# Eric-qi/NeuroQuant

Hardware: AMD Instinct MI355X
Metric: calibration iters/sec (HNeRV Bunny 1280x640, 21k iters) + final PSNR vs ref (higher is better)
Workload: dtype f32 operands split into bf16 hi+lo, 3 BF16 MFMAs per product, fp32 accumulate (bf16x3); fp32 MFMA on small layers; 1 GPU; HNeRV Bunny_1280x640_3M, channel_wise, bits 6 5 4 5 5 6 6, phase-2 (AdaRound) iteration; per_gpu_batch=2, global_batch=2, frames=132, parallelism=dp1

## Files before the change

include/nq_hip.h:

```cpp
#ifndef NQ_HIP_H
#define NQ_HIP_H

#include <stdint.h>

#ifdef __cplusplus
extern "C" {
#endif

typedef void* nq_stream_t;

#define NQ_API __attribute__((visibility("default")))

#define NQ_OK 0
#define NQ_ERR_INVALID (-1)
#define NQ_ERR_UNSUPPORTED (-2)
#define NQ_ERR_LAUNCH (-3)

NQ_API int nq_abi_version(void);
NQ_API const char* nq_error_string(int code);


NQ_API int nq_scale_init_max(const float* x, int64_t rows, int64_t row_len, int n_levels, float* delta, float* zp,
                      nq_stream_t stream);

// ... 113 lines not shown

#define NQ_EPI_PLAIN 0
#define NQ_EPI_PS_GELU 1
#define NQ_EPI_TANH 2
#define NQ_EPI_PS 3
#define NQ_EPI_DGRAD_GELU 4
#define NQ_EPI_X_SPLIT 0x100
#define NQ_EPI_Y_SPLIT 0x200
NQ_API int nq_split_words(const float* x, float* y, int64_t n, nq_stream_t stream);
NQ_API int64_t nq_conv_forward_ws_floats(int B, int Cin, int H, int W, int Cout, int k);
NQ_API int nq_conv_split_out(int B, int Cin, int H, int W, int Cout, int k, int r, int epilogue, int in_gelu, int has_bias);
NQ_API int nq_conv_forward(const float* x, const float* wt, const float* bias, float* y, float* z, float* ws, int B, int Cin, int H,
                    int W, int Cout, int k, int krows, int ld, int r, int epilogue, int in_gelu, const float* zprev,
                    nq_stream_t stream);

NQ_API int nq_conv3_supported(int B, int Cin, int H, int W, int Cout, int k);
NQ_API int nq_conv3_split_io(int B, int Cin, int H, int W, int Cout, int k);
NQ_API int64_t nq_conv_forward3_ws_floats(int B, int Cin, int H, int W, int Cout, int k);
NQ_API int64_t nq_conv3_weight_bytes(int Cin, int Cout, int k);
NQ_API int nq_weight_layout3(const float* w, void* wt3, int Cin, int Cout, int k, int transposed, nq_stream_t stream);
typedef struct nq_wl3_seg {
  const float* w;
  void* wt3;
  int Cin, Cout, k, transposed;
} nq_wl3_seg;
NQ_API int nq_weight_layout3_multi(const nq_wl3_seg* segs, int nseg, nq_stream_t stream);
NQ_API int nq_weight_layouts_all(const nq_wl3_seg* segs3, int n3, const nq_wl_seg* segsf, int nf, nq_stream_t stream);
NQ_API int nq_conv_forward3(const float* x, const void* wt3, const float* bias, float* y, float* z, const float* zprev, float* ws, int B,
                     int Cin, int H, int W, int Cout, int k, int r, int epilogue, nq_stream_t stream);

NQ_API int nq_conv_wgrad3_supported(int B, int Cin, int H, int W, int Cout, int k);
NQ_API int64_t nq_conv_wgrad3_ws_floats(int B, int Cin, int H, int W, int Cout, int k);
NQ_API int nq_conv_wgrad3_plan(int B, int Cin, int H, int W, int Cout, int k, int* mi, int* ni, int* nsplit, int* pc);
NQ_API int nq_conv_wgrad3(const float* x, const float* dy, float* dw, float* db, float* ws, int B, int Cin, int H, int W, int Cout,
                   int k, nq_stream_t stream);
NQ_API int nq_conv_wgrad3_split_io(int B, int Cin, int H, int W, int Cout, int k);
NQ_API int nq_conv_wgrad3_fmt(const float* x, const float* dy, float* dw, float* db, float* ws, int B, int Cin, int H, int W, int Cout,
                       int k, int fmt, nq_stream_t stream);
NQ_API int nq_conv_wgrad3_swapped(const float* x, const float* dy, float* dw, float* ws, int B, int Cin, int H, int W, int Cout, int k,
                           nq_stream_t stream);

NQ_API int64_t nq_conv_wgrad_ws_floats(int B, int Cin, int H, int W, int Cout, int k);
NQ_API int nq_conv_wgrad(const float* x, const float* dy, float* dw, float* db, float* ws, int B, int Cin, int H, int W, int Cout,
                  int k, int x_gelu, nq_stream_t stream);

typedef struct nq_wgr_seg {
  const float* slab;
  const float* slab_db;
  float* dw;
  float* db;
  int Cout, N, co_pad, n_pad, nsplit;
  int swap_kk;
  int sg;
} nq_wgr_seg;
NQ_API int nq_conv_wgrad3_slabs(const float* x, const float* dy, float* dw, float* db, float* ws, int B, int Cin, int H, int W, int Cout,
                         int k, nq_wgr_seg* seg, nq_stream_t stream);
NQ_API int nq_conv_wgrad3_slabs_fmt(const float* x, const float* dy, float* dw, float* db, float* ws, int B, int Cin, int H, int W,
                             int Cout, int k, nq_wgr_seg* seg, int fmt, nq_stream_t stream);
NQ_API int nq_conv_wgrad3_swapped_slabs(const float* x, const float* dy, float* dw, float* ws, int B, int Cin, int H, int W, int Cout,
                                 int k, nq_wgr_seg* seg, nq_stream_t stream);
NQ_API int nq_conv_wgrad_slabs(const float* x, const float* dy, float* dw, float* db, float* ws, int B, int Cin, int H, int W, int Cout,
                        int k, int x_gelu, nq_wgr_seg* seg, nq_stream_t stream);
NQ_API int nq_wgrad_reduce_multi(const nq_wgr_seg* segs, int nseg, nq_stream_t stream);

NQ_API int nq_ps_gelu_backward(const float* da, const float* z, float* dconv, int B, int C, int H, int W, int r,
                        nq_stream_t stream);

NQ_API int nq_tanh_out_backward(const float* dimg, const float* img, float* dconv, int64_t n, nq_stream_t stream);

NQ_API int nq_l2_loss(const float* pred, const float* tgt, float* loss, float* dpred, float* ws, int64_t n, int64_t mean_count,
               float gscale, nq_stream_t stream);

NQ_API int nq_channel_sum(const float* x, float* out, float* ws, int B, int C, int64_t HW, nq_stream_t stream);

NQ_API int nq_l2_loss_tanh_head(const float* pred, const float* tgt, const uint8_t* cache_u8, const int64_t* idx, float* loss,
                         float* dconv, float* db, float* ws, int B, int C, int64_t HW, int64_t mean_count, float gscale,
                         nq_stream_t stream);

NQ_API int64_t nq_head_forward_loss_ws_floats(int B, int H, int W);
NQ_API int nq_head_forward_loss(const float* x, const float* wt, int ld, const float* bias, float* y, const float* tgt,
                         const uint8_t* cache_u8, const int64_t* idx, float* loss, float* dconv, float* db, float* ws, int B,
                         int Cin, int H, int W, int64_t mean_count, float gscale, nq_stream_t stream);

NQ_API int nq_frame_sse(const float* out, const float* gt, float* sse, int64_t frames, int64_t frame_len, nq_stream_t stream);

NQ_API int64_t nq_ms_ssim_ws_floats(int64_t frames, int C, int H, int W);
NQ_API int nq_ms_ssim(const float* out, const float* gt, float* msssim, float* ws, int64_t frames, int C, int H, int W,
               nq_stream_t stream);

NQ_API int nq_gather_frames_u8(const uint8_t* src, const int64_t* idx, float* dst, int64_t n, int64_t frame_len,
                        nq_stream_t stream);

NQ_API int nq_act_dd(const float* x, const float* g, const float* g2, float* y, int64_t n, int mode, nq_stream_t stream);
NQ_API int nq_pixel_shuffle(const float* x, float* y, int B, int C, int H, int W, int r, int inverse, nq_stream_t stream);
NQ_API int nq_bias_add(const float* x, const float* bias, float* y, int B, int C, int64_t HW, nq_stream_t stream);

#ifdef __cplusplus
}
#endif
#endif
```

neuroquant_amd/_lib.py:

```python
import ctypes
import os
from ctypes import c_char_p, c_float, c_int, c_int64, c_void_p, POINTER, Structure

_HERE = os.path.dirname(os.path.abspath(__file__))
LIB_PATH = os.environ.get("NQ_LIB") or os.path.join(_HERE, "libnqhip.so")

NQ_OK = 0
ABI_VERSION = 5
EPI_PLAIN, EPI_PS_GELU, EPI_TANH, EPI_PS, EPI_DGRAD_GELU = 0, 1, 2, 3, 4


class NQLibraryError(RuntimeError):
    pass


class AdaSeg(Structure):
    _fields_ = [("x", c_void_p), ("gy", c_void_p), ("alpha", c_void_p), ("delta", c_void_p), ("zp", c_void_p),
                ("out", c_void_p), ("rows", c_int64), ("row_len", c_int64), ("per_row", c_int), ("n_levels", c_int),
                ("soft", c_int), ("reg_weight", c_float)]


class WL3Seg(Structure):
    _fields_ = [("w", c_void_p), ("wt3", c_void_p), ("Cin", c_int), ("Cout", c_int), ("k", c_int), ("transposed", c_int)]


class WLSeg(Structure):
    _fields_ = [("w", c_void_p), ("wt_fwd", c_void_p), ("wt_bwd", c_void_p), ("Cout", c_int), ("Cin", c_int), ("k", c_int),
                ("krows_fwd", c_int), ("ld_fwd", c_int), ("krows_bwd", c_int), ("ld_bwd", c_int)]


class FwhtSeg(Structure):
    _fields_ = [("x", c_void_p), ("y", c_void_p), ("outer", c_int64), ("inner", c_int64), ("n", c_int), ("n_in", c_int),
                ("n_out", c_int)]


class AdaAdamSeg(Structure):
    _fields_ = [("x", c_void_p), ("gy", c_void_p), ("alpha", c_void_p), ("delta", c_void_p), ("zp", c_void_p), ("m", c_void_p),
                ("v", c_void_p), ("rows", c_int64), ("row_len", c_int64), ("per_row", c_int), ("n_levels", c_int),
                ("reg_weight", c_float)]


class WgrSeg(Structure):
    _fields_ = [("slab", c_void_p), ("slab_db", c_void_p), ("dw", c_void_p), ("db", c_void_p), ("Cout", c_int), ("N", c_int),
                ("co_pad", c_int), ("n_pad", c_int), ("nsplit", c_int), ("swap_kk", c_int), ("sg", c_int)]


class FqFwhtSeg(Structure):
    _fields_ = [("x", c_void_p), ("alpha", c_void_p), ("delta", c_void_p), ("zp", c_void_p), ("m", c_void_p), ("v", c_void_p),
                ("gy", c_void_p), ("y", c_void_p), ("outer", c_int64), ("inner", c_int64), ("n", c_int), ("c_in", c_int),
                ("per_row", c_int), ("n_levels", c_int), ("soft", c_int), ("reg_weight", c_float)]


class AdamSeg(Structure):
    _fields_ = [("p", c_void_p), ("g", c_void_p), ("m", c_void_p), ("v", c_void_p), ("n", c_int64)]


def _load():
    if not os.path.exists(LIB_PATH):
        raise NQLibraryError(
            f"{LIB_PATH} not found: build it with `python -c 'import __graft_entry__ as g; g.build()'` "
            "(or `make -C neuroquant_amd/csrc`).  neuroquant_amd has no CPU/eager fallback.")
    import torch
    lib = ctypes.CDLL(LIB_PATH)
    P, I, L, F = c_void_p, c_int, c_int64, c_float

    def sig(name, res, *args):
        fn = getattr(lib, name)
        fn.restype = res
        fn.argtypes = list(args)

    sig("nq_abi_version", I)
    got = lib.nq_abi_version()
    if got != ABI_VERSION:
        raise NQLibraryError(f"{LIB_PATH} has ABI version {got}, this package binds version {ABI_VERSION}: rebuild it "
                             "(`make -C neuroquant_amd/csrc`)")
    sig("nq_error_string", c_char_p, I)
    sig("nq_scale_init_max", I, P, L, L, I, P, P, P)
    sig("nq_uaq_forward", I, P, P, P, P, L, L, I, I, P)
    sig("nq_uaq_backward", I, P, P, P, P, P, P, L, L, I, I, P)
    sig("nq_adaround_init", I, P, P, P, P, P, P, L, L, I, P)
    sig("nq_adaround_forward", I, P, P, P, P, P, P, L, L, I, I, I, P)
    sig("nq_adaround_backward", I, P, P, P, P, P, P, L, L, I, I, F, F, P)
    sig("nq_adaround_adam_multi", I, POINTER(AdaAdamSeg), I, F, F, F, F, F, F, P, P)
    sig("nq_adaround_forward_multi", I, POINTER(AdaSeg), I, P)
    sig("nq_uaq_forward_multi", I, POINTER(AdaSeg), I, P)
    sig("nq_uaq_backward_multi", I, POINTER(AdaSeg), I, P)
    sig("nq_adaround_backward_multi", I, POINTER(AdaSeg), I, F, P)
    sig("nq_adam_step_multi", I, POINTER(AdamSeg), I, F, F, F, F, F, P)
    sig("nq_step_prologue", I, P, P, P, P, P, I, I, P)
    sig("nq_step_prologue_gather", I, P, P, P, P, P, I, I, P, L, L, P, P)
    sig("nq_adaround_backward_multi_dyn", I, POINTER(AdaSeg), I, P, P)
    sig("nq_adam_step_multi_dyn", I, POINTER(AdamSeg), I, P, F, F, F, P)
    sig("nq_reduce_ws_floats", L, L)
    sig("nq_round_loss", I, P, L, F, F, P, P, I, P)
    sig("nq_round_loss_backward", I, P, L, F, F, P, P, I, P)
    sig("nq_adam_step", I, P, P, P, P, L, F, F, F, F, F, P)
    sig("nq_fwht", I, P, P, L, I, L, I, I, P)
    sig("nq_fwht_multi", I, POINTER(FwhtSeg), I, P)
    sig("nq_weight_layouts", I, P, P, P, I, I, I, I, I, I, I, P)
    sig("nq_conv_operand_dims", I, I, I, I, POINTER(c_int), POINTER(c_int))
    sig("nq_conv_forward_ws_floats", L, I, I, I, I, I, I)
    sig("nq_conv_forward", I, P, P, P, P, P, P, I, I, I, I, I, I, I, I, I, I, I, P, P)
    sig("nq_conv3_supported", I, I, I, I, I, I, I)
    sig("nq_conv3_split_io", I, I, I, I, I, I, I)
    sig("nq_conv_split_out", I, I, I, I, I, I, I, I, I, I, I)
    sig("nq_split_words", I, P, P, L, P)
    sig("nq_conv_wgrad3_split_io", I, I, I, I, I, I, I)
    sig("nq_conv_wgrad3_fmt", I, P, P, P, P, P, I, I, I, I, I, I, I, P)
    sig("nq_conv_wgrad3_slabs_fmt", I, P, P, P, P, P, I, I, I, I, I, I, POINTER(WgrSeg), I, P)
    sig("nq_conv3_weight_bytes", L, I, I, I)
    sig("nq_weight_layout3", I, P, P, I, I, I, I, P)
    sig("nq_weight_layout3_multi", I, POINTER(WL3Seg), I, P)
    sig("nq_weight_layouts_multi", I, POINTER(WLSeg), I, P)
    sig("nq_weight_layouts_all", I, POINTER(WL3Seg), I, POINTER(WLSeg), I, P)
    sig("nq_conv_forward3_ws_floats", L, I, I, I, I, I, I)
    sig("nq_conv_forward3", I, P, P, P, P, P, P, P, I, I, I, I, I, I, I, I, P)
    sig("nq_conv_wgrad3_supported", I, I, I, I, I, I, I)
    sig("nq_conv_wgrad3_ws_floats", L, I, I, I, I, I, I)
    sig("nq_conv_wgrad3_plan", I, I, I, I, I, I, I, POINTER(c_int), POINTER(c_int), POINTER(c_int), POINTER(c_int))
    sig("nq_conv_wgrad3", I, P, P, P, P, P, I, I, I, I, I, I, P)
    sig("nq_conv_wgrad3_swapped", I, P, P, P, P, I, I, I, I, I, I, P)
    sig("nq_conv_wgrad3_slabs", I, P, P, P, P, P, I, I, I, I, I, I, POINTER(WgrSeg), P)
    sig("nq_conv_wgrad3_swapped_slabs", I, P, P, P, P, I, I, I, I, I, I, POINTER(WgrSeg), P)
    sig("nq_conv_wgrad_slabs", I, P, P, P, P, P, I, I, I, I, I, I, I, POINTER(WgrSeg), P)
    sig("nq_wgrad_reduce_multi", I, POINTER(WgrSeg), I, P)
    sig("nq_conv_wgrad_ws_floats", L, I, I, I, I, I, I)
    sig("nq_conv_wgrad", I, P, P, P, P, P, I, I, I, I, I, I, I, P)
    sig("nq_ps_gelu_backward", I, P, P, P, I, I, I, I, I, P)
    sig("nq_tanh_out_backward", I, P, P, P, L, P)
    sig("nq_l2_loss", I, P, P, P, P, P, L, L, F, P)
    sig("nq_channel_sum", I, P, P, P, I, I, L, P)
    sig("nq_l2_loss_tanh_head", I, P, P, P, P, P, P, P, P, I, I, L, L, F, P)
    sig("nq_frame_sse", I, P, P, P, L, L, P)
    sig("nq_ms_ssim_ws_floats", L, L, I, I, I)
    sig("nq_ms_ssim", I, P, P, P, P, L, I, I, I, P)
    sig("nq_gather_frames_u8", I, P, P, P, L, L, P)
    sig("nq_adaround_fwht_multi", I, POINTER(FqFwhtSeg), I, P)
    sig("nq_fwht_adaround_adam_multi", I, POINTER(FqFwhtSeg), I, F, F, F, F, F, F, P, P)
    sig("nq_head_forward_loss_ws_floats", L, I, I, I)
    sig("nq_head_forward_loss", I, P, P, I, P, P, P, P, P, P, P, P, P, I, I, I, I, L, F, P)
    sig("nq_act_dd", I, P, P, P, P, L, I, P)
    sig("nq_pixel_shuffle", I, P, P, I, I, I, I, I, I, P)
    sig("nq_bias_add", I, P, P, P, I, I, L, P)
    return lib


EXPORTS = (
    "nq_abi_version", "nq_error_string", "nq_scale_init_max", "nq_uaq_forward", "nq_uaq_backward",
    "nq_adaround_init", "nq_adaround_forward", "nq_adaround_backward", "nq_reduce_ws_floats", "nq_round_loss", "nq_round_loss_backward",
    "nq_adam_step", "nq_adaround_adam_multi", "nq_adaround_forward_multi", "nq_uaq_forward_multi", "nq_uaq_backward_multi", "nq_adaround_backward_multi", "nq_adam_step_multi", "nq_step_prologue", "nq_step_prologue_gather", "nq_adaround_backward_multi_dyn", "nq_adam_step_multi_dyn", "nq_fwht", "nq_fwht_multi", "nq_weight_layouts", "nq_conv_operand_dims", "nq_conv_forward_ws_floats", "nq_conv_forward",
    "nq_conv3_supported", "nq_conv3_weight_bytes", "nq_weight_layout3", "nq_weight_layout3_multi", "nq_weight_layouts_multi", "nq_conv_forward3_ws_floats", "nq_conv_forward3",
    "nq_conv_wgrad3_supported", "nq_conv_wgrad3_ws_floats", "nq_conv_wgrad3_plan", "nq_conv_wgrad3", "nq_conv_wgrad3_swapped",
    "nq_conv_wgrad3_slabs", "nq_conv_wgrad3_swapped_slabs", "nq_conv_wgrad_slabs", "nq_wgrad_reduce_multi",
    "nq_conv_wgrad_ws_floats", "nq_conv_wgrad", "nq_ps_gelu_backward", "nq_tanh_out_backward", "nq_l2_loss",
    "nq_channel_sum", "nq_l2_loss_tanh_head", "nq_frame_sse", "nq_ms_ssim_ws_floats", "nq_ms_ssim", "nq_gather_frames_u8",
    "nq_act_dd", "nq_pixel_shuffle", "nq_bias_add", "nq_conv3_split_io", "nq_conv_split_out", "nq_split_words",
    "nq_conv_wgrad3_split_io", "nq_conv_wgrad3_fmt", "nq_conv_wgrad3_slabs_fmt", "nq_head_forward_loss_ws_floats", "nq_head_forward_loss",
    "nq_adaround_fwht_multi", "nq_fwht_adaround_adam_multi", "nq_weight_layouts_all",
)

_lib = None


def lib():
    global _lib
    if _lib is None:
        _lib = _load()
    return _lib


def check(rc, what=""):
    if rc != NQ_OK:
        msg = lib().nq_error_string(rc).decode()
        raise NQLibraryError(f"libnqhip {what}: {msg} ({rc})")
```

neuroquant_amd/csrc/conv3.hip:

```cpp
#include <cstdlib>
#include "nq_common.h"
#include "conv3_layout.h"

extern "C" {
int nq_conv_igemm3_k3(const float*, const void*, const float*, float*, float*, const float*, int, int, int, int, int, int, int,
                      int, int, int, float*, hipStream_t);
int nq_conv_igemm3_k5(const float*, const void*, const float*, float*, float*, const float*, int, int, int, int, int, int, int,
                      int, int, int, float*, hipStream_t);
int nq_conv_splitk_finish(const float*, const float*, float*, float*, const float*, int, int, int, int, int, int, int, hipStream_t);
int nq_conv3_nst_k3();
int nq_conv3_nst_k5();
int nq_conv3_nst8_k3();
int nq_conv3_nst8_k5();
int nq_conv3_nstk_k3(int);
int nq_conv3_nstk_k5(int);
int nq_conv_flat3_plan(int, int, int, int, int, int, int*, int*, int*, int*);
int nq_conv_flat3(const float*, const void*, const float*, float*, float*, const float*, float*, int, int, int, int, int, int, int, int,
                  int, int, int, int, hipStream_t);
int nq_conv_wgrad_flat3_ok(int, int, int, int, int, int);
int nq_conv_wgrad_flat3(const float*, const float*, float*, float*, int, int, int, int, int, int, hipStream_t);
int nq_conv_wgrad3_k3(const float*, const float*, float*, float*, int, int, int, int, int, int, int, int, int, int, int, int, hipStream_t);
int nq_conv_wgrad3_k5(const float*, const float*, float*, float*, int, int, int, int, int, int, int, int, int, int, int, int, hipStream_t);
}

namespace {

constexpr int CC = 16;

inline int pick_mi3(int Cout) {
  if (Cout <= 16) return 1;
  if (Cout <= 32) return 2;
  int best = 3, best_pad = 1 << 30;
  for (int mi = 5; mi >= 3; --mi) {
    int mt = 16 * mi, pad = (Cout + mt - 1) / mt * mt;
    if (pad < best_pad) {
      best_pad = pad;
      best = mi;
    }
  }
  if (Cout > 256 && (Cout + 63) / 64 * 64 <= best_pad + best_pad * 6 / 100) return 4;
  return best;
}
inline int nst_of(int k) { return k == 5 ? nq_conv3_nst_k5() : nq_conv3_nst_k3(); }
inline int nstk_of(int k, int kind) { return k == 5 ? nq_conv3_nstk_k5(kind) : nq_conv3_nstk_k3(kind); }
inline int tail_kind_of(int Cin, int mi) {
  const int r = Cin - CC * ((Cin + CC - 1) / CC - 1);
  return r <= 4 ? 1 : (r <= 8 ? 2 : (r <= 12 ? 3 : 0));
}
inline int64_t total_steps3(int Cin, int k, int mi) {
  const int nchunk = (Cin + CC - 1) / CC;
  return (int64_t)(nchunk - 1) * nst_of(k) + nstk_of(k, tail_kind_of(Cin, mi));
}

struct WL3 {
  const float* w;
  uint4* out;
  int Cin, Cout, KK, NST, NSTT, nchunk, tail, co_tiles, MT, transposed;
  int co16;
  int64_t slots;
};

constexpr int WL3_KKMAX = 25;
template <int KK>
__device__ __forceinline__ void wl3_tile(const WL3& p, int c, int g16, float* __restrict__ T ) {
  constexpr int RS = 16 * KK + 1;
  const int tid = threadIdx.x;
  const int nfull = p.nchunk - (p.tail ? 1 : 0);
  const int kind = (c == nfull) ? p.tail : 0;
  const int nst = kind ? p.NSTT : p.NST;
  const int64_t gs0 = (int64_t)c * p.NST;
  const int Ra = p.transposed ? p.Cin : p.Cout;
  const int Cb = p.transposed ? p.Cout : p.Cin;
  const int a0 = p.transposed ? c * 16 : g16 * 16, b0 = p.transposed ? g16 * 16 : c * 16;
  {
    float v[KK];
#pragma unroll
    for (int j = 0; j < KK; ++j) {
      const int e = tid + j * 256;
      const int a = e / (16 * KK), rem = e - a * (16 * KK);
      const int bb = rem / KK;
      const bool ok = a0 + a < Ra && b0 + bb < Cb;
      const float t = p.w[ok ? ((int64_t)(a0 + a) * Cb + b0) * KK + rem : 0];
      v[j] = ok ? t : 0.f;
    }
#pragma unroll
// ... 175 lines not shown
  p.pc = 0;
  const bool pc_ok = wgrad3_pc_enabled() && (int64_t)B * Cin * H * W * 4 < (1ll << 31) && (int64_t)B * Cout * H * W * 4 < (1ll << 31);
  if (pc_ok && p.ni >= 5 && p.mi >= 3 && tiles <= 256) {
    int sy = 1;
    int ns_pc = 256 / tiles;
    const int segs_x = (W + 31) / 32;
    static const int minseg = [] { const char* e = std::getenv("NQ_WGRAD3_MINSEG"); return e ? atoi(e) : 6; }();
    if (!wgrad3_ss1() && ns_pc >= 1) {
      if (H % 4 == 0 && segs_x * (H / 4) * B / ns_pc >= minseg) sy = 4;
      else if (H % 2 == 0 && segs_x * (H / 2) * B / ns_pc >= minseg) sy = 2;
    }
    const int nseg_pc = segs_x * (H / sy) * B;
    const int need = minseg < 16 ? minseg : 16;
    static const int shrink = [] { const char* e = std::getenv("NQ_WGRAD3_SHRINK"); return e ? atoi(e) : 1; }();
    if (shrink && ns_pc >= 1 && nseg_pc / ns_pc < need && (nseg_pc / need) * tiles >= 192) ns_pc = nseg_pc / need;
    if (ns_pc >= 1 && nseg_pc / ns_pc >= need) {
      p.pc = sy == 1 ? 1 : 10 + sy;
      p.nsplit = ns_pc;
    }
  }
  if (pc_ok && p.ni == 1 && p.mi >= 2 && p.mi <= 5 && tiles == 1 && W % 128 == 0) {
    const int nseg_pc = (W / 128) * H * B;
    if (nseg_pc / 256 >= 8) {
      p.pc = 4;
      static const int hs = [] { const char* e = std::getenv("NQ_WGRAD3_HEAD_SPLITS"); return e ? atoi(e) : 512; }();
      p.nsplit = (p.mi <= 3 && nseg_pc / hs >= 8) ? hs : 256;
    }
  }
  return p;
}

template <int SG>
__global__ __launch_bounds__(256) void wgrad3_reduce_kernel(const float* __restrict__ slab, const float* __restrict__ slab_db,
                                                            float* __restrict__ dw, float* __restrict__ db, int Cout, int N,
                                                            int co_pad, int n_pad, int nsplit, int swap_kk) {
  constexpr int OG = 256 / SG;
  __shared__ float part[SG][OG];
  const int o = threadIdx.x % OG, g = threadIdx.x / OG;
  const int64_t i = (int64_t)blockIdx.x * OG + o;
  const int64_t total = (int64_t)Cout * N;
  float s = 0.f;
  if (i < total) {
    const int co = (int)(i / N), n = (int)(i - (int64_t)co * N);
    const float* p = slab + (int64_t)co * n_pad + n;
    const int64_t stride = (int64_t)co_pad * n_pad;
#pragma unroll 4
    for (int k = g; k < nsplit; k += SG) s += p[k * stride];
  } else if (db && i < total + Cout) {
    const int co = (int)(i - total);
#pragma unroll 4
    for (int k = g; k < nsplit; k += SG) s += slab_db[(int64_t)k * co_pad + co];
  }
  part[g][o] = s;
  __syncthreads();
  if (g == 0) {
    float t = part[0][o];
#pragma unroll
    for (int j = 1; j < SG; ++j) t += part[j][o];
    if (i < total) {
      if (swap_kk > 0) {
        const int co = (int)(i / N), n = (int)(i - (int64_t)co * N);
        const int ci = n / swap_kk, tap = n - ci * swap_kk;
        dw[((int64_t)ci * Cout + co) * swap_kk + (swap_kk - 1 - tap)] = t;
      } else {
        dw[i] = t;
      }
    } else if (db && i < total + Cout) {
      db[(int)(i - total)] = t;
    }
  }
}

constexpr int WGR_MAXSEG = 16;
struct WGRMulti {
  nq_wgr_seg s[WGR_MAXSEG];
  int blk0[WGR_MAXSEG + 1];
  int nseg;
};
__global__ __launch_bounds__(256) void wgrad_reduce_multi_kernel(WGRMulti t) {
  __shared__ float4 part[256];
  int k = 0;
  while (k + 1 < t.nseg && (int)blockIdx.x >= t.blk0[k + 1]) ++k;
  const nq_wgr_seg& q = t.s[k];
  const int SG = q.sg, OG = 256 / SG;
  const int o = threadIdx.x % OG, g = threadIdx.x / OG;
  const int N = q.N, Cout = q.Cout, nsplit = q.nsplit;
  const int NQ = (N + 3) >> 2;
  const int64_t i = (int64_t)((int)blockIdx.x - t.blk0[k]) * OG + o;
  const int64_t total = (int64_t)Cout * NQ;
  float4 s = make_float4(0.f, 0.f, 0.f, 0.f);
  int co = 0, n = 0;
  if (i < total) {
    co = (int)(i / NQ);
    n = 4 * (int)(i - (int64_t)co * NQ);
    const float* p = q.slab + (int64_t)co * q.n_pad + n;
    const int64_t stride = (int64_t)q.co_pad * q.n_pad;
#pragma unroll 8
    for (int j = g; j < nsplit; j += SG) {
      const float4 v = *reinterpret_cast<const float4*>(p + j * stride);
      s.x += v.x; s.y += v.y; s.z += v.z; s.w += v.w;
    }
  } else if (q.db && i < total + Cout) {
    const int cb = (int)(i - total);
#pragma unroll 8
    for (int j = g; j < nsplit; j += SG) s.x += q.slab_db[(int64_t)j * q.co_pad + cb];
  }
  if (SG > 1) {
    part[g * OG + o] = s;
    __syncthreads();
    if (g != 0) return;
    s = part[o];
    for (int j = 1; j < SG; ++j) {
      const float4 v = part[j * OG + o];
      s.x += v.x; s.y += v.y; s.z += v.z; s.w += v.w;
    }
  }
  if (i < total) {
    const float sv[4] = {s.x, s.y, s.z, s.w};
    if (q.swap_kk > 0) {
#pragma unroll
      for (int e = 0; e < 4; ++e) {
        if (n + e >= N) break;
        const int ci = (n + e) / q.swap_kk, tap = (n + e) - ci * q.swap_kk;
        q.dw[((int64_t)ci * Cout + co) * q.swap_kk + (q.swap_kk - 1 - tap)] = sv[e];
      }
    } else if ((N & 3) == 0) {
      *reinterpret_cast<float4*>(q.dw + (int64_t)co * N + n) = s;
    } else {
#pragma unroll
      for (int e = 0; e < 4; ++e)
        if (n + e < N) q.dw[(int64_t)co * N + n + e] = sv[e];
    }
  } else if (q.db && i < total + Cout) {
    q.db[(int)(i - total)] = s.x;
  }
}

}

extern "C" {

int nq_conv3_supported(int B, int Cin, int H, int W, int Cout, int k) {
  if (!(k == 3 || k == 5) || B <= 0 || Cin <= 0 || Cout <= 4 || Cin <= 4) return 0;
  if ((int64_t)B * Cin * H * W * 4 >= 0xFFFFFF00ll) return 0;
  if (use_flat3(B, Cin, H, W, Cout, k, nullptr) && (int64_t)Cin * k * k * Cout >= 65536) return 1;
  const Fwd3Plan p = plan_fwd3(B, Cin, H, W, Cout);
  return p.wgs * p.nsplit >= 128;
}

int64_t nq_conv_forward3_ws_floats(int B, int Cin, int H, int W, int Cout, int k) {
  if (!(k == 3 || k == 5) || B <= 0 || Cin <= 0 || H <= 0 || W <= 0 || Cout <= 0) return 0;
  int fns = 1;
  if (use_flat3(B, Cin, H, W, Cout, k, &fns)) return fns > 1 ? (int64_t)fns * B * Cout * H * W : 0;
  const Fwd3Plan p = plan_fwd3(B, Cin, H, W, Cout);
  return p.nsplit > 1 ? (int64_t)p.nsplit * B * Cout * H * W : 0;
}

int64_t nq_conv3_weight_bytes(int Cin, int Cout, int k) {
  if (!(k == 3 || k == 5)) return 0;
  const int mi = pick_mi3(Cout), mt = 16 * mi;
  const int64_t co_tiles = (Cout + mt - 1) / mt, nchunk = (Cin + CC - 1) / CC;
  (void)nchunk;
  return total_steps3(Cin, k, mi) * 2 * co_tiles * 4 * mt * 16;
}

static bool wl3_fill(WL3& p, const float* w, void* wt3, int Cin, int Cout, int k, int transposed) {
  if (!w || !wt3 || !(k == 3 || k == 5) || Cin <= 0 || Cout <= 0) return false;
  const int mi = pick_mi3(Cout);
  p.w = w; p.out = reinterpret_cast<uint4*>(wt3);
  p.Cin = Cin; p.Cout = Cout; p.KK = k * k; p.NST = nst_of(k); p.tail = tail_kind_of(Cin, mi); p.NSTT = nstk_of(k, p.tail);
  p.MT = 16 * mi; p.co_tiles = (Cout + p.MT - 1) / p.MT; p.nchunk = (Cin + CC - 1) / CC; p.transposed = transposed;
  p.slots = total_steps3(Cin, k, mi) * p.co_tiles * 4 * p.MT;
  p.co16 = (p.co_tiles * p.MT + 15) / 16;
  return true;
}

int nq_weight_layout3(const float* w, void* wt3, int Cin, int Cout, int k, int transposed, nq_stream_t stream) {
  WL3 p;
  if (!wl3_fill(p, w, wt3, Cin, Cout, k, transposed)) return NQ_ERR_INVALID;
  hipLaunchKernelGGL(weight_layout3_kernel, dim3((unsigned)(p.nchunk * p.co16)), dim3(256), 0, nq_s(stream), p);
  return nq_launch_status();
}

int nq_weight_layout3_multi(const nq_wl3_seg* segs, int nseg, nq_stream_t stream) {
  if (!segs || nseg <= 0) return NQ_ERR_INVALID;
  for (int base = 0; base < nseg; base += WL3_MAXSEG) {
    WL3Multi t;
    t.nseg = (nseg - base < WL3_MAXSEG) ? nseg - base : WL3_MAXSEG;
    int blocks = 0;
    for (int i = 0; i < t.nseg; ++i) {
      const nq_wl3_seg& h = segs[base + i];
      if (!wl3_fill(t.s[i], h.w, h.wt3, h.Cin, h.Cout, h.k, h.transposed)) return NQ_ERR_INVALID;
      t.blk0[i] = blocks;
      blocks += t.s[i].nchunk * t.s[i].co16;
    }
    t.blk0[t.nseg] = blocks;
    hipLaunchKernelGGL(weight_layout3_multi_kernel, dim3((unsigned)blocks), dim3(256), 0, nq_s(stream), t);
  }
  return nq_launch_status();
// ... 212 lines not shown
```

neuroquant_amd/csrc/conv_head.hip:

```cpp
#include <cstdlib>
#include <cstring>
#include <type_traits>

#include "nq_common.h"

namespace {

constexpr int MAXCO = 4;
using f32x2 = __attribute__((ext_vector_type(2))) float;
using f32x4 = __attribute__((ext_vector_type(4))) float;

template <int I0, int N, class F>
__device__ __forceinline__ void hf2_rows(F&& f) {
  if constexpr (I0 < N) {
    f(std::integral_constant<int, I0>{});
    hf2_rows<I0 + 1, N>(f);
  }
}

template <int KS>
__global__ __launch_bounds__(256) void head_fwd_kernel(const float* __restrict__ x, const float* __restrict__ wt, int ld,
                                                       const float* __restrict__ bias, float* __restrict__ y, int Cin,
                                                       int H, int W, int CO, int epi, int tiles_x) {
  constexpr int KK = KS * KS, PAD = KS / 2;
// ... 215 lines not shown
    __builtin_amdgcn_s_waitcnt(0xC07F);
    __builtin_amdgcn_sched_barrier(0);
    load_x(ci + 2, vA, eA);
    load_w(ci + 2, wA);
    __builtin_amdgcn_sched_barrier(0);
    compute(vB, eB, wB);
    __builtin_amdgcn_s_waitcnt(0xC07F);
    __builtin_amdgcn_sched_barrier(0);
  }
  if (Cin & 1) compute(vA, eA, wA);

  float bv[NCO];
#pragma unroll
  for (int co = 0; co < NCO; ++co) bv[co] = bias ? bias[co] : 0.f;
  float lsum = 0.f, gsum[NCO];
#pragma unroll
  for (int co = 0; co < NCO; ++co) gsum[co] = 0.f;
  __amdgpu_buffer_rsrc_t rs_d = rs_y;
  int64_t tbase = 0;
  if constexpr (LOSS) {
    rs_d = __builtin_amdgcn_make_buffer_rsrc(la.dconv, 0, (int)((unsigned)a.B * NCO * HWb), 0x00020000);
    tbase = (la.cache ? la.idx[b] : (int64_t)b) * NCO * (int64_t)H * W;
  }
#pragma unroll
  for (int r = 0; r < R; ++r) {
    const int oy = y0 + r;
    const bool in = oy < H && gx < W;
    const unsigned so = in ? ((unsigned)b * NCO * (unsigned)H + (unsigned)oy) * Wb + (unsigned)gx * 4u : OOB;
#pragma unroll
    for (int co = 0; co < NCO; ++co) {
      f32x4 o;
#pragma unroll
      for (int p = 0; p < 4; ++p) {
        const float v = acc[r][co][p >> 1][p & 1] + bv[co];
        o[p] = TANH ? tanhf(v) * 0.5f + 0.5f : v;
      }
      __builtin_amdgcn_raw_buffer_store_b128(__builtin_bit_cast(__attribute__((ext_vector_type(4))) unsigned, o), rs_y,
                                             so == OOB ? OOB : so + (unsigned)co * HWb, 0, 0);
      if constexpr (LOSS) {
        f32x4 t4 = {0.f, 0.f, 0.f, 0.f};
        if (in) {
          const int64_t te = tbase + ((int64_t)co * H + oy) * W + gx;
          if (la.cache) {
            const uchar4 u = *reinterpret_cast<const uchar4*>(la.cache + te);
            t4 = f32x4{(float)u.x / 255.f, (float)u.y / 255.f, (float)u.z / 255.f, (float)u.w / 255.f};
          } else {
            t4 = *reinterpret_cast<const f32x4*>(la.tgt + te);
          }
        }
        f32x4 dc;
#pragma unroll
        for (int p = 0; p < 4; ++p) {
          const float d = o[p] - t4[p];
          const float g = la.gcoef * d;
          const float u = 2.f * o[p] - 1.f;
          const float rr = g * 0.5f * (1.f - u * u);
          dc[p] = rr;
          if (in) {
            lsum += d * d;
            gsum[co] += rr;
          }
        }
        __builtin_amdgcn_raw_buffer_store_b128(__builtin_bit_cast(__attribute__((ext_vector_type(4))) unsigned, dc), rs_d,
                                               so == OOB ? OOB : so + (unsigned)co * HWb, 0, 0);
      }
    }
  }
  if constexpr (LOSS) {
    lsum = nq_wave_sum(lsum);
#pragma unroll
    for (int co = 0; co < NCO; ++co) gsum[co] = nq_wave_sum(gsum[co]);
    if (lane == 0) {
      float* w4 = la.ws + (int64_t)wid * 4;
      w4[0] = lsum;
#pragma unroll
      for (int co = 0; co < NCO && co < 3; ++co) w4[1 + co] = gsum[co];
    }
  }
}

__global__ __launch_bounds__(256) void head_loss_stage2(const float* __restrict__ ws, int waves, float scale,
                                                        float* __restrict__ loss, float* __restrict__ db) {
  __shared__ float red[16];
  float acc = 0.f;
  for (int i = threadIdx.x; i < waves; i += 256) acc += ws[(int64_t)i * 4 + blockIdx.x];
  const float s = nq_block_sum(acc, red);
  if (threadIdx.x == 0) {
    if (blockIdx.x == 0) loss[0] = 0.f + s * scale;
    else db[blockIdx.x - 1] = s;
  }
}

template <int KS, int R2, int NCO, int PX>
__global__ __launch_bounds__(256) __attribute__((amdgpu_waves_per_eu((KS <= 3 && NCO <= 3 && R2 && PX == 4) ? 4 : 1, 8))) void head_dgrad_kernel(const float* __restrict__ dy, const float* __restrict__ wt, int ld,
                                                         const float* __restrict__ zprev, float* __restrict__ out,
                                                         int Cin, int H, int W, int CO, int r, int tiles_x) {
  constexpr int KK = KS * KS, PAD = KS / 2;
  constexpr int TW = 64, TPR = TW / PX, TH = 256 / TPR;
  constexpr int PH = TH + KS - 1, PW = TW + KS - 1;
  constexpr int PWS = (PW + 3) / 4 * 4;
  __shared__ __attribute__((aligned(16))) float patch[NCO * PH * PWS];
  constexpr int KKP = (KK + 3) / 4 * 4;
  constexpr int WROW = NCO * KKP;
  constexpr int WL_MAX = 64;
  __shared__ __attribute__((aligned(16))) float wl[WL_MAX * WROW];

  const int tid = threadIdx.x;
  const int row = tid / TPR, c4 = (tid % TPR) * PX;
  const int lid = nq_xcd_chunk((int)blockIdx.x, (int)gridDim.x);
  const int tiles = tiles_x * ((H + TH - 1) / TH), tile = lid % tiles;
  const int tile_x = tile % tiles_x, tile_y = tile / tiles_x;
  const int x0 = tile_x * TW, y0 = tile_y * TH, b = lid / tiles;
  const int64_t HW = (int64_t)H * W;
  const float* __restrict__ dyb = dy + (int64_t)b * CO * HW;

  for (int e = tid; e < CO * PH * PW; e += 256) {
    int co = e / (PH * PW), rem = e - co * (PH * PW);
    int rr = rem / PW, c = rem - rr * PW;
    int gy = y0 - PAD + rr, gx = x0 - PAD + c;
    float v = 0.f;
    if (gy >= 0 && gy < H && gx >= 0 && gx < W) v = dyb[(int64_t)co * HW + (int64_t)gy * W + gx];
    patch[(co * PH + rr) * PWS + c] = v;
  }
  __syncthreads();
  float nb[NCO][KS][PX + KS - 1];
#pragma unroll
  for (int co = 0; co < NCO; ++co)
#pragma unroll
    for (int kh = 0; kh < KS; ++kh)
#pragma unroll
      for (int j = 0; j < PX + KS - 1; ++j) nb[co][kh][j] = (co < CO) ? patch[(co * PH + row + kh) * PWS + c4 + j] : 0.f;

  const int gy = y0 + row, gx0 = x0 + c4;
  const bool active = (gy < H && gx0 < W);
  const bool full = (gx0 + PX - 1 < W);
#pragma unroll 1
  for (int ci = 0; ci < Cin; ++ci) {
    if (ci % WL_MAX == 0) {
      __syncthreads();
      const int nci = min(WL_MAX, Cin - ci);
      for (int e = tid; e < nci * WROW; e += 256) {
        const int cl = e / WROW, j = e - cl * WROW;
        const int co = j / KKP, tap = j - co * KKP;
        wl[e] = (co < CO && tap < KK) ? wt[(int64_t)(co * KK + tap) * ld + ci + cl] : 0.f;
      }
      __syncthreads();
    }
    if (!active) continue;
    float acc[PX];
#pragma unroll
    for (int p = 0; p < PX; ++p) acc[p] = 0.f;
    const float* __restrict__ wrow = wl + (ci % WL_MAX) * WROW;
#pragma unroll
    for (int co = 0; co < NCO; ++co) {
      if (co < CO) {
        float wv[KKP];
#pragma unroll
        for (int q = 0; q < KKP / 4; ++q) {
          const float4 t = *reinterpret_cast<const float4*>(wrow + co * KKP + 4 * q);
          wv[4 * q] = t.x; wv[4 * q + 1] = t.y; wv[4 * q + 2] = t.z; wv[4 * q + 3] = t.w;
        }
#pragma unroll
        for (int kh = 0; kh < KS; ++kh)
#pragma unroll
          for (int kw = 0; kw < KS; ++kw) {
#pragma unroll
            for (int p = 0; p < PX; ++p) acc[p] = fmaf(wv[kh * KS + kw], nb[co][kh][p + kw], acc[p]);
          }
        __builtin_amdgcn_sched_barrier(0);
// ... 148 lines not shown
            acc0 = __builtin_elementwise_fma(w2, f32x2{in[kw], in[kw + 1]}, acc0);
            acc1 = __builtin_elementwise_fma(w2, f32x2{in[kw + 2], in[kw + 3]}, acc1);
          }
      const f32x4 zz = z[r];
      f32x2 ev = {acc0[0] * zz[0], acc1[0] * zz[2]}, od = {acc0[1] * zz[1], acc1[1] * zz[3]};
      if (a.out_split) {
        ev = f32x2{nq_split_word_f(ev[0]), nq_split_word_f(ev[1])};
        od = f32x2{nq_split_word_f(od[0]), nq_split_word_f(od[1])};
      }
      const unsigned vo = oo[r];
      __builtin_amdgcn_raw_buffer_store_b64(__builtin_bit_cast(__attribute__((ext_vector_type(2))) unsigned, ev), rs_o, vo, so, 0);
      __builtin_amdgcn_raw_buffer_store_b64(__builtin_bit_cast(__attribute__((ext_vector_type(2))) unsigned, od), rs_o,
                                            vo == OOB ? OOB : vo + plane_b, so, 0);
    }
  };

  f32x4 zA[R], zB[R], wA[WROW / 4], wB[WROW / 4];
  load_z(0, zA);
  load_w(0, wA);
#pragma unroll 1
  for (int ci = 0; ci + 1 < Cin; ci += 2) {
    load_z(ci + 1, zB);
    load_w(ci + 1, wB);
    __builtin_amdgcn_sched_barrier(0);
    compute(ci, zA, wA);
    __builtin_amdgcn_sched_barrier(0);
    load_z(ci + 2, zA);
    load_w(ci + 2, wA);
    __builtin_amdgcn_sched_barrier(0);
    compute(ci + 1, zB, wB);
    __builtin_amdgcn_sched_barrier(0);
  }
  if (Cin & 1) compute(Cin - 1, zA, wA);
}

}

extern "C" {

int nq_head_supported(int Cout, int k) { return Cout <= MAXCO && (k == 1 || k == 3 || k == 5); }

int nq_head_forward(const float* x, const float* wt, int ld, const float* bias, float* y, int B, int Cin, int H, int W,
                    int Cout, int k, int epi, hipStream_t st) {
  const char* hv = getenv("NQ_HEAD_FWD");
  const bool v1 = hv && hv[0] == '1';
  if (k == 3 && Cout == 3 && (W & 3) == 0 && (ld & 3) == 0 && (int64_t)B * Cin * H * W * 4 < 0xFFFFFF00ll && !v1) {
    int R = 4;
    if (const char* rd = getenv("NQ_HEAD_RD")) R = atoi(rd);
    HeadFwd2Args a;
    a.B = B; a.Cin = Cin; a.H = H; a.W = W; a.ld = ld;
    a.strips = (W + 255) / 256; a.rblocks = (H + R - 1) / R;
    a.x_bytes = (unsigned)((int64_t)B * Cin * H * W * 4);
    a.hot_first = head_hot_first(B, a.strips, a.rblocks);
    const int waves = B * a.strips * a.rblocks;
    dim3 g2((unsigned)((waves + 3) / 4)), blk2(256);
    const size_t lds = 0;
    const bool th = epi == NQ_EPI_TANH;
#define NQ_HF2(R_)                                                                                              \
  if (R == R_) {                                                                                                \
    if (th) hipLaunchKernelGGL((head_fwd2_kernel<R_, 3, true>), g2, blk2, lds, st, x, wt, bias, y, a);          \
    else hipLaunchKernelGGL((head_fwd2_kernel<R_, 3, false>), g2, blk2, lds, st, x, wt, bias, y, a);            \
    return nq_launch_status();                                                                                  \
  }
    NQ_HF2(4)
    NQ_HF2(5)
#undef NQ_HF2
    return NQ_ERR_UNSUPPORTED;
  }
  const int tiles_x = (W + 63) / 64, tiles = tiles_x * ((H + 15) / 16);
  dim3 g((unsigned)(tiles * B)), blk(256);
  switch (k) {
    case 1: hipLaunchKernelGGL(head_fwd_kernel<1>, g, blk, 0, st, x, wt, ld, bias, y, Cin, H, W, Cout, epi, tiles_x); break;
    case 3: hipLaunchKernelGGL(head_fwd_kernel<3>, g, blk, 0, st, x, wt, ld, bias, y, Cin, H, W, Cout, epi, tiles_x); break;
    default: hipLaunchKernelGGL(head_fwd_kernel<5>, g, blk, 0, st, x, wt, ld, bias, y, Cin, H, W, Cout, epi, tiles_x); break;
  }
  return nq_launch_status();
}

int64_t nq_head_forward_loss_ws_floats(int B, int H, int W) {
  if (B <= 0 || H <= 0 || W <= 0) return 0;
  return (int64_t)B * ((W + 255) / 256) * ((H + 3) / 4) * 4;
}

int nq_head_forward_loss(const float* x, const float* wt, int ld, const float* bias, float* y, const float* tgt,
                         const uint8_t* cache_u8, const int64_t* idx, float* loss, float* dconv, float* db, float* ws, int B,
                         int Cin, int H, int W, int64_t mean_count, float gscale, nq_stream_t stream) {
  if (!x || !wt || !y || !loss || !dconv || !db || !ws || B <= 0 || Cin <= 0 || H <= 0 || W <= 0 || mean_count <= 0) return NQ_ERR_INVALID;
  if ((tgt == nullptr) == (cache_u8 == nullptr) || (cache_u8 && !idx)) return NQ_ERR_INVALID;
  if ((W & 3) != 0 || (ld & 3) != 0 || (int64_t)B * Cin * H * W * 4 >= 0xFFFFFF00ll) return NQ_ERR_UNSUPPORTED;
  constexpr int R = 4;
  HeadFwd2Args a;
  a.B = B; a.Cin = Cin; a.H = H; a.W = W; a.ld = ld;
  a.strips = (W + 255) / 256; a.rblocks = (H + R - 1) / R;
  a.x_bytes = (unsigned)((int64_t)B * Cin * H * W * 4);
  a.hot_first = head_hot_first(B, a.strips, a.rblocks);
  HeadLossArgs la;
  la.tgt = tgt; la.cache = cache_u8; la.idx = idx; la.dconv = dconv; la.ws = ws;
  la.gcoef = (float)(2.0 / (double)mean_count) * gscale;
  const int waves = B * a.strips * a.rblocks;
  hipStream_t st = nq_s(stream);
  hipLaunchKernelGGL((head_fwd2_kernel<R, 3, true, true>), dim3((unsigned)((waves + 3) / 4)), dim3(256), 0, st, x, wt, bias, y, a, la);
  hipLaunchKernelGGL(head_loss_stage2, dim3(4), dim3(256), 0, st, ws, waves, (float)(1.0 / (double)mean_count), loss, db);
  return nq_launch_status();
}

int nq_head_dgrad_streams(int B, int Cin, int H, int W, int Cout, int k, int r, int has_z) {
  const char* hv = getenv("NQ_HEAD_DGRAD");
  const char* rd = getenv("NQ_HEAD_DG_R");
  const int R = rd ? atoi(rd) : 4;
  return k == 3 && Cout == 3 && r == 2 && has_z && (W % 4 == 0) && (H % 2 == 0) && (int64_t)B * Cin * H * W * 4 < 0xFFFFFF00ll &&
         !(hv && hv[0] == '1') && (size_t)Cin * 28 * 4 <= 64 * 1024 && (R == 2 || R == 4);
}

int nq_head_dgrad(const float* dy, const float* wt, int ld, const float* zprev, float* out, int B, int Cin, int H, int W,
                  int Cout, int k, int r, int out_split, hipStream_t st) {
  if (out_split && !nq_head_dgrad_streams(B, Cin, H, W, Cout, k, r, zprev != nullptr)) return NQ_ERR_UNSUPPORTED;
  const char* hv = getenv("NQ_HEAD_DGRAD");
  if (k == 3 && Cout == 3 && r == 2 && zprev && (W % 4 == 0) && (H % 2 == 0) && (int64_t)B * Cin * H * W * 4 < 0xFFFFFF00ll &&
      !(hv && hv[0] == '1')) {
    int R = 4;
    if (const char* rd = getenv("NQ_HEAD_DG_R")) R = atoi(rd);
    HeadDg2Args a;
    a.B = B; a.Cin = Cin; a.H = H; a.W = W; a.ld = ld;
    a.strips = (W + 255) / 256; a.rblocks = (H + R - 1) / R;
    a.dy_bytes = (unsigned)((int64_t)B * Cout * H * W * 4);
    a.z_bytes = (unsigned)((int64_t)B * Cin * H * W * 4);
    a.out_split = out_split;
    const int waves = B * a.strips * a.rblocks;
    dim3 g2((unsigned)((waves + 3) / 4)), blk2(256);
    const size_t lds = (size_t)Cin * 28 * 4;
    if (lds <= 64 * 1024) {
      if (R == 2) hipLaunchKernelGGL((head_dgrad2_kernel<2, 3>), g2, blk2, lds, st, dy, wt, zprev, out, a);
      else if (R == 4) hipLaunchKernelGGL((head_dgrad2_kernel<4, 3>), g2, blk2, lds, st, dy, wt, zprev, out, a);
      else return NQ_ERR_UNSUPPORTED;
      return nq_launch_status();
    }
  }
  const bool r2 = (r == 2) && (W % 4 == 0) && (H % 2 == 0);
  const bool px8 = r2 && (W % 8 == 0) && k <= 3;
  const int th = px8 ? 32 : 16;
  const int tiles_x = (W + 63) / 64, tiles = tiles_x * ((H + th - 1) / th);
  dim3 g((unsigned)(tiles * B)), blk(256);
#define NQ_HD(KS_, R2_, PX_)                                                                                          \
  do {                                                                                                                \
    if (Cout <= 3)                                                                                                    \
      hipLaunchKernelGGL((head_dgrad_kernel<KS_, R2_, 3, PX_>), g, blk, 0, st, dy, wt, ld, zprev, out, Cin, H, W, Cout, r, \
                         tiles_x);                                                                                    \
    else                                                                                                              \
      hipLaunchKernelGGL((head_dgrad_kernel<KS_, R2_, 4, PX_>), g, blk, 0, st, dy, wt, ld, zprev, out, Cin, H, W, Cout, r, \
                         tiles_x);                                                                                    \
  } while (0)
  switch (k) {
    case 1: if (px8) NQ_HD(1, 1, 8); else if (r2) NQ_HD(1, 1, 4); else NQ_HD(1, 0, 4); break;
    case 3: if (px8) NQ_HD(3, 1, 8); else if (r2) NQ_HD(3, 1, 4); else NQ_HD(3, 0, 4); break;
    default: if (r2) NQ_HD(5, 1, 4); else NQ_HD(5, 0, 4); break;
  }
#undef NQ_HD
  return nq_launch_status();
}

}
```

neuroquant_amd/csrc/conv_tiny.hip:

```cpp
#include "nq_common.h"

namespace {

template <int KSL>
__global__ __launch_bounds__(256) void tiny_pw_fwd_kernel(const float* __restrict__ x, const float* __restrict__ wt,
                                                          const float* __restrict__ bias, float* __restrict__ y,
                                                          float* __restrict__ z, const float* __restrict__ zprev, int B,
                                                          int Cin, int H, int W, int Cout, int ld, int r, int epi) {
  constexpr int OPB = 256 / KSL;
  __shared__ float part[KSL][OPB];
  const int HW = H * W;
  const int o = threadIdx.x % OPB, ks = threadIdx.x / OPB;
  const int64_t t = (int64_t)blockIdx.x * OPB + o;
  const bool live = t < (int64_t)B * HW * Cout;
  const int co = live ? (int)(t % Cout) : 0, bp = live ? (int)(t / Cout) : 0;
  const int b = bp / HW, p = bp - b * HW;
  const float* __restrict__ xp = x + (int64_t)b * Cin * HW + p;
  float acc = 0.f;
#pragma unroll 8
  for (int ci = ks; ci < Cin; ci += KSL) acc = fmaf(wt[(int64_t)ci * ld + co], xp[(int64_t)ci * HW], acc);
  if (KSL > 1) {
    part[ks][o] = acc;
    __syncthreads();
    if (ks != 0) return;
    acc = part[0][o];
#pragma unroll
    for (int j = 1; j < KSL; ++j) acc += part[j][o];
  }
  if (!live) return;
  float v = acc + (bias ? bias[co] : 0.f);
  const int py = p / W, px = p - py * W;
  if (epi == NQ_EPI_PS_GELU || epi == NQ_EPI_PS) {
    const int rr = r * r, C = Cout / rr;
    const int c = co / rr, rem = co - c * rr, si = rem / r, sj = rem - si * r;
    const int64_t o = (((int64_t)b * C + c) * (H * r) + (int64_t)py * r + si) * ((int64_t)W * r) + (int64_t)px * r + sj;
    if (epi == NQ_EPI_PS_GELU) {
      float gv, dv;
      nq_gelu_pair(v, gv, dv);
      y[o] = gv;
      z[o] = dv;
    } else {
      z[o] = v;
    }
  } else if (epi == NQ_EPI_DGRAD_GELU) {
    const int64_t i = ((int64_t)b * Cout + co) * HW + p;
    v *= zprev[i];
    if (r == 1) {
      y[i] = v;
    } else {
      const int rr = r * r, yq = py / r, xq = px / r;
      const int ch = co * rr + (py - yq * r) * r + (px - xq * r);
      y[(((int64_t)b * Cout * rr + ch) * (H / r) + yq) * (int64_t)(W / r) + xq] = v;
    }
  } else {
    const int64_t i = ((int64_t)b * Cout + co) * HW + p;
    y[i] = (epi == NQ_EPI_TANH) ? tanhf(v) * 0.5f + 0.5f : v;
  }
}

__global__ __launch_bounds__(256) void tiny_pw_wgrad_kernel(const float* __restrict__ x, const float* __restrict__ dy,
                                                            float* __restrict__ dw, float* __restrict__ db, int B, int Cin,
                                                            int HW, int Cout) {
  const int64_t t = (int64_t)blockIdx.x * 256 + threadIdx.x;
  const int64_t nw = (int64_t)Cout * Cin;
  if (t < nw) {
    const int co = (int)(t / Cin), ci = (int)(t - (int64_t)co * Cin);
    float acc = 0.f;
    for (int b = 0; b < B; ++b) {
      const float* __restrict__ dp = dy + ((int64_t)b * Cout + co) * HW;
      const float* __restrict__ xp = x + ((int64_t)b * Cin + ci) * HW;
      if ((HW & 7) == 0) {
        for (int p = 0; p < HW; p += 8) {
          const float4 d0 = *reinterpret_cast<const float4*>(dp + p), d1 = *reinterpret_cast<const float4*>(dp + p + 4);
          const float4 x0 = *reinterpret_cast<const float4*>(xp + p), x1 = *reinterpret_cast<const float4*>(xp + p + 4);
          acc = fmaf(d0.x, x0.x, acc); acc = fmaf(d0.y, x0.y, acc); acc = fmaf(d0.z, x0.z, acc); acc = fmaf(d0.w, x0.w, acc);
          acc = fmaf(d1.x, x1.x, acc); acc = fmaf(d1.y, x1.y, acc); acc = fmaf(d1.z, x1.z, acc); acc = fmaf(d1.w, x1.w, acc);
        }
      } else {
        for (int p = 0; p < HW; ++p) acc = fmaf(dp[p], xp[p], acc);
      }
    }
    dw[t] = acc;
  } else if (db && t < nw + Cout) {
    const int co = (int)(t - nw);
    float acc = 0.f;
    for (int b = 0; b < B; ++b) {
      const float* __restrict__ dp = dy + ((int64_t)b * Cout + co) * HW;
      for (int p = 0; p < HW; ++p) acc += dp[p];
    }
    db[co] = acc;
  }
}

}

extern "C" {

int nq_tiny_pw_supported(int B, int Cin, int H, int W, int Cout, int k) {
  return k == 1 && (int64_t)B * H * W <= 256 && (int64_t)B * H * W * Cout < (1ll << 31);
}

int nq_tiny_pw_forward(const float* x, const float* wt, const float* bias, float* y, float* z, const float* zprev, int B,
                       int Cin, int H, int W, int Cout, int ld, int r, int epi, hipStream_t st) {
  const int64_t total = (int64_t)B * H * W * Cout;
  if (Cin > 1024)
    hipLaunchKernelGGL(tiny_pw_fwd_kernel<64>, dim3((unsigned)((total + 3) / 4)), dim3(256), 0, st, x, wt, bias, y, z, zprev,
                       B, Cin, H, W, Cout, ld, r, epi);
  else if (Cin > 256)
    hipLaunchKernelGGL(tiny_pw_fwd_kernel<16>, dim3((unsigned)((total + 15) / 16)), dim3(256), 0, st, x, wt, bias, y, z, zprev,
                       B, Cin, H, W, Cout, ld, r, epi);
  else if (Cin > 48)
    hipLaunchKernelGGL(tiny_pw_fwd_kernel<4>, dim3((unsigned)((total + 63) / 64)), dim3(256), 0, st, x, wt, bias, y, z, zprev,
                       B, Cin, H, W, Cout, ld, r, epi);
  else
    hipLaunchKernelGGL(tiny_pw_fwd_kernel<1>, dim3((unsigned)((total + 255) / 256)), dim3(256), 0, st, x, wt, bias, y, z, zprev,
                       B, Cin, H, W, Cout, ld, r, epi);
  return nq_launch_status();
}

int nq_tiny_pw_wgrad(const float* x, const float* dy, float* dw, float* db, int B, int Cin, int H, int W, int Cout,
                     hipStream_t st) {
  const int64_t total = (int64_t)Cout * Cin + (db ? Cout : 0);
  hipLaunchKernelGGL(tiny_pw_wgrad_kernel, dim3((unsigned)((total + 255) / 256)), dim3(256), 0, st, x, dy, dw, db, B, Cin,
                     H * W, Cout);
  return nq_launch_status();
}

}
```

neuroquant_amd/csrc/nq_common.h:

```cpp
#pragma once
#include <hip/hip_runtime.h>
#include <stdint.h>

#include <atomic>

#include "../../include/nq_hip.h"

#define NQ_WAVE 64

static inline int nq_launch_status() {
  hipError_t e = hipGetLastError();
  return e == hipSuccess ? NQ_OK : NQ_ERR_LAUNCH;
}

static inline hipStream_t nq_s(nq_stream_t s) { return reinterpret_cast<hipStream_t>(s); }

template <auto Kernel>
static inline int nq_lds_optin(size_t lds) {
  if (lds <= 64 * 1024) return NQ_OK;
  static std::atomic<size_t> granted[64];
  int dev = 0;
  if (hipGetDevice(&dev) != hipSuccess) return NQ_ERR_LAUNCH;
  std::atomic<size_t>& g = granted[dev & 63];
  if (g.load(std::memory_order_acquire) >= lds) return NQ_OK;
  if (hipFuncSetAttribute(reinterpret_cast<const void*>(Kernel), hipFuncAttributeMaxDynamicSharedMemorySize, (int)lds) != hipSuccess)
    return NQ_ERR_LAUNCH;
  size_t cur = g.load(std::memory_order_relaxed);
  while (cur < lds && !g.compare_exchange_weak(cur, lds, std::memory_order_release)) {
  }
  return NQ_OK;
}

__device__ __forceinline__ int nq_xcd_chunk(int id, int n) {
  const int q = n >> 3, r = n & 7;
  const int k = id & 7, i = id >> 3;
  return k * q + (k < r ? k : r) + i;
}

__device__ __forceinline__ void nq_gelu_pair(float v, float& g, float& dg) {
  const float ax = fabsf(v) * 0.70710678118654752440f;
  const float e = __builtin_amdgcn_exp2f((v * v) * -0.72134752044448170368f);
  const float t = __builtin_amdgcn_rcpf(__builtin_fmaf(0.3275911f, ax, 1.0f));
  float p = __builtin_fmaf(1.061405429f, t, -1.453152027f);
  p = __builtin_fmaf(p, t, 1.421413741f);
  p = __builtin_fmaf(p, t, -0.284496736f);
  p = __builtin_fmaf(p, t, 0.254829592f);
  const float erf_abs = 1.0f - (p * t) * e;
  const float er = __builtin_copysignf(erf_abs, v);
  const float cdf = __builtin_fmaf(0.5f, er, 0.5f);
  g = v * cdf;
  dg = __builtin_fmaf(v, 0.39894228040143267794f * e, cdf);
}

__device__ __forceinline__ unsigned nq_split_word_u(float v) {
  const __bf16 h = (__bf16)v;
  const __bf16 l = (__bf16)(v - (float)h);
  return ((unsigned)__builtin_bit_cast(unsigned short, h) << 16) | (unsigned)__builtin_bit_cast(unsigned short, l);
}
__device__ __forceinline__ float nq_split_word_f(float v) { return __builtin_bit_cast(float, nq_split_word_u(v)); }
__device__ __forceinline__ float nq_split_word_value(unsigned w) {
  return __builtin_bit_cast(float, w & 0xffff0000u) + __builtin_bit_cast(float, w << 16);
}

__device__ __forceinline__ float nq_wave_sum(float v) {
#pragma unroll
  for (int o = 32; o > 0; o >>= 1) v += __shfl_down(v, o, 64);
  return v;
}
__device__ __forceinline__ float nq_wave_min(float v) {
#pragma unroll
  for (int o = 32; o > 0; o >>= 1) v = fminf(v, __shfl_down(v, o, 64));
  return v;
}
__device__ __forceinline__ float nq_wave_max(float v) {
#pragma unroll
  for (int o = 32; o > 0; o >>= 1) v = fmaxf(v, __shfl_down(v, o, 64));
  return v;
}

__device__ __forceinline__ float nq_block_sum(float v, float* smem ) {
  const int lane = threadIdx.x & 63, wave = threadIdx.x >> 6, nw = (blockDim.x + 63) >> 6;
  v = nq_wave_sum(v);
  __syncthreads();
  if (lane == 0) smem[wave] = v;
  __syncthreads();
  float r = 0.f;
  if (threadIdx.x == 0)
    for (int i = 0; i < nw; ++i) r += smem[i];
  return r;
}

#define NQ_GAMMA (-0.1f)
#define NQ_ZETA (1.1f)

__device__ __forceinline__ float nq_sigmoid(float a) { return 1.0f / (1.0f + expf(-a)); }

static __global__ __launch_bounds__(256) void nq_sum_stage2(const float* __restrict__ ws, int64_t nparts, float scale,
                                                           float* __restrict__ out, int accumulate) {
  __shared__ float red[16];
  float acc = 0.f;
  for (int64_t i = threadIdx.x; i < nparts; i += 256) acc += ws[i];
  float s = nq_block_sum(acc, red);
  if (threadIdx.x == 0) out[0] = (accumulate ? out[0] : 0.f) + s * scale;
}
#define NQ_RED_CHUNK 4096
```

neuroquant_amd/csrc/quant.hip:

```cpp
#include "nq_common.h"
#include "quant_elem.h"

namespace {

constexpr int TPB = 256;
constexpr int EPT = 4;

__global__ __launch_bounds__(TPB) void scale_init_kernel(const float* __restrict__ x, int64_t row_len, int n_levels,
                                                         float* __restrict__ delta, float* __restrict__ zp) {
  __shared__ float smin[4], smax[4];
  const float* xr = x + (int64_t)blockIdx.x * row_len;
  float mn = 0.f, mx = 0.f;
  for (int64_t i = threadIdx.x; i < row_len; i += TPB) {
    float v = xr[i];
    mn = fminf(mn, v);
    mx = fmaxf(mx, v);
  }
  mn = nq_wave_min(mn);
  mx = nq_wave_max(mx);
  if ((threadIdx.x & 63) == 0) {
    smin[threadIdx.x >> 6] = mn;
    smax[threadIdx.x >> 6] = mx;
  }
  __syncthreads();
  if (threadIdx.x == 0) {
    for (int i = 1; i < TPB / 64; ++i) {
      mn = fminf(mn, smin[i]);
      mx = fmaxf(mx, smax[i]);
    }
    float d = (float)(((double)mx - (double)mn) / (double)(n_levels - 1));
    d = fmaxf(d, 1e-8f);
    delta[blockIdx.x] = d;
    zp[blockIdx.x] = rintf((-mn) / d);
  }
}

__global__ __launch_bounds__(TPB) void uaq_fwd_kernel(const float* __restrict__ x, const float* __restrict__ delta,
                                                      const float* __restrict__ zp, float* __restrict__ y,
                                                      int64_t row_len, int per_row, float qmax, unsigned bpr) {
  const int64_t row = blockIdx.x / bpr;
  const float d = per_row ? delta[row] : delta[0];
  const float z = per_row ? zp[row] : zp[0];
  const int64_t base = row * row_len;
  int64_t i = (int64_t)(blockIdx.x - row * bpr) * (TPB * EPT) + threadIdx.x;
#pragma unroll
  for (int e = 0; e < EPT; ++e, i += TPB) {
    if (i < row_len) {
      float xi = rintf(x[base + i] / d) + z;
      float xq = fminf(fmaxf(xi, 0.f), qmax);
      y[base + i] = (xq - z) * d;
    }
  }
}

__global__ __launch_bounds__(TPB) void uaq_bwd_kernel(const float* __restrict__ x, const float* __restrict__ gy,
                                                      const float* __restrict__ delta, const float* __restrict__ zp,
                                                      float* __restrict__ ddelta, float* __restrict__ dx,
                                                      int64_t row_len, int per_row, float qmax) {
  __shared__ float red[16];
  const int64_t row = blockIdx.x;
  const float d = per_row ? delta[row] : delta[0];
  const float z = per_row ? zp[row] : zp[0];
  const int64_t base = row * row_len;
  float acc = 0.f;
  for (int64_t i = threadIdx.x; i < row_len; i += TPB) {
    float u = x[base + i] / d;
    float xi = rintf(u) + z;
    float xq = fminf(fmaxf(xi, 0.f), qmax);
    float inside = (xi >= 0.f && xi <= qmax) ? 1.f : 0.f;
    const float g = gy[base + i];
    acc += g * ((xq - z) - inside * u);
    if (dx) dx[base + i] = inside != 0.f ? (g * d) / d : 0.f;
  }
  float s = nq_block_sum(acc, red);
  if (threadIdx.x == 0) ddelta[row] = s;
}

__device__ __forceinline__ float half_round_trip(float v) { return (float)(_Float16)v; }

__global__ void adaround_scale_kernel(const float* __restrict__ din, const float* __restrict__ zin,
                                      float* __restrict__ dout, float* __restrict__ zout, int64_t n) {
  int64_t i = (int64_t)blockIdx.x * blockDim.x + threadIdx.x;
  if (i < n) {
    dout[i] = half_round_trip(din[i]);
// ... 178 lines not shown
      const bool in = i0 + j < sg.n;
      xv[j] = in ? sg.x[i0 + j] : 0.f;
      av[j] = in ? sg.alpha[i0 + j] : 0.f;
      if (BWD) gv[j] = in ? sg.gy[i0 + j] : 0.f;
    }
  }
  const int64_t row0 = sg.per_row ? i0 / sg.row_len : 0;
  const int rem0 = sg.per_row ? (int)(i0 - row0 * sg.row_len) : 0;
  const float rb = (BWD && t.dyn) ? t.dyn[0] : t.reg_b;
  const float rw = (BWD && t.dyn) ? sg.reg_weight * t.dyn[1] : sg.reg_weight;
#pragma unroll
  for (int j = 0; j < 4; ++j) {
    int64_t row = 0;
    if (sg.per_row) row = (sg.row_len >= 4) ? row0 + ((rem0 + j >= sg.row_len) ? 1 : 0) : (i0 + j) / sg.row_len;
    if (i0 + j >= sg.n) row = 0;
    const float d = sg.delta[row], z = sg.zp[row];
    if (BWD) {
      ov[j] = ada_bwd_elem(xv[j], gv[j], av[j], d, z, sg.qmax, rw, rb);
    } else {
      float xq;
      ov[j] = ada_fwd_elem(xv[j], av[j], d, z, sg.qmax, sg.soft, xq);
    }
  }
  if (vec) {
    *reinterpret_cast<float4*>(sg.out + i0) = make_float4(ov[0], ov[1], ov[2], ov[3]);
  } else {
#pragma unroll
    for (int j = 0; j < 4; ++j)
      if (i0 + j < sg.n) sg.out[i0 + j] = ov[j];
  }
}

__global__ __launch_bounds__(TPB) void adam_multi_kernel(AdamMulti t, float step_size, float beta1, float beta2, float eps,
                                                         float bc2_sqrt, const float* __restrict__ dyn) {
  if (dyn) {
    step_size = dyn[2];
    bc2_sqrt = dyn[3];
  }
  const int k = find_seg(t, blockIdx.x);
  const AdamSegD& sg = t.s[k];
  const int64_t i0 = (int64_t)(blockIdx.x - t.blk0[k]) * (TPB * EPT) + 4 * threadIdx.x;
  if (i0 >= sg.n) return;
  if (sg.vec && i0 + 3 < sg.n) {
    const float4 g4 = *reinterpret_cast<const float4*>(sg.g + i0);
    float4 m4 = *reinterpret_cast<const float4*>(sg.m + i0), v4 = *reinterpret_cast<const float4*>(sg.v + i0);
    float4 p4 = *reinterpret_cast<const float4*>(sg.p + i0);
    const float g[4] = {g4.x, g4.y, g4.z, g4.w};
    float m[4] = {m4.x, m4.y, m4.z, m4.w}, v[4] = {v4.x, v4.y, v4.z, v4.w}, p[4] = {p4.x, p4.y, p4.z, p4.w};
#pragma unroll
    for (int j = 0; j < 4; ++j) {
      m[j] = m[j] + (1.f - beta1) * (g[j] - m[j]);
      v[j] = v[j] * beta2 + (1.f - beta2) * (g[j] * g[j]);
      const float denom = sqrtf(v[j]) / bc2_sqrt + eps;
      p[j] = p[j] - step_size * (m[j] / denom);
    }
    *reinterpret_cast<float4*>(sg.m + i0) = make_float4(m[0], m[1], m[2], m[3]);
    *reinterpret_cast<float4*>(sg.v + i0) = make_float4(v[0], v[1], v[2], v[3]);
    *reinterpret_cast<float4*>(sg.p + i0) = make_float4(p[0], p[1], p[2], p[3]);
  } else {
#pragma unroll
    for (int j = 0; j < 4; ++j)
      if (i0 + j < sg.n) adam_elem(sg.p, sg.g, sg.m, sg.v, i0 + j, step_size, beta1, beta2, eps, bc2_sqrt);
  }
}

struct AdaAdamSegD {
  const float* x;
  const float* gy;
  float* alpha;
  const float* delta;
  const float* zp;
  float* m;
  float* v;
  int64_t n;
  int row_len, per_row;
  float qmax, reg_weight;
  int vec;
};
struct AdaAdamMulti {
  AdaAdamSegD s[MAXSEG];
  int blk0[MAXSEG + 1];
  int nseg;
};
__global__ __launch_bounds__(TPB) void adaround_adam_multi_kernel(AdaAdamMulti t, float reg_b, float step_size, float beta1,
                                                                  float beta2, float eps, float bc2_sqrt,
                                                                  const float* __restrict__ dyn) {
  float gate = 1.f;
  if (dyn) {
    reg_b = dyn[0];
    gate = dyn[1];
    step_size = dyn[2];
    bc2_sqrt = dyn[3];
  }
  const int k = find_seg(t, blockIdx.x);
  const AdaAdamSegD& sg = t.s[k];
  const int64_t i0 = (int64_t)(blockIdx.x - t.blk0[k]) * (TPB * EPT) + 4 * threadIdx.x;
  if (i0 >= sg.n) return;
  const bool vec = sg.vec && (i0 + 3 < sg.n);
  float xv[4], av[4], gv[4], mv[4], vv[4];
  if (vec) {
    const float4 x4 = *reinterpret_cast<const float4*>(sg.x + i0), a4 = *reinterpret_cast<const float4*>(sg.alpha + i0);
    const float4 g4 = *reinterpret_cast<const float4*>(sg.gy + i0);
    const float4 m4 = *reinterpret_cast<const float4*>(sg.m + i0), v4 = *reinterpret_cast<const float4*>(sg.v + i0);
    xv[0] = x4.x; xv[1] = x4.y; xv[2] = x4.z; xv[3] = x4.w;
    av[0] = a4.x; av[1] = a4.y; av[2] = a4.z; av[3] = a4.w;
    gv[0] = g4.x; gv[1] = g4.y; gv[2] = g4.z; gv[3] = g4.w;
    mv[0] = m4.x; mv[1] = m4.y; mv[2] = m4.z; mv[3] = m4.w;
    vv[0] = v4.x; vv[1] = v4.y; vv[2] = v4.z; vv[3] = v4.w;
  } else {
#pragma unroll
    for (int j = 0; j < 4; ++j) {
      const bool in = i0 + j < sg.n;
      xv[j] = in ? sg.x[i0 + j] : 0.f;
      av[j] = in ? sg.alpha[i0 + j] : 0.f;
      gv[j] = in ? sg.gy[i0 + j] : 0.f;
      mv[j] = in ? sg.m[i0 + j] : 0.f;
      vv[j] = in ? sg.v[i0 + j] : 0.f;
    }
  }
  const int64_t row0 = sg.per_row ? i0 / sg.row_len : 0;
  const int rem0 = sg.per_row ? (int)(i0 - row0 * sg.row_len) : 0;
  const float rw = dyn ? sg.reg_weight * gate : sg.reg_weight;
#pragma unroll
  for (int j = 0; j < 4; ++j) {
    int64_t row = 0;
    if (sg.per_row) row = (sg.row_len >= 4) ? row0 + ((rem0 + j >= sg.row_len) ? 1 : 0) : (i0 + j) / sg.row_len;
    if (i0 + j >= sg.n) row = 0;
    const float g = ada_bwd_elem(xv[j], gv[j], av[j], sg.delta[row], sg.zp[row], sg.qmax, rw, reg_b);
    mv[j] = mv[j] + (1.f - beta1) * (g - mv[j]);
    vv[j] = vv[j] * beta2 + (1.f - beta2) * (g * g);
    const float denom = sqrtf(vv[j]) / bc2_sqrt + eps;
    av[j] = av[j] - step_size * (mv[j] / denom);
  }
  if (vec) {
    *reinterpret_cast<float4*>(sg.m + i0) = make_float4(mv[0], mv[1], mv[2], mv[3]);
    *reinterpret_cast<float4*>(sg.v + i0) = make_float4(vv[0], vv[1], vv[2], vv[3]);
    *reinterpret_cast<float4*>(sg.alpha + i0) = make_float4(av[0], av[1], av[2], av[3]);
  } else {
#pragma unroll
    for (int j = 0; j < 4; ++j)
      if (i0 + j < sg.n) {
        sg.m[i0 + j] = mv[j];
        sg.v[i0 + j] = vv[j];
        sg.alpha[i0 + j] = av[j];
      }
  }
}

struct UaqSegD {
  const float* x;
  const float* gy;
  const float* delta;
  const float* zp;
  float* out;
  int64_t n;
  int64_t rows;
  int row_len, per_row;
  float qmax;
};
struct UaqMulti {
  UaqSegD s[MAXSEG];
  int blk0[MAXSEG + 1];
  int nseg;
};
__global__ __launch_bounds__(TPB) void uaq_fwd_multi_kernel(UaqMulti t) {
  const int k = find_seg(t, blockIdx.x);
  const UaqSegD& sg = t.s[k];
  int64_t i = (int64_t)(blockIdx.x - t.blk0[k]) * (TPB * EPT) + threadIdx.x;
#pragma unroll
  for (int e = 0; e < EPT; ++e, i += TPB) {
    if (i < sg.n) {
      const int64_t row = sg.per_row ? i / sg.row_len : 0;
      const float d = sg.delta[row], z = sg.zp[row];
      float xi = rintf(sg.x[i] / d) + z;
      float xq = fminf(fmaxf(xi, 0.f), sg.qmax);
      sg.out[i] = (xq - z) * d;
    }
  }
}
__global__ __launch_bounds__(TPB) void uaq_bwd_multi_kernel(UaqMulti t) {
  __shared__ float red[16];
  const int k = find_seg(t, blockIdx.x);
  const UaqSegD& sg = t.s[k];
  const int64_t row = blockIdx.x - t.blk0[k];
  const float d = sg.delta[row], z = sg.zp[row];
  const int64_t base = row * sg.row_len;
  float acc = 0.f;
  for (int64_t i = threadIdx.x; i < sg.row_len; i += TPB) {
    float u = sg.x[base + i] / d;
    float xi = rintf(u) + z;
    float xq = fminf(fmaxf(xi, 0.f), sg.qmax);
    float inside = (xi >= 0.f && xi <= sg.qmax) ? 1.f : 0.f;
    acc += sg.gy[base + i] * ((xq - z) - inside * u);
  }
  float s = nq_block_sum(acc, red);
  if (threadIdx.x == 0) sg.out[row] = s;
}

inline unsigned blocks_per_row(int64_t row_len) { return (unsigned)((row_len + TPB * EPT - 1) / (TPB * EPT)); }
inline dim3 row_grid(int64_t rows, int64_t row_len) { return dim3((unsigned)(rows * blocks_per_row(row_len)), 1, 1); }
inline bool bad_rows(int64_t rows, int64_t row_len) {
  return rows <= 0 || row_len <= 0 || rows * (int64_t)blocks_per_row(row_len) > 0x7fffffffLL;
}

}

extern "C" {

int nq_abi_version(void) { return 5; }

const char* nq_error_string(int code) {
  switch (code) {
    case NQ_OK: return "ok";
    case NQ_ERR_INVALID: return "invalid argument";
    case NQ_ERR_UNSUPPORTED: return "unsupported shape";
    case NQ_ERR_LAUNCH: return "HIP launch error";
    default: return "unknown error";
  }
}

int nq_scale_init_max(const float* x, int64_t rows, int64_t row_len, int n_levels, float* delta, float* zp,
                      nq_stream_t stream) {
  if (!x || !delta || !zp || rows <= 0 || row_len <= 0 || n_levels < 2) return NQ_ERR_INVALID;
  hipLaunchKernelGGL(scale_init_kernel, dim3((unsigned)rows), dim3(TPB), 0, nq_s(stream), x, row_len, n_levels, delta,
                     zp);
  return nq_launch_status();
}

// ... 160 lines not shown
          h.row_len > 0x7fffffffLL)
        return NQ_ERR_INVALID;
      AdaSegD& d = t.s[k];
      d.x = h.x; d.gy = h.gy; d.alpha = h.alpha; d.delta = h.delta; d.zp = h.zp; d.out = h.out;
      d.n = h.rows * h.row_len; d.row_len = (int)h.row_len; d.per_row = h.per_row; d.soft = h.soft;
      d.qmax = (float)(h.n_levels - 1); d.reg_weight = h.reg_weight;
      d.vec = (((uintptr_t)h.x | (uintptr_t)h.alpha | (uintptr_t)h.out | (uintptr_t)(bwd ? h.gy : h.x)) & 15) == 0;
      t.blk0[k] = blocks;
      blocks += (int)((d.n + TPB * EPT - 1) / (TPB * EPT));
    }
    t.blk0[t.nseg] = blocks;
    if (bwd)
      hipLaunchKernelGGL(adaround_multi_kernel<true>, dim3((unsigned)blocks), dim3(TPB), 0, nq_s(stream), t);
    else
      hipLaunchKernelGGL(adaround_multi_kernel<false>, dim3((unsigned)blocks), dim3(TPB), 0, nq_s(stream), t);
  }
  return nq_launch_status();
}

int nq_adaround_forward_multi(const nq_ada_seg* segs, int nseg, nq_stream_t stream) {
  return ada_multi(segs, nseg, 0.f, nullptr, false, stream);
}

int nq_adaround_backward_multi(const nq_ada_seg* segs, int nseg, float reg_b, nq_stream_t stream) {
  return ada_multi(segs, nseg, reg_b, nullptr, true, stream);
}

int nq_adaround_backward_multi_dyn(const nq_ada_seg* segs, int nseg, const float* dyn, nq_stream_t stream) {
  if (!dyn) return NQ_ERR_INVALID;
  return ada_multi(segs, nseg, 0.f, dyn, true, stream);
}

int nq_step_prologue(const int64_t* order, const float* scal, int* step, int64_t* cur_idx, float* cur_scal, int B, int nscal,
                     nq_stream_t stream) {
  if (!order || !scal || !step || !cur_idx || !cur_scal || B <= 0 || B > 256 || nscal <= 0 || nscal > 256) return NQ_ERR_INVALID;
  hipLaunchKernelGGL(step_prologue_kernel, dim3(1), dim3(256), 0, nq_s(stream), order, scal, step, cur_idx, cur_scal, B, nscal);
  return nq_launch_status();
}

int nq_step_prologue_gather(const int64_t* order, const float* scal, int* step, int64_t* cur_idx, float* cur_scal, int B, int nscal,
                            const float* table, int64_t table_rows, int64_t row_len, float* out, nq_stream_t stream) {
  if (!order || !scal || !step || !cur_idx || !cur_scal || B <= 0 || B > 256 || nscal <= 0 || nscal > 256 || !table || !out ||
      table_rows <= 0 || row_len <= 0)
    return NQ_ERR_INVALID;
  const int64_t total = (int64_t)B * row_len;
  int gb = (int)((total + 4095) / 4096);
  if (gb < 1) gb = 1;
  if (gb > 64) gb = 64;
  hipLaunchKernelGGL(step_prologue_gather_kernel, dim3(1 + gb), dim3(256), 0, nq_s(stream), order, scal, step, cur_idx, cur_scal, B,
                     nscal, table, table_rows, row_len, out);
  return nq_launch_status();
}

static int adam_multi(const nq_adam_seg* segs, int nseg, float step_size, float beta1, float beta2, float eps, float bc2_sqrt,
                      const float* dyn, nq_stream_t stream);

int nq_adaround_adam_multi(const nq_ada_adam_seg* segs, int nseg, float reg_b, float step_size, float beta1, float beta2, float eps,
                           float bc2_sqrt, const float* dyn, nq_stream_t stream) {
  if (!segs || nseg <= 0) return NQ_ERR_INVALID;
  for (int base = 0; base < nseg; base += MAXSEG) {
    AdaAdamMulti t;
    t.nseg = (nseg - base < MAXSEG) ? nseg - base : MAXSEG;
    int blocks = 0;
    for (int k = 0; k < t.nseg; ++k) {
      const nq_ada_adam_seg& h = segs[base + k];
      if (!h.x || !h.gy || !h.alpha || !h.delta || !h.zp || !h.m || !h.v || h.rows <= 0 || h.row_len <= 0 ||
          h.row_len > 0x7fffffffLL)
        return NQ_ERR_INVALID;
      AdaAdamSegD& d = t.s[k];
      d.x = h.x; d.gy = h.gy; d.alpha = h.alpha; d.delta = h.delta; d.zp = h.zp; d.m = h.m; d.v = h.v;
      d.n = h.rows * h.row_len; d.row_len = (int)h.row_len; d.per_row = h.per_row;
      d.qmax = (float)(h.n_levels - 1); d.reg_weight = h.reg_weight;
      d.vec = (((uintptr_t)h.x | (uintptr_t)h.gy | (uintptr_t)h.alpha | (uintptr_t)h.m | (uintptr_t)h.v) & 15) == 0;
      t.blk0[k] = blocks;
      blocks += (int)((d.n + TPB * EPT - 1) / (TPB * EPT));
    }
    t.blk0[t.nseg] = blocks;
    hipLaunchKernelGGL(adaround_adam_multi_kernel, dim3((unsigned)blocks), dim3(TPB), 0, nq_s(stream), t, reg_b, step_size,
                       beta1, beta2, eps, bc2_sqrt, dyn);
  }
  return nq_launch_status();
}

int nq_adam_step_multi(const nq_adam_seg* segs, int nseg, float step_size, float beta1, float beta2, float eps,
                       float bc2_sqrt, nq_stream_t stream) {
  return adam_multi(segs, nseg, step_size, beta1, beta2, eps, bc2_sqrt, nullptr, stream);
}

int nq_adam_step_multi_dyn(const nq_adam_seg* segs, int nseg, const float* dyn, float beta1, float beta2, float eps,
                           nq_stream_t stream) {
  if (!dyn) return NQ_ERR_INVALID;
  return adam_multi(segs, nseg, 0.f, beta1, beta2, eps, 1.f, dyn, stream);
}

static int adam_multi(const nq_adam_seg* segs, int nseg, float step_size, float beta1, float beta2, float eps, float bc2_sqrt,
                      const float* dyn, nq_stream_t stream) {
  if (!segs || nseg <= 0) return NQ_ERR_INVALID;
  for (int base = 0; base < nseg; base += MAXSEG) {
    AdamMulti t;
    t.nseg = (nseg - base < MAXSEG) ? nseg - base : MAXSEG;
    int blocks = 0;
    for (int k = 0; k < t.nseg; ++k) {
      const nq_adam_seg& h = segs[base + k];
      if (!h.p || !h.g || !h.m || !h.v || h.n <= 0) return NQ_ERR_INVALID;
      t.s[k].p = h.p; t.s[k].g = h.g; t.s[k].m = h.m; t.s[k].v = h.v; t.s[k].n = h.n;
      t.s[k].vec = (((uintptr_t)h.p | (uintptr_t)h.g | (uintptr_t)h.m | (uintptr_t)h.v) & 15) == 0;
      t.blk0[k] = blocks;
      blocks += (int)((h.n + TPB * EPT - 1) / (TPB * EPT));
    }
    t.blk0[t.nseg] = blocks;
    hipLaunchKernelGGL(adam_multi_kernel, dim3((unsigned)blocks), dim3(TPB), 0, nq_s(stream), t, step_size, beta1, beta2,
                       eps, bc2_sqrt, dyn);
  }
  return nq_launch_status();
}

}
```

neuroquant_amd/ops.py:

```python
import contextlib
import ctypes
import functools
import math
import os
import threading

import torch
from torch.autograd import Function

from . import _lib as L

_QCACHE = {}


def _q(name, *args):
    key = (name, args, os.environ.get("NQ_WGRAD3_PC"), os.environ.get("NQ_WGRAD3_SS"))
    v = _QCACHE.get(key)
    if v is None:
        v = _QCACHE[key] = getattr(L.lib(), name)(*args)
    return v

EPI_PLAIN, EPI_PS_GELU, EPI_TANH, EPI_PS, EPI_DGRAD_GELU = (L.EPI_PLAIN, L.EPI_PS_GELU, L.EPI_TANH, L.EPI_PS,
                                                                L.EPI_DGRAD_GELU)
EPI_X_SPLIT, EPI_Y_SPLIT = 0x100, 0x200
# ... 135 lines not shown


def adam_step(p, g, m, v, lr, step, beta1=0.9, beta2=0.999, eps=1e-8):
    bc1 = 1 - beta1 ** step
    bc2 = 1 - beta2 ** step
    L.check(L.lib().nq_adam_step(_p(p), _p(_dev(g)), _p(m), _p(v), p.numel(), lr / bc1, beta1, beta2, eps, bc2 ** 0.5,
                                 _stream()), "adam_step")


def adaround_forward_multi(items):
    segs = (L.AdaSeg * len(items))()
    outs = []
    for sg, (x, alpha, delta, zp, n_levels, soft) in zip(segs, items):
        x, alpha, delta, zp = _dev(x), _dev(alpha), _dev(delta), _dev(zp)
        rows, rl, per_row = _rows(x, delta)
        y = torch.empty_like(x)
        outs.append(y)
        sg.x, sg.gy, sg.alpha, sg.delta, sg.zp, sg.out = _p(x), None, _p(alpha), _p(delta), _p(zp), _p(y)
        sg.rows, sg.row_len, sg.per_row, sg.n_levels, sg.soft, sg.reg_weight = rows, rl, per_row, n_levels, int(bool(soft)), 0.0
    L.check(L.lib().nq_adaround_forward_multi(segs, len(items), _stream()), "adaround_forward_multi")
    return outs


def uaq_forward_multi(items):
    segs = (L.AdaSeg * len(items))()
    outs = []
    for sg, (x, delta, zp, n_levels) in zip(segs, items):
        x, delta, zp = _dev(x), _dev(delta), _dev(zp)
        rows, rl, per_row = _rows(x, delta)
        y = torch.empty_like(x)
        outs.append(y)
        sg.x, sg.gy, sg.alpha, sg.delta, sg.zp, sg.out = _p(x), None, None, _p(delta), _p(zp), _p(y)
        sg.rows, sg.row_len, sg.per_row, sg.n_levels, sg.soft, sg.reg_weight = rows, rl, per_row, n_levels, 0, 0.0
    L.check(L.lib().nq_uaq_forward_multi(segs, len(items), _stream()), "uaq_forward_multi")
    return outs


def uaq_backward_multi(items):
    segs = (L.AdaSeg * len(items))()
    outs, keep = [], []
    for sg, (x, gy, delta, zp, n_levels) in zip(segs, items):
        x, gy, delta, zp = _dev(x), _dev(gy), _dev(delta), _dev(zp)
        rows, rl, per_row = _rows(x, delta)
        dd = torch.empty_like(delta)
        outs.append(dd)
        keep.append((x, gy))
        sg.x, sg.gy, sg.alpha, sg.delta, sg.zp, sg.out = _p(x), _p(gy), None, _p(delta), _p(zp), _p(dd)
        sg.rows, sg.row_len, sg.per_row, sg.n_levels, sg.soft, sg.reg_weight = rows, rl, per_row, n_levels, 0, 0.0
    L.check(L.lib().nq_uaq_backward_multi(segs, len(items), _stream()), "uaq_backward_multi")
    return outs


def step_prologue(order_tab, scal_tab, step_ctr, cur_idx, cur_scal):
    L.check(L.lib().nq_step_prologue(_p(order_tab), _p(scal_tab), _p(step_ctr), _p(cur_idx), _p(cur_scal), cur_idx.numel(),
                                     cur_scal.numel(), _stream()), "step_prologue")


def step_prologue_gather(order_tab, scal_tab, step_ctr, cur_idx, cur_scal, table, out):
    table = _dev(table)
    if step_ctr.numel() < 2 or out.shape[0] != cur_idx.numel() or out[0].numel() != table[0].numel() or not out.is_contiguous():
        raise RuntimeError("step_prologue_gather: step_ctr needs two ints, out must be (B,) + table.shape[1:], contiguous")
    L.check(L.lib().nq_step_prologue_gather(_p(order_tab), _p(scal_tab), _p(step_ctr), _p(cur_idx), _p(cur_scal), cur_idx.numel(),
                                            cur_scal.numel(), _p(table), table.shape[0], table[0].numel(), _p(out), _stream()),
            "step_prologue_gather")


def adaround_backward_multi(items, reg_b=0.0, dyn=None):
    segs = (L.AdaSeg * len(items))()
    outs = []
    for sg, (x, gy, alpha, delta, zp, n_levels, reg_weight) in zip(segs, items):
        x, gy, alpha, delta, zp = _dev(x), _dev(gy), _dev(alpha), _dev(delta), _dev(zp)
        rows, rl, per_row = _rows(x, delta)
        da = torch.empty_like(alpha)
        outs.append(da)
        sg.x, sg.gy, sg.alpha, sg.delta, sg.zp, sg.out = _p(x), _p(gy), _p(alpha), _p(delta), _p(zp), _p(da)
        sg.rows, sg.row_len, sg.per_row, sg.n_levels, sg.soft, sg.reg_weight = rows, rl, per_row, n_levels, 1, float(reg_weight)
    if dyn is not None:
        L.check(L.lib().nq_adaround_backward_multi_dyn(segs, len(items), _p(dyn), _stream()), "adaround_backward_multi_dyn")
    else:
        L.check(L.lib().nq_adaround_backward_multi(segs, len(items), float(reg_b), _stream()), "adaround_backward_multi")
    return outs


def adaround_adam_multi(items, opt, reg_b=0.0, dyn=None, beta1=0.9, beta2=0.999, eps=1e-8):
    assert len(items) == len(opt.params)
    opt.t += 1
    segs = (L.AdaAdamSeg * len(items))()
    keep = []
    for i, (sg, (x, gy, alpha, delta, zp, n_levels, reg_weight)) in enumerate(zip(segs, items)):
        x, gy, alpha, delta, zp = _dev(x), _dev(gy), _dev(alpha), _dev(delta), _dev(zp)
        if alpha.data_ptr() != opt.params[i].data_ptr():
            raise RuntimeError("adaround_adam_multi: items must be in the optimiser's parameter order")
        rows, rl, per_row = _rows(x, delta)
        keep.append((x, gy))
        sg.x, sg.gy, sg.alpha, sg.delta, sg.zp, sg.m, sg.v = _p(x), _p(gy), _p(alpha), _p(delta), _p(zp), _p(opt.m[i]), _p(opt.v[i])
        sg.rows, sg.row_len, sg.per_row, sg.n_levels, sg.reg_weight = rows, rl, per_row, n_levels, float(reg_weight)
    step_size, bc2_sqrt = opt.scalars(opt.t, beta1, beta2)
    L.check(L.lib().nq_adaround_adam_multi(segs, len(items), float(reg_b), step_size, beta1, beta2, eps, bc2_sqrt, _p(dyn),
                                           _stream()), "adaround_adam_multi")


class FusedAdam:

    def __init__(self, params, lr):
        self.params = [p for p in params]
        self.lr = lr
        self.t = 0
        self.m = [torch.zeros_like(p) for p in self.params]
        self.v = [torch.zeros_like(p) for p in self.params]

    def zero_grad(self):
        for p in self.params:
            p.grad = None

    def scalars(self, t, beta1=0.9, beta2=0.999):
        return self.lr / (1 - beta1 ** t), (1 - beta2 ** t) ** 0.5

    def step(self, grads=None, beta1=0.9, beta2=0.999, eps=1e-8, dyn=None):
        self.t += 1
        todo = [(p, (p.grad if grads is None else grads[i]), self.m[i], self.v[i]) for i, p in enumerate(self.params)]
        todo = [t for t in todo if t[1] is not None]
        if not todo:
            return
        segs = (L.AdamSeg * len(todo))()
        keep = []
        for sg, (p, g, m, v) in zip(segs, todo):
            g = _dev(g).contiguous()
            keep.append(g)
            sg.p, sg.g, sg.m, sg.v, sg.n = _p(p.data), _p(g), _p(m), _p(v), p.numel()
        if dyn is not None:
            L.check(L.lib().nq_adam_step_multi_dyn(segs, len(todo), _p(dyn), beta1, beta2, eps, _stream()), "adam_step_multi_dyn")
            return
        bc1, bc2 = 1 - beta1 ** self.t, 1 - beta2 ** self.t
        L.check(L.lib().nq_adam_step_multi(segs, len(todo), self.lr / bc1, beta1, beta2, eps, bc2 ** 0.5, _stream()),
                "adam_step_multi")


class _UAQFn(Function):
    @staticmethod
    def forward(ctx, x, delta, zp, n_levels):
        ctx.save_for_backward(x, delta, zp)
        ctx.n_levels = n_levels
        return uaq_forward(x, delta, zp, n_levels)

    @staticmethod
    def backward(ctx, gy):
        x, delta, zp = ctx.saved_tensors
        if ctx.needs_input_grad[0]:
            dd, dx = uaq_backward(x, gy, delta, zp, ctx.n_levels, want_dx=True)
            return dx, dd.view_as(delta), None, None
        return None, uaq_backward(x, gy, delta, zp, ctx.n_levels).view_as(delta), None, None


class _AdaRoundFn(Function):
    @staticmethod
    def forward(ctx, x, alpha, delta, zp, n_levels, soft):
        y, xq = adaround_forward(x, alpha, delta, zp, n_levels, soft, want_xq=True)
        ctx.save_for_backward(x, alpha, delta, zp)
        ctx.n_levels, ctx.soft = n_levels, soft
        ctx.mark_non_differentiable(xq)
        return y, xq

    @staticmethod
    def backward(ctx, gy, _gxq):
        x, alpha, delta, zp = ctx.saved_tensors
        if ctx.needs_input_grad[2] and os.environ.get("NQ_STRICT_GRADS"):
            raise NotImplementedError("d(delta) of the AdaRound fake-quant is not built (never stepped by the reference)")
        da = adaround_backward(x, gy, alpha, delta, zp, ctx.n_levels) if ctx.soft else None
        return None, da, None, None, None, None


class _RoundLossFn(Function):
    @staticmethod
    def forward(ctx, alpha, b, weight):
        ctx.save_for_backward(alpha)
        ctx.b, ctx.weight = float(b), float(weight)
        return round_loss(alpha, b, weight)

    @staticmethod
    def backward(ctx, g):
# ... 208 lines not shown
        y = torch.empty((B, cout, H, W), device=x.device, dtype=torch.float32)
    nws = _q("nq_conv_forward_ws_floats", B, cin, H, W, cout, k)
    ws = torch.empty(nws, device=x.device, dtype=torch.float32) if nws else None
    _timed(("conv_igemm", k, cin, cout, H, W, B, epilogue),
           lambda: L.check(L.lib().nq_conv_forward(_p(x), _p(wt), _p(bias), _p(y), _p(z), _p(ws), B, cin, H, W, cout, k,
                                                   dims[0], dims[1], r, epilogue | fmt, 1 if in_gelu else 0, _p(zprev),
                                                   _stream()), "conv_forward"))
    return y, z


def conv3_supported(B, cin, H, W, cout, k):
    return bool(_q("nq_conv3_supported", B, cin, H, W, cout, k))


def conv3_split_io(B, cin, H, W, cout, k):
    return int(_q("nq_conv3_split_io", B, cin, H, W, cout, k))


def conv_wgrad3_split_io(B, cin, H, W, cout, k):
    return int(_q("nq_conv_wgrad3_split_io", B, cin, H, W, cout, k))


def conv_split_out(B, cin, H, W, cout, k, r, epilogue, has_bias=False):
    return bool(_q("nq_conv_split_out", B, cin, H, W, cout, k, r, epilogue, 0, 1 if has_bias else 0))


def split_words(x):
    x = _dev(x).contiguous()
    y = torch.empty_like(x)
    L.check(L.lib().nq_split_words(_p(x), _p(y), x.numel(), _stream()), "split_words")
    return y


def weight_layout3(w, transposed=False):
    w = _dev(w)
    cw_out, cw_in, k, _ = w.shape
    cin, cout = (cw_out, cw_in) if transposed else (cw_in, cw_out)
    buf = torch.empty(_q("nq_conv3_weight_bytes", cin, cout, k), device=w.device, dtype=torch.uint8)
    L.check(L.lib().nq_weight_layout3(_p(w), _p(buf), cin, cout, k, 1 if transposed else 0, _stream()), "weight_layout3")
    return buf


def weight_layout3_multi(items):
    segs = (L.WL3Seg * len(items))()
    outs = []
    for sg, (w, transposed) in zip(segs, items):
        w = _dev(w)
        cw_out, cw_in, k, _ = w.shape
        cin, cout = (cw_out, cw_in) if transposed else (cw_in, cw_out)
        buf = torch.empty(_q("nq_conv3_weight_bytes", cin, cout, k), device=w.device, dtype=torch.uint8)
        outs.append(buf)
        sg.w, sg.wt3, sg.Cin, sg.Cout, sg.k, sg.transposed = _p(w), _p(buf), cin, cout, k, int(bool(transposed))
    if items:
        L.check(L.lib().nq_weight_layout3_multi(segs, len(items), _stream()), "weight_layout3_multi")
    return outs


def conv3_forward_raw(x, wt3, bias, cout, k, epilogue, r, zprev=None, fmt=0):
    B, cin, H, W = x.shape
    y = z = None
    if epilogue in (EPI_PS_GELU, EPI_PS):
        z = torch.empty((B, cout // (r * r), H * r, W * r), device=x.device, dtype=torch.float32)
        if epilogue == EPI_PS_GELU:
            y = torch.empty_like(z)
    elif epilogue == EPI_DGRAD_GELU:
        y = torch.empty((B, cout * r * r, H // r, W // r), device=x.device, dtype=torch.float32)
    else:
        y = torch.empty((B, cout, H, W), device=x.device, dtype=torch.float32)
    nws = _q("nq_conv_forward3_ws_floats", B, cin, H, W, cout, k)
    ws = torch.empty(nws, device=x.device, dtype=torch.float32) if nws else None
    _timed(("conv_igemm3", k, cin, cout, H, W, B, epilogue),
           lambda: L.check(L.lib().nq_conv_forward3(_p(x), _p(wt3), _p(bias), _p(y), _p(z), _p(zprev), _p(ws), B, cin, H, W,
                                                    cout, k, r, epilogue | fmt, _stream()), "conv_forward3"))
    return y, z


def conv_wgrad3_supported(B, cin, H, W, cout, k):
    return bool(_q("nq_conv_wgrad3_supported", B, cin, H, W, cout, k))


class PendingReductions:

    def __init__(self):
        self.segs, self.keep = [], []

    def add(self, seg, *tensors):
        self.segs.append(seg)
        self.keep.append(tensors)

    def flush(self):
        if self.segs:
            arr = (L.WgrSeg * len(self.segs))(*self.segs)
            L.check(L.lib().nq_wgrad_reduce_multi(arr, len(self.segs), _stream()), "wgrad_reduce_multi")
        self.segs, self.keep = [], []


def conv_wgrad3_raw(x, dy, cout, k, want_db, out=None, defer=None, fmt=0):
    B, cin, H, W = x.shape
    ws = torch.empty(_q("nq_conv_wgrad3_ws_floats", B, cin, H, W, cout, k), device=x.device, dtype=torch.float32)
    dw = torch.empty((cout, cin, k, k), device=x.device, dtype=torch.float32) if out is None else out[0]
    db = (torch.empty(cout, device=x.device, dtype=torch.float32) if out is None else out[1]) if want_db else None
    if defer is not None:
        seg = L.WgrSeg()
        _timed(("conv_wgrad3", k, cin, cout, H, W, B, 0),
               lambda: L.check(L.lib().nq_conv_wgrad3_slabs_fmt(_p(x), _p(dy), _p(dw), _p(db), _p(ws), B, cin, H, W, cout, k,
                                                                ctypes.byref(seg), fmt, _stream()), "conv_wgrad3_slabs"))
        defer.add(seg, ws, dw, db)
        return dw, db
    _timed(("conv_wgrad3", k, cin, cout, H, W, B, 0),
           lambda: L.check(L.lib().nq_conv_wgrad3_fmt(_p(x), _p(dy), _p(dw), _p(db), _p(ws), B, cin, H, W, cout, k, fmt,
                                                      _stream()), "conv_wgrad3"))
    return dw, db


def channel_sum(x):
    x = _dev(x)
    B, C = x.shape[0], x.shape[1]
    out = torch.empty(C, device=x.device, dtype=torch.float32)
    ws = torch.empty(512 * C, device=x.device, dtype=torch.float32)
    L.check(L.lib().nq_channel_sum(_p(x), _p(out), _p(ws), B, C, x.numel() // (B * C), _stream()), "channel_sum")
    return out


def conv_wgrad_swapped3(x, dy, cout, k, want_db, out=None, defer=None):
    B, cin, H, W = x.shape
    ws = torch.empty(_q("nq_conv_wgrad3_ws_floats", B, cout, H, W, cin, k), device=x.device, dtype=torch.float32)
    dw = torch.empty((cout, cin, k, k), device=x.device, dtype=torch.float32) if out is None else out[0]
    if defer is not None:
        seg = L.WgrSeg()
        _timed(("conv_wgrad3", k, cout, cin, H, W, B, 0),
               lambda: L.check(L.lib().nq_conv_wgrad3_swapped_slabs(_p(x), _p(dy), _p(dw), _p(ws), B, cin, H, W, cout, k,
                                                                    ctypes.byref(seg), _stream()), "conv_wgrad3_swapped_slabs"))
        defer.add(seg, ws, dw)
    else:
        _timed(("conv_wgrad3", k, cout, cin, H, W, B, 0),
               lambda: L.check(L.lib().nq_conv_wgrad3_swapped(_p(x), _p(dy), _p(dw), _p(ws), B, cin, H, W, cout, k, _stream()),
                               "conv_wgrad3_swapped"))
    db = None
    if want_db:
        db = channel_sum(dy)
        if out is not None:
            out[1].copy_(db)
            db = out[1]
    return dw, db


def conv_wgrad_raw(x, dy, cout, k, want_db, x_gelu=False, out=None, defer=None):
    B, cin, H, W = x.shape
    ws = torch.empty(_q("nq_conv_wgrad_ws_floats", B, cin, H, W, cout, k), device=x.device, dtype=torch.float32)
    dw = torch.empty((cout, cin, k, k), device=x.device, dtype=torch.float32) if out is None else out[0]
    db = (torch.empty(cout, device=x.device, dtype=torch.float32) if out is None else out[1]) if want_db else None
    if defer is not None:
        seg = L.WgrSeg()
        _timed(("conv_wgrad", k, cin, cout, H, W, B, 0),
               lambda: L.check(L.lib().nq_conv_wgrad_slabs(_p(x), _p(dy), _p(dw), _p(db), _p(ws), B, cin, H, W, cout, k,
                                                           1 if x_gelu else 0, ctypes.byref(seg), _stream()), "conv_wgrad_slabs"))
        defer.add(seg, ws, dw, db)
        return dw, db
    _timed(("conv_wgrad", k, cin, cout, H, W, B, 0),
           lambda: L.check(L.lib().nq_conv_wgrad(_p(x), _p(dy), _p(dw), _p(db), _p(ws), B, cin, H, W, cout, k,
                                                 1 if x_gelu else 0, _stream()), "conv_wgrad"))
    return dw, db


class _ConvFn(Function):

    @staticmethod
    def forward(ctx, x, w, b, epilogue, r):
        x, w = _dev(x, "x"), _dev(w, "weight")
        b = _dev(b, "bias") if b is not None else None
        cout, cin, k, k2 = w.shape
        if k != k2 or x.shape[1] != cin:
            raise ValueError(f"conv shape mismatch: x {tuple(x.shape)} w {tuple(w.shape)}")
        need_dx = ctx.needs_input_grad[0]
        wt, dims, wb, dims_b = weight_layouts(w, need_dx)
        y, z = conv_forward_raw(x, wt, dims, b, cout, k, epilogue, r)
        ctx.save_for_backward(x, wb, z if epilogue == EPI_PS_GELU else (y if epilogue == EPI_TANH else None))
        ctx.meta = (cout, cin, k, epilogue, r, dims_b, b is not None)
        return y

    @staticmethod
    def backward(ctx, gy):
        x, wb, aux = ctx.saved_tensors
        cout, cin, k, epilogue, r, dims_b, has_b = ctx.meta
        B, _, H, W = x.shape
        gy = _dev(gy, "grad")
        if epilogue == EPI_PS_GELU:
            dconv = torch.empty((B, cout, H, W), device=x.device, dtype=torch.float32)
            L.check(L.lib().nq_ps_gelu_backward(_p(gy), _p(aux), _p(dconv), B, cout // (r * r), H, W, r, _stream()),
                    "ps_gelu_backward")
        elif epilogue == EPI_TANH:
            dconv = torch.empty_like(gy)
            L.check(L.lib().nq_tanh_out_backward(_p(gy), _p(aux), _p(dconv), gy.numel(), _stream()), "tanh_backward")
        else:
            dconv = gy
        dx = dw = db = None
        if ctx.needs_input_grad[0]:
            dx, _ = conv_forward_raw(dconv, wb, dims_b, None, cin, k, EPI_PLAIN, 1)
        if ctx.needs_input_grad[1] or (has_b and ctx.needs_input_grad[2]):
            dw, db = conv_wgrad_raw(x, dconv, cout, k, has_b)
        return dx, dw, db, None, None


_PRECISION = None


def set_conv_precision(precision):
    global _PRECISION
    if precision not in (None, "fp32", "bf16x3"):
        raise ValueError(f"unknown conv precision {precision!r}")
    _PRECISION = precision


def get_conv_precision():
    return _PRECISION or os.environ.get("NQ_CONV_PRECISION", "bf16x3")


def _use3(precision):
    return (precision or get_conv_precision()) == "bf16x3"


def _conv_plain(x, w, precision=None):
    cout, cin, k, _ = w.shape
    B, _, H, W = x.shape
    if _use3(precision) and conv3_supported(B, cin, H, W, cout, k):
        return conv3_forward_raw(x, weight_layout3(w), None, cout, k, EPI_PLAIN, 1)[0]
    wt, dims, _, _ = weight_layouts(w, need_bwd=False)
    return conv_forward_raw(x, wt, dims, None, cout, k, EPI_PLAIN, 1)[0]


def _dgrad_plain(gy, w, precision=None):
    cout, cin, k, _ = w.shape
    B, _, H, W = gy.shape
    if _use3(precision) and conv3_supported(B, cout, H, W, cin, k):
        return conv3_forward_raw(gy, weight_layout3(w, transposed=True), None, cin, k, EPI_PLAIN, 1)[0]
    _, _, wb, dims_b = weight_layouts(w, need_bwd=True)
    return conv_forward_raw(gy, wb, dims_b, None, cin, k, EPI_PLAIN, 1)[0]


def _wgrad_plain(x, gy, k, precision=None):
    B, cin, H, W = x.shape
    cout = gy.shape[1]
    if _use3(precision) and conv_wgrad3_supported(B, cin, H, W, cout, k):
        return conv_wgrad3_raw(x, gy, cout, k, False)[0]
    if _use3(precision) and cout <= 4 and cin > 4 and cout * k * k <= 64 and conv_wgrad3_supported(B, cout, H, W, cin, k):
        return conv_wgrad_swapped3(x, gy, cout, k, False)[0]
    return conv_wgrad_raw(x, gy, cout, k, False)[0]
# ... 187 lines not shown
            x = _space_from_channels(x, *spec.fc_hw)
        if r > 1:
            x = pixel_shuffle_dd(x, r)
        if act:
            x = gelu_dd(x)
    return tanh_out_dd(x) if spec.tanh_out else x


def conv2d_fused(x, w, b, epilogue=EPI_PLAIN, r=1):
    if not torch.is_grad_enabled() or not (x.requires_grad or w.requires_grad or (b is not None and b.requires_grad)):
        x, w = _dev(x, "x"), _dev(w, "weight")
        b = _dev(b, "bias") if b is not None else None
        cout, cin, k, k2 = w.shape
        if k != k2 or x.shape[1] != cin:
            raise ValueError(f"conv shape mismatch: x {tuple(x.shape)} w {tuple(w.shape)}")
        B, _, H, W = x.shape
        if _use3(None) and conv3_supported(B, cin, H, W, cout, k):
            return conv3_forward_raw(x, weight_layout3(w), b, cout, k, epilogue, r)[0]
        wt, dims, _, _ = weight_layouts(w, False)
        return conv_forward_raw(x, wt, dims, b, cout, k, epilogue, r)[0]
    return _ConvFn.apply(x, w, b, epilogue, r)


class DecoderSpec:

    def __init__(self, layers, fc_hw=(1, 1), tanh_out=True, precision=None):
        self.layers = [tuple(l) for l in layers]
        self.fc_hw = tuple(fc_hw)
        self.tanh_out = tanh_out
        self.precision = precision or get_conv_precision()
        if self.precision not in ("fp32", "bf16x3"):
            raise ValueError(f"unknown conv precision {self.precision!r}")
        self.overlap_wgrad = os.environ.get("NQ_WGRAD_STREAM", "0") == "1"


def _space_from_channels(x, fh, fw):
    n, c, h, w = x.shape
    return x.view(n, -1, fh, fw, h, w).permute(0, 1, 4, 2, 5, 3).reshape(n, -1, fh * h, fw * w)


def _channels_from_space(g, fh, fw):
    n, c, hh, ww = g.shape
    return g.view(n, c, hh // fh, fh, ww // fw, fw).permute(0, 1, 3, 5, 2, 4).reshape(n, c * fh * fw, hh // fh, ww // fw)


_ARENA_TLS = threading.local()


def _arena_state():
    return getattr(_ARENA_TLS, "state", (None, False))


def set_grad_arena_hook(fn, two_phase=False):
    _ARENA_TLS.state = (fn, bool(two_phase) and fn is not None)


@contextlib.contextmanager
def grad_arena_hook(fn, two_phase=False):
    prev = _arena_state()
    set_grad_arena_hook(fn, two_phase)
    try:
        yield
    finally:
        _ARENA_TLS.state = prev


def arena_reduced(img):
    return bool(getattr(getattr(img, "grad_fn", None), "nq_arena_reduced", False))


_LOSS_TLS = threading.local()


@contextlib.contextmanager
def fused_head_loss(tgt=None, cache_u8=None, idx=None):
    prev = getattr(_LOSS_TLS, "req", None)
    _LOSS_TLS.req = None if os.environ.get("NQ_FUSED_HEAD_LOSS", "1") == "0" else (tgt, cache_u8, idx)
    try:
        yield
    finally:
        _LOSS_TLS.req = prev


def head_forward_loss_raw(x, wt, dims, bias, cout, k, tgt=None, cache_u8=None, idx=None):
    B, cin, H, W = x.shape
    if cout != 3 or k != 3 or (W & 3) or (dims[1] & 3) or os.environ.get("NQ_HEAD_FWD") == "1":
        return None
    if cache_u8 is not None:
        if not cache_u8.is_cuda or cache_u8.dtype != torch.uint8 or not cache_u8.is_contiguous() \
                or tuple(cache_u8.shape[1:]) != (cout, H, W) or idx is None or idx.numel() != B:
            return None
        idx = idx.to(device=x.device, dtype=torch.int64).contiguous()
        tgt = None
    elif tgt is not None:
        if not tgt.is_cuda or tgt.dtype != torch.float32 or tuple(tgt.shape) != (B, cout, H, W):
            return None
        tgt = tgt.contiguous()
    else:
        return None
    y = torch.empty((B, cout, H, W), device=x.device, dtype=torch.float32)
    dconv = torch.empty_like(y)
    loss = torch.empty((), device=x.device, dtype=torch.float32)
    db = torch.empty(cout, device=x.device, dtype=torch.float32)
    ws = torch.empty(_q("nq_head_forward_loss_ws_floats", B, H, W), device=x.device, dtype=torch.float32)
    rc = _timed(("conv_igemm", k, cin, cout, H, W, B, EPI_TANH),
                lambda: L.lib().nq_head_forward_loss(_p(x), _p(wt), dims[1], _p(bias), _p(y), _p(tgt), _p(cache_u8), _p(idx), _p(loss),
                                                     _p(dconv), _p(db), _p(ws), B, cin, H, W, B * H * W, 1.0, _stream()))
    if rc == -2:
        return None
    L.check(rc, "head_forward_loss")
    return y, loss, dconv, db


_SIDE_STREAMS = {}


def _side_stream(device):
    key = torch.device(device).index
    if key not in _SIDE_STREAMS:
        _SIDE_STREAMS[key] = torch.cuda.Stream(device=device)
    return _SIDE_STREAMS[key]


class _DecoderStackFn(Function):

    @staticmethod
    def forward(ctx, emb, spec, *wb):
        x = _dev(emb, "embedding")
        n = len(spec.layers)
        saved_in, saved_z, metas = [], [], []
        in_gelu = False
        zprev = None
        Bx, Hx, Wx = x.shape[0], x.shape[2], x.shape[3]
        plan, items = [], []
        fio, bio, wio = [0] * n, [0] * n, [0] * n
        for l, (k, r, act) in enumerate(spec.layers):
            W = _dev(wb[2 * l], "weight")
            cout, cin = W.shape[0], W.shape[1]
            use3 = spec.precision == "bf16x3" and conv3_supported(Bx, cin, Hx, Wx, cout, k)
            use3_bwd = spec.precision == "bf16x3" and l > 0 and conv3_supported(Bx, cout, Hx, Wx, cin, k)
            plan.append((use3, use3_bwd, len(items) if use3 else -1, len(items) + int(use3) if use3_bwd else -1))
            if use3:
                items.append((W, False))
                fio[l] = conv3_split_io(Bx, cin, Hx, Wx, cout, k)
            if use3_bwd:
                items.append((W, True))
                bio[l] = conv3_split_io(Bx, cout, Hx, Wx, cin, k)
            if spec.precision == "bf16x3" and conv_wgrad3_supported(Bx, cin, Hx, Wx, cout, k):
                wio[l] = conv_wgrad3_split_io(Bx, cin, Hx, Wx, cout, k)
            if l == n - 1 and l > 0 and not use3_bwd:
                kp, rp, actp = spec.layers[l - 1]
                if actp and conv_split_out(Bx, cout, Hx, Wx, cin, k, rp, EPI_DGRAD_GELU):
                    bio[l] = EPI_Y_SPLIT
            if l == 0:
                Hx, Wx = Hx * spec.fc_hw[0], Wx * spec.fc_hw[1]
            Hx, Wx = Hx * r, Wx * r
        split_on = spec.precision == "bf16x3" and os.environ.get("NQ_SPLIT_IO", "1") != "0"
        xsp, gsp = [False] * n, [False] * n
        if split_on:
            for l in range(2, n):
                xsp[l] = bool(spec.layers[l - 1][2] and (fio[l - 1] & EPI_Y_SPLIT) and (fio[l] & EPI_X_SPLIT) and (wio[l] & 1))
            for l in range(1, n - 1):
                gsp[l] = bool((bio[l + 1] & EPI_Y_SPLIT) and (bio[l] & EPI_X_SPLIT) and (wio[l] & 2) and spec.layers[l - 1][2]
                              and not (l == 1 and spec.fc_hw != (1, 1)))
        need_bs = [(l > 0 and not plan[l][1]) or (l == 0 and ctx.needs_input_grad[0]) for l in range(n)]
        fp32_items = [(_dev(wb[2 * l], "weight"), not plan[l][0], need_bs[l]) for l in range(n)
                      if (not plan[l][0]) or need_bs[l]]
        operands, fp32_list = weight_layouts_all(items, fp32_items)
        fp32_ops = iter(fp32_list)
        for l, (k, r, act) in enumerate(spec.layers):
            W = _dev(wb[2 * l], "weight")
            b = _dev(wb[2 * l + 1], "bias") if wb[2 * l + 1] is not None else None
            cout, cin = W.shape[0], W.shape[1]
            use3, use3_bwd, i_f, i_b = plan[l]
            need_b = need_bs[l]
            wt = dims = wbk = dims_b = None
            if use3:
                wt3 = operands[i_f]
            if (not use3) or need_b:
                wt, dims, wbk, dims_b = next(fp32_ops)
                if not need_b:
                    wbk = dims_b = None
            last = l == n - 1
            if last:
                epi = EPI_TANH if spec.tanh_out else EPI_PLAIN
            elif act:
                epi = EPI_PS_GELU
            elif r > 1:
                epi = EPI_PS
            else:
                epi = EPI_PLAIN
            fused_loss = None
            if last and epi == EPI_TANH and not use3 and getattr(_LOSS_TLS, "req", None) is not None:
                tgt_, cache_, idx_ = _LOSS_TLS.req
                fused_loss = head_forward_loss_raw(x, wt, dims, b, cout, k, tgt_, cache_, idx_)
            if fused_loss is not None:
                y, z = fused_loss[0], None
            elif use3:
                y, z = conv3_forward_raw(x, wt3, b, cout, k, epi, r,
                                         fmt=(EPI_X_SPLIT if xsp[l] else 0) | (EPI_Y_SPLIT if l + 1 < n and xsp[l + 1] else 0))
            else:
                y, z = conv_forward_raw(x, wt, dims, b, cout, k, epi, r, in_gelu=in_gelu)
            saved_in.append(x)
            saved_z.append(zprev)
            metas.append((k, r, act, cout, cin, in_gelu, wbk, dims_b, b is not None, operands[i_b] if use3_bwd else None,
                          xsp[l], gsp[l]))
            if epi == EPI_PS_GELU:
                x, zprev, in_gelu = y, z, False
            elif epi == EPI_PS:
                x, zprev, in_gelu = z, None, False
            else:
                x, zprev, in_gelu = y, None, False
            if l == 0 and spec.fc_hw != (1, 1):
                x = _space_from_channels(x, *spec.fc_hw).contiguous()
        ctx.spec, ctx.metas, ctx.n = spec, metas, n
        ctx.save_for_backward(x, *saved_in, *saved_z)
        ctx.nq_arena, ctx.nq_arena_reduced = _arena_state(), False
        ctx.nq_head = _HeadHandoff() if spec.tanh_out else None
        if fused_loss is not None:
            ctx.nq_head.loss, ctx.nq_head.dconv, ctx.nq_head.db = fused_loss[1], fused_loss[2], fused_loss[3]
            ctx.nq_head.version = fused_loss[2]._version
        return x

    @staticmethod
    def backward(ctx, g_img):
        hook = ctx.nq_arena[0]
        steps = _decoder_backward_steps(ctx, g_img)
        while True:
            try:
                part, last = next(steps)
            except StopIteration as done:
                return done.value
            if last is None:
                hook(part)
            else:
                hook(part, last)


def _decoder_backward_steps(ctx, g_img):
    spec, metas, n = ctx.spec, ctx.metas, ctx.n
    saved = ctx.saved_tensors
    img, xs, zs = saved[0], saved[1:1 + n], saved[1 + n:]
    d_emb = None
    g = _dev(g_img, "grad")
    head_db = None
    head = ctx.nq_head
    if head is not None and head.loss is not None:
        head.dconv = head.db = head.loss = None
    if head is not None and head.dconv is not None:
        if head.dconv.data_ptr() != g.data_ptr() or g.shape != head.dconv.shape:
            raise RuntimeError("neuroquant_amd: the gradient returned by ops.l2_loss_head_grad must be passed to "
                               "backward() as it is (it already contains the tanh backward of this decoder)")
        dconv = g
        head_db = head.db if g._version == head.version else None
        head.dconv = head.db = None
    elif spec.tanh_out:
        dconv = torch.empty_like(g)
        L.check(L.lib().nq_tanh_out_backward(_p(g), _p(img), _p(dconv), g.numel(), _stream()), "tanh_backward")
    else:
        dconv = g
    grads = [None] * (2 * n)
    main = torch.cuda.current_stream()
    side = _side_stream(g.device) if spec.overlap_wgrad else None
    keep = []

    arena = views = None
    arena_hook, arena_two_phase = ctx.nq_arena
    if arena_hook is not None:
        sizes = []
        for l in range(n):
            k, r, act, cout, cin = metas[l][:5]
            sizes += [cout * cin * k * k, cout if metas[l][8] else 0]
        arena = torch.empty(sum(sizes), device=g.device, dtype=torch.float32)
        views, off = [], 0
        for l in range(n):
            k, r, act, cout, cin = metas[l][:5]
            wv = arena[off:off + sizes[2 * l]].view(cout, cin, k, k)
            off += sizes[2 * l]
            bv = arena[off:off + sizes[2 * l + 1]] if sizes[2 * l + 1] else None
            off += sizes[2 * l + 1]
            views.append((wv, bv))

    pending = PendingReductions() if side is None and os.environ.get("NQ_DEFER_REDUCE", "1") != "0" else None

    def wgrad(l, dconv):
        k, r, act, cout, cin, in_gelu, wbk, dims_b, has_b, W3, x_split, g_split = metas[l]
        x_in = xs[l]
        Bx, _, Hx, Wx = x_in.shape
        out = views[l] if views is not None else None
        if spec.precision == "bf16x3" and not in_gelu and conv_wgrad3_supported(Bx, cin, Hx, Wx, cout, k):
            return conv_wgrad3_raw(x_in, dconv, cout, k, has_b, out=out, defer=pending,
                                   fmt=(1 if x_split else 0) | (2 if g_split else 0))
        if spec.precision == "bf16x3" and not in_gelu and cout <= 4 and cin > 4 and cout * k * k <= 64 \
                and conv_wgrad3_supported(Bx, cout, Hx, Wx, cin, k):
            if l == n - 1 and has_b and head_db is not None:
                dw, _ = conv_wgrad_swapped3(x_in, dconv, cout, k, False, out=out, defer=pending)
                if out is not None:
                    out[1].copy_(head_db)
                    return dw, out[1]
                return dw, head_db
            return conv_wgrad_swapped3(x_in, dconv, cout, k, has_b, out=out, defer=pending)
        return conv_wgrad_raw(x_in, dconv, cout, k, has_b, x_gelu=in_gelu, out=out, defer=pending)

    def dgrad(l, dconv):
        k, r, act, cout, cin, in_gelu, wbk, dims_b, has_b, W3, x_split, g_split = metas[l]
        kp, rp, actp = spec.layers[l - 1]
        epi_b, r_b, zp = (EPI_DGRAD_GELU, rp, zs[l]) if actp else (EPI_PLAIN, 1, None)
        if not actp and rp != 1:
            raise NotImplementedError("PixelShuffle without activation between decoder layers")
        out_split = EPI_Y_SPLIT if metas[l - 1][11] else 0
        if W3 is not None:
            d, _ = conv3_forward_raw(dconv, W3, None, cin, k, epi_b, r_b, zprev=zp, fmt=(EPI_X_SPLIT if g_split else 0) | out_split)
        else:
            d, _ = conv_forward_raw(dconv, wbk, dims_b, None, cin, k, epi_b, r_b, zprev=zp, fmt=out_split)
        if not actp and l == 1 and spec.fc_hw != (1, 1):
            d = _channels_from_space(d, *spec.fc_hw).contiguous()
        return d

    def emb_grad(dconv):
        k, r, act, cout, cin, in_gelu, wbk, dims_b, has_b, W3 = metas[0][:10]
        return conv_forward_raw(dconv, wbk, dims_b, None, cin, k, EPI_PLAIN, 1)[0]

    if arena is not None and arena_two_phase and n > 1:
        dcs = [None] * n
        dcs[n - 1] = dconv
        for l in range(n - 1, 0, -1):
            dcs[l - 1] = dgrad(l, dcs[l])
        if ctx.needs_input_grad[0]:
            d_emb = emb_grad(dcs[0])
        flops = [metas[l][3] * metas[l][4] * metas[l][0] ** 2 * xs[l].shape[2] * xs[l].shape[3] for l in range(n)]
        split, late = n - 1, flops[n - 1]
        while split > 1 and late < 0.8 * sum(flops):
            split -= 1
            late += flops[split]
        for l in range(split):
            grads[2 * l], grads[2 * l + 1] = wgrad(l, dcs[l])
            dcs[l] = None
        off = sum(sizes[:2 * split])
        if pending is not None:
            pending.flush()
        yield arena[:off], False
        for l in range(split, n):
            grads[2 * l], grads[2 * l + 1] = wgrad(l, dcs[l])
            dcs[l] = None
        if pending is not None:
            pending.flush()
        yield arena[off:], True
        ctx.nq_arena_reduced = True
        return (d_emb, None) + tuple(grads)

    for l in range(n - 1, -1, -1):
        if side is not None:
            keep.append(dconv)
            side.wait_stream(main)
            with torch.cuda.stream(side):
                dw, db = wgrad(l, dconv)
            for t in (dw, db):
                if t is not None:
                    t.record_stream(main)
        else:
            dw, db = wgrad(l, dconv)
        grads[2 * l], grads[2 * l + 1] = dw, db
        if l == 0:
            if ctx.needs_input_grad[0]:
                d_emb = emb_grad(dconv)
            break
        dconv = dgrad(l, dconv)
    if side is not None:
        main.wait_stream(side)
        keep.clear()
    if pending is not None:
        pending.flush()
    if arena is not None:
        yield arena, None
        ctx.nq_arena_reduced = True
    return (d_emb, None) + tuple(grads)




class _ManualNode:

    def __init__(self, n_inputs, want_emb_grad=False):
        self.needs_input_grad = (bool(want_emb_grad), False) + (True,) * n_inputs
        self.saved_tensors = ()

    def save_for_backward(self, *tensors):
        self.saved_tensors = tensors


def decoder_forward_manual(emb, spec: DecoderSpec, weights, two_phase=True):
    flat = []
    for W, b in weights:
        flat += [W, b]
    node = _ManualNode(len(flat))
    with torch.no_grad():
        img = _DecoderStackFn.forward(node, emb, spec, *flat)
    node.nq_arena = ("manual", bool(two_phase))
    return img, node


def decoder_backward_steps(node, g_img):
    return _decoder_backward_steps(node, g_img)


def decoder_stack(emb, spec: DecoderSpec, weights):
    flat = []
    for W, b in weights:
        flat += [W, b]
    return _DecoderStackFn.apply(emb, spec, *flat)


class _L2LossFn(Function):

    @staticmethod
    def forward(ctx, pred, tgt):
        pred, tgt = _dev(pred, "pred"), _dev(tgt, "tgt")
        n = pred.numel()
        mean_count = n // pred.shape[1]
        loss = torch.empty((), device=pred.device, dtype=torch.float32)
        dpred = torch.empty_like(pred) if ctx.needs_input_grad[0] else None
        ws = torch.empty(_q("nq_reduce_ws_floats", n), device=pred.device, dtype=torch.float32)
        L.check(L.lib().nq_l2_loss(_p(pred), _p(tgt), _p(loss), _p(dpred), _p(ws), n, mean_count, 1.0, _stream()), "l2_loss")
        ctx.save_for_backward(dpred)
        return loss

    @staticmethod
    def backward(ctx, g):
        (dpred,) = ctx.saved_tensors
        return dpred * g, None


def l2_loss(pred, tgt):
    return _L2LossFn.apply(pred, tgt)


def l2_loss_and_grad(pred, tgt):
    pred_d, tgt = _dev(pred.detach(), "pred"), _dev(tgt, "tgt")
    n = pred_d.numel()
    loss = torch.empty((), device=pred_d.device, dtype=torch.float32)
    dpred = torch.empty_like(pred_d)
    ws = torch.empty(_q("nq_reduce_ws_floats", n), device=pred_d.device, dtype=torch.float32)
    L.check(L.lib().nq_l2_loss(_p(pred_d), _p(tgt), _p(loss), _p(dpred), _p(ws), n, n // pred_d.shape[1], 1.0, _stream()),
            "l2_loss")
    return loss, dpred


class _HeadHandoff:
    __slots__ = ("dconv", "db", "version", "loss")

    def __init__(self):
        self.dconv = self.db = self.version = self.loss = None


def l2_loss_tanh_head_raw(pred, tgt=None, cache_u8=None, idx=None):
# ... 73 lines not shown
```

neuroquant_amd/quantization/calib_model.py:

```python
import contextlib
import logging
import os

import torch
import torch.nn as nn

from .. import ops
from ..utils import allreduce_mean_
from .data_utils import LinearTempDecay
from .quant_layer import QuantModule
from .quant_model import QuantModel
from .quantizer import AdaRoundQuantizer, lp_loss


def _quant_modules(module: nn.Module, out=None):
    out = [] if out is None else out
    for name, child in module.named_children():
        if 'encoder' in name:
            continue
        if isinstance(child, QuantModule):
            out.append(child)
        else:
            _quant_modules(child, out)
    return out
# ... 158 lines not shown
    fused_stack = None
    if dp_graph:
        from ..models._decode import _fused_stack
        fused_stack = _fused_stack(model.model) if hasattr(model, 'model') else None
        if fused_stack is None:
            dp_graph = use_graph = False

    def _capture_staged(run_body):
        graphs, parts = [torch.cuda.CUDAGraph()], []
        pool = torch.cuda.graph_pool_handle()
        cap = torch.cuda.Stream()
        cap.wait_stream(torch.cuda.current_stream())
        torch.cuda.synchronize()
        with torch.cuda.stream(cap):
            graphs[0].capture_begin(pool=pool, capture_error_mode="thread_local")

            def cut(k, part):
                graphs[-1].capture_end()
                parts.append(part)
                graphs.append(torch.cuda.CUDAGraph())
                graphs[-1].capture_begin(pool=pool, capture_error_mode="thread_local")

            run_body(cut)
            graphs[-1].capture_end()
        torch.cuda.current_stream().wait_stream(cap)
        return graphs, parts

    def _replay_staged(staged_graph):
        import torch.distributed as dist
        graphs, parts = staged_graph
        works = []
        for g, part in zip(graphs[:-1], parts):
            g.replay()
            works.append(_mean_all_reduce(part))
        for fin in works:
            fin()
        graphs[-1].replay()

    fuse_had = bool(hadamard) and os.environ.get("NQ_FUSED_FWHT", "1") != "0" and \
        all(ops.fq_fwht_fusable(L.n, L.src.shape[2] * L.src.shape[3]) for L in layers)

    def run(epochs, params, opt_lr, max_count, ada):
        nonlocal done
        opt = ops.FusedAdam(params, lr=opt_lr)
        loss_start = max_count * warmup
        temp = LinearTempDecay(max_count, rel_start_decay=warmup, start_b=b_range[0], end_b=b_range[1])
        count = 0

        def sched(c):
            b = temp(c)
            reg_on = ada and not (c < loss_start)
            return (b if reg_on else 0), reg_on

        def body(get_batch, b, reg_on, dyn, want_log, staged=None):
            img, inputs = get_batch()
            if ada and fuse_had:
                items = []
                for L in layers:
                    (xw, aw, dw_, zw, nlw, sw), (xb, ab, db_, zb, nlb, sb) = L.ada_items()
                    items += [(xw, aw, dw_, zw, nlw, sw, L.n, L.c_in), (xb, ab, db_, zb, nlb, sb, 0, 0)]
                fq = ops.adaround_fwht_multi(items)
                for i, L in enumerate(layers):
                    L._finish(fq[2 * i], fq[2 * i + 1], transformed=True)
            elif ada:
                fq = ops.adaround_forward_multi(
                    [it for L in layers for it in L.ada_items()])
                if hadamard:
                    had = ops.fwht_channels_multi([(fq[2 * i], L.n, L.c_in) for i, L in enumerate(layers)])
                    for i, L in enumerate(layers):
                        L._finish(had[i], fq[2 * i + 1], transformed=True)
                else:
                    for i, L in enumerate(layers):
                        L._finish(fq[2 * i], fq[2 * i + 1])
            else:
                fq = ops.uaq_forward_multi([it for L in layers for it in L.uaq_items()])
                if hadamard:
                    had = ops.fwht_channels_multi([(fq[2 * i], L.n, L.c_in) for i, L in enumerate(layers)])
                    for i, L in enumerate(layers):
                        L._finish(had[i], fq[2 * i + 1], transformed=True)
                else:
                    for i, L in enumerate(layers):
                        L._finish(fq[2 * i], fq[2 * i + 1])
            node = None
            loss_req = ops.fused_head_loss(cache_u8=img[0], idx=img[1]) if isinstance(img, tuple) else ops.fused_head_loss(tgt=img)
            with loss_req:
                if staged is None:
                    img_out, _, _ = model(inputs)
                else:
                    spec, provs = fused_stack
                    img_out, node = ops.decoder_forward_manual(inputs, spec, [p() for p in provs],
                                                               two_phase=os.environ.get("NQ_DP_OVERLAP", "1") != "0")
            fused = ops.l2_loss_head_grad(img_out, cache_u8=img[0], idx=img[1], node=node) if isinstance(img, tuple) \
                else ops.l2_loss_head_grad(img_out, tgt=img, node=node)
            if fused is None:
                if isinstance(img, tuple):
                    img = ops.gather_frames_u8(img[0], img[1])
                fused = ops.l2_loss_and_grad(img_out, img)
            rec, dimg = fused
            if staged is None:
                img_out.backward(dimg)
            else:
                steps, k = ops.decoder_backward_steps(node, dimg), 0
                while True:
                    try:
                        part, _last = next(steps)
                    except StopIteration as fin:
                        res = fin.value
                        break
                    staged(k, part)
                    k += 1
                for i, L in enumerate(layers):
                    L.W.grad, L.b.grad = res[2 + 2 * i], res[3 + 2 * i]
            if dp and staged is None and not ops.arena_reduced(img_out):
                allreduce_mean_([t.grad for L in layers for t in (L.W, L.b)])
            if want_log:
                rl = torch.zeros((), device=device)
                if reg_on:
                    for L in layers:
                        ops.round_loss(L.m.weight_quantizer.alpha.data, b, weight, out=rl, accumulate=True)
                total, rl_f = float(rec) + float(rl), float(rl)
                if recorder is not None:
                    recorder.append((total, rl_f, float(b), count))
                if count % 500 == 0:
                    logging.info('Total loss:\t{:.4f} (rec:{:.4f}, round:{:.4f})\tb={:.2f}\tcount={}'.format(
                        total, float(rec), rl_f, b, count))
            grads = []
            if ada and fuse_had and probe is None and os.environ.get("NQ_FUSED_ADAM", "1") != "0":
                items = []
                for L in layers:
                    wq, bq = L.m.weight_quantizer, L.m.bias_quantizer
                    items.append((L.src, L.W.grad, wq.alpha.data, wq.delta.data, wq.zero_point, wq.n_levels,
                                  weight if (reg_on or dyn is not None) else 0.0, L.n, L.c_in))
                    items.append((L.bias, L.b.grad, bq.alpha.data, bq.delta.data, bq.zero_point, bq.n_levels, 0.0, 0, 0))
                ops.fwht_adaround_adam_multi(items, opt, b, dyn=dyn)
                grads = None
            elif ada:
                items = []
                gWs = ops.fwht_channels_multi([(L.W.grad, L.n, L.n) for L in layers]) if hadamard else None
                for i, L in enumerate(layers):
                    gW, gb = (gWs[i], L.b.grad) if hadamard else L.grads()
                    wq, bq = L.m.weight_quantizer, L.m.bias_quantizer
                    items.append((L.src, gW, wq.alpha.data, wq.delta.data, wq.zero_point, wq.n_levels,
                                  weight if (reg_on or dyn is not None) else 0.0))
                    items.append((L.bias, gb, bq.alpha.data, bq.delta.data, bq.zero_point, bq.n_levels, 0.0))
                if probe is None and os.environ.get("NQ_FUSED_ADAM", "1") != "0":
                    ops.adaround_adam_multi(items, opt, b, dyn=dyn)
                    grads = None
                else:
                    grads = ops.adaround_backward_multi(items, b, dyn=dyn)
            else:
                gWs = ops.fwht_channels_multi([(L.W.grad, L.n, L.n) for L in layers]) if hadamard else None
                items = []
                for i, L in enumerate(layers):
                    gW, gb = (gWs[i], L.b.grad) if hadamard else L.grads()
                    wq, bq = L.m.weight_quantizer, L.m.bias_quantizer
                    items.append((L.src, gW, wq.delta.data, wq.zero_point, wq.n_levels))
                    items.append((L.bias, gb, bq.delta.data, bq.zero_point, bq.n_levels))
                grads = ops.uaq_backward_multi(items)
            if probe is not None:
                probe('ada' if ada else 'uaq', layers, grads)
            if grads is not None:
                opt.step(grads, dyn=dyn)
            for L in layers:
                L.release()

        if not use_graph:
            for _ in range(epochs):
                model.train()
                for sample in gt:
                    if step_hook is not None:
                        step_hook(done)
                    if max_steps is not None and done >= max_steps:
                        return
                    count += 1
                    b, reg_on = sched(count)
                    img = sample['img'].to(device, non_blocking=True)
                    inputs = cali_data[sample['idx'].to(device, non_blocking=True)]
                    body(lambda: (img, inputs), b, reg_on, None, recorder is not None or count % 500 == 0)
                    done += 1
            return

        st = None
        graph, warm = None, 0
        for _ in range(epochs):
            model.train()
            idx_tab = gt.epoch_indices()
            nb, per = idx_tab.shape
            if st is None or st['order'].shape[0] < nb or st['cur_idx'].numel() != per:
                st = dict(order=torch.zeros((nb, per), device=device, dtype=torch.int64),
                          scal=torch.zeros((nb, 4), device=device, dtype=torch.float32),
                          step=torch.zeros(2, device=device, dtype=torch.int32),
                          emb=torch.zeros((per,) + tuple(cali_data.shape[1:]), device=device, dtype=torch.float32),
                          cur_idx=torch.zeros(per, device=device, dtype=torch.int64),
                          cur_scal=torch.zeros(4, device=device, dtype=torch.float32))
                graph, warm = None, 0
            rows = []
            for c in range(count + 1, count + nb + 1):
                b, reg_on = sched(c)
                rows.append((float(b), 1.0 if reg_on else 0.0) + opt.scalars(opt.t + (c - count)))
            st['scal'][:nb].copy_(torch.tensor(rows, dtype=torch.float32), non_blocking=True)
            st['order'][:nb].copy_(idx_tab)
            st['step'].zero_()

            def static_batch():
                ops.step_prologue_gather(st['order'], st['scal'], st['step'], st['cur_idx'], st['cur_scal'], cali_data, st['emb'])
                return (gt.cache.frames, st['cur_idx']), st['emb']

            for i in range(nb):
                if step_hook is not None:
                    step_hook(done)
                if max_steps is not None and done >= max_steps:
                    return
                count += 1
                b, reg_on = sched(count)
                want_log = count % 500 == 0
                if want_log or warm < 3 or ops.profiling_active():
                    body(static_batch, b, reg_on, st['cur_scal'], want_log)
                    warm += 1
                elif graph is None and dp_graph:
                    graph = _capture_staged(lambda cut: body(static_batch, b, reg_on, st['cur_scal'], False, staged=cut))
                    _replay_staged(graph)
                elif graph is None:
                    graph = torch.cuda.CUDAGraph()
                    with torch.cuda.graph(graph):
                        body(static_batch, b, reg_on, st['cur_scal'], False)
                    graph.replay()
                elif dp_graph:
                    _replay_staged(graph)
                    opt.t += 1
# ... 29 lines not shown
```

Baseline: 496.1 it/s (B=2 frames per iteration-equivalent, summed over GPUs).

## Defer wgrad reductions, tiny wgrads and head loss tail into fused Adam kernel

Adds a step-tail mechanism that postpones the head loss stage-2 reduction, the split-K wgrad slab reductions and tiny pointwise wgrad computations, then runs them inside one combined reduce+AdaRound+Adam kernel at the end of the step. This targets the cost of several small kernel launches and the round trips through intermediate gradient buffers per iteration. In exchange it adds cross-stage bookkeeping and keeps buffers alive longer. It also risks ordering bugs when the loss is read before it has been finished.

New measurement: 498.4 it/s (B=2 frames per iteration-equivalent, summed over GPUs), median of 6. No clear change (+0.5%).

```diff
diff --git a/include/nq_hip.h b/include/nq_hip.h
--- a/include/nq_hip.h
+++ b/include/nq_hip.h
@@ -219,6 +219,34 @@
                          const uint8_t* cache_u8, const int64_t* idx, float* loss, float* dconv, float* db, float* ws, int B,
                          int Cin, int H, int W, int64_t mean_count, float gscale, nq_stream_t stream);
 
+typedef struct nq_head_tail {
+  const float* ws;
+  float* loss;
+  float* db;
+  int waves;
+  float scale;
+} nq_head_tail;
+NQ_API int nq_head_forward_loss_deferred(const float* x, const float* wt, int ld, const float* bias, float* y, const float* tgt,
+                                  const uint8_t* cache_u8, const int64_t* idx, float* loss, float* dconv, float* db, float* ws,
+                                  int B, int Cin, int H, int W, int64_t mean_count, float gscale, nq_head_tail* tail,
+                                  nq_stream_t stream);
+NQ_API int nq_head_loss_finish(const nq_head_tail* tail, nq_stream_t stream);
+
+typedef struct nq_tiny_wg_seg {
+  const float* x;
+  const float* dy;
+  float* dw;
+  float* db;
+  int B, Cin, HW, Cout;
+} nq_tiny_wg_seg;
+NQ_API int nq_tiny_pw_wgrad_describe(const float* x, const float* dy, float* dw, float* db, int B, int Cin, int H, int W, int Cout,
+                              int k, nq_tiny_wg_seg* seg);
+NQ_API int nq_tiny_pw_wgrad_multi(const nq_tiny_wg_seg* segs, int nseg, nq_stream_t stream);
+
+NQ_API int nq_reduce_adaround_adam_multi(const nq_ada_adam_seg* segs, int nseg, const nq_wgr_seg* reds, int nred,
+                                  const nq_tiny_wg_seg* tiny, int ntiny, const nq_head_tail* tail, float reg_b, float step_size,
+                                  float beta1, float beta2, float eps, float bc2_sqrt, const float* dyn, nq_stream_t stream);
+
 NQ_API int nq_frame_sse(const float* out, const float* gt, float* sse, int64_t frames, int64_t frame_len, nq_stream_t stream);
 
 NQ_API int64_t nq_ms_ssim_ws_floats(int64_t frames, int C, int H, int W);
diff --git a/neuroquant_amd/_lib.py b/neuroquant_amd/_lib.py
--- a/neuroquant_amd/_lib.py
+++ b/neuroquant_amd/_lib.py
@@ -43,6 +43,15 @@
 class WgrSeg(Structure):
     _fields_ = [("slab", c_void_p), ("slab_db", c_void_p), ("dw", c_void_p), ("db", c_void_p), ("Cout", c_int), ("N", c_int),
                 ("co_pad", c_int), ("n_pad", c_int), ("nsplit", c_int), ("swap_kk", c_int), ("sg", c_int)]
+
+
+class TinyWgSeg(Structure):
+    _fields_ = [("x", c_void_p), ("dy", c_void_p), ("dw", c_void_p), ("db", c_void_p), ("B", c_int), ("Cin", c_int),
+                ("HW", c_int), ("Cout", c_int)]
+
+
+class HeadTail(Structure):
+    _fields_ = [("ws", c_void_p), ("loss", c_void_p), ("db", c_void_p), ("waves", c_int), ("scale", c_float)]
 
 
 class FqFwhtSeg(Structure):
@@ -139,6 +148,12 @@
     sig("nq_fwht_adaround_adam_multi", I, POINTER(FqFwhtSeg), I, F, F, F, F, F, F, P, P)
     sig("nq_head_forward_loss_ws_floats", L, I, I, I)
     sig("nq_head_forward_loss", I, P, P, I, P, P, P, P, P, P, P, P, P, I, I, I, I, L, F, P)
+    sig("nq_head_forward_loss_deferred", I, P, P, I, P, P, P, P, P, P, P, P, P, I, I, I, I, L, F, POINTER(HeadTail), P)
+    sig("nq_head_loss_finish", I, POINTER(HeadTail), P)
+    sig("nq_reduce_adaround_adam_multi", I, POINTER(AdaAdamSeg), I, POINTER(WgrSeg), I, POINTER(TinyWgSeg), I, POINTER(HeadTail),
+        F, F, F, F, F, F, P, P)
+    sig("nq_tiny_pw_wgrad_describe", I, P, P, P, P, I, I, I, I, I, I, POINTER(TinyWgSeg))
+    sig("nq_tiny_pw_wgrad_multi", I, POINTER(TinyWgSeg), I, P)
     sig("nq_act_dd", I, P, P, P, P, L, I, P)
     sig("nq_pixel_shuffle", I, P, P, I, I, I, I, I, I, P)
     sig("nq_bias_add", I, P, P, P, I, I, L, P)
@@ -157,6 +172,8 @@
     "nq_act_dd", "nq_pixel_shuffle", "nq_bias_add", "nq_conv3_split_io", "nq_conv_split_out", "nq_split_words",
     "nq_conv_wgrad3_split_io", "nq_conv_wgrad3_fmt", "nq_conv_wgrad3_slabs_fmt", "nq_head_forward_loss_ws_floats", "nq_head_forward_loss",
     "nq_adaround_fwht_multi", "nq_fwht_adaround_adam_multi", "nq_weight_layouts_all",
+    "nq_head_forward_loss_deferred", "nq_head_loss_finish", "nq_reduce_adaround_adam_multi",
+    "nq_tiny_pw_wgrad_describe", "nq_tiny_pw_wgrad_multi",
 )
 
 _lib = None
diff --git a/neuroquant_amd/csrc/conv3.hip b/neuroquant_amd/csrc/conv3.hip
--- a/neuroquant_amd/csrc/conv3.hip
+++ b/neuroquant_amd/csrc/conv3.hip
@@ -1,6 +1,7 @@
 #include <cstdlib>
 #include "nq_common.h"
 #include "conv3_layout.h"
+#include "wgrad_reduce.h"
 
 extern "C" {
 int nq_conv_igemm3_k3(const float*, const void*, const float*, float*, float*, const float*, int, int, int, int, int, int, int,
@@ -342,39 +343,12 @@
   int k = 0;
   while (k + 1 < t.nseg && (int)blockIdx.x >= t.blk0[k + 1]) ++k;
   const nq_wgr_seg& q = t.s[k];
-  const int SG = q.sg, OG = 256 / SG;
-  const int o = threadIdx.x % OG, g = threadIdx.x / OG;
-  const int N = q.N, Cout = q.Cout, nsplit = q.nsplit;
-  const int NQ = (N + 3) >> 2;
-  const int64_t i = (int64_t)((int)blockIdx.x - t.blk0[k]) * OG + o;
-  const int64_t total = (int64_t)Cout * NQ;
-  float4 s = make_float4(0.f, 0.f, 0.f, 0.f);
-  int co = 0, n = 0;
-  if (i < total) {
-    co = (int)(i / NQ);
-    n = 4 * (int)(i - (int64_t)co * NQ);
-    const float* p = q.slab + (int64_t)co * q.n_pad + n;
-    const int64_t stride = (int64_t)q.co_pad * q.n_pad;
-#pragma unroll 8
-    for (int j = g; j < nsplit; j += SG) {
-      const float4 v = *reinterpret_cast<const float4*>(p + j * stride);
-      s.x += v.x; s.y += v.y; s.z += v.z; s.w += v.w;
-    }
-  } else if (q.db && i < total + Cout) {
-    const int cb = (int)(i - total);
-#pragma unroll 8
-    for (int j = g; j < nsplit; j += SG) s.x += q.slab_db[(int64_t)j * q.co_pad + cb];
-  }
-  if (SG > 1) {
-    part[g * OG + o] = s;
-    __syncthreads();
-    if (g != 0) return;
-    s = part[o];
-    for (int j = 1; j < SG; ++j) {
-      const float4 v = part[j * OG + o];
-      s.x += v.x; s.y += v.y; s.z += v.z; s.w += v.w;
-    }
-  }
+  const int N = q.N, Cout = q.Cout;
+  const int64_t total = (int64_t)Cout * ((N + 3) >> 2);
+  float4 s;
+  int64_t i;
+  int co, n;
+  if (!nq_wgr_sum(q, (int)blockIdx.x - t.blk0[k], part, s, i, co, n)) return;
   if (i < total) {
     const float sv[4] = {s.x, s.y, s.z, s.w};
     if (q.swap_kk > 0) {
diff --git a/neuroquant_amd/csrc/conv_head.hip b/neuroquant_amd/csrc/conv_head.hip
--- a/neuroquant_amd/csrc/conv_head.hip
+++ b/neuroquant_amd/csrc/conv_head.hip
@@ -321,9 +321,7 @@
 __global__ __launch_bounds__(256) void head_loss_stage2(const float* __restrict__ ws, int waves, float scale,
                                                         float* __restrict__ loss, float* __restrict__ db) {
   __shared__ float red[16];
-  float acc = 0.f;
-  for (int i = threadIdx.x; i < waves; i += 256) acc += ws[(int64_t)i * 4 + blockIdx.x];
-  const float s = nq_block_sum(acc, red);
+  const float s = nq_head_tail_sum(ws, waves, (int)blockIdx.x, red);
   if (threadIdx.x == 0) {
     if (blockIdx.x == 0) loss[0] = 0.f + s * scale;
     else db[blockIdx.x - 1] = s;
@@ -638,9 +636,9 @@
   return (int64_t)B * ((W + 255) / 256) * ((H + 3) / 4) * 4;
 }
 
-int nq_head_forward_loss(const float* x, const float* wt, int ld, const float* bias, float* y, const float* tgt,
-                         const uint8_t* cache_u8, const int64_t* idx, float* loss, float* dconv, float* db, float* ws, int B,
-                         int Cin, int H, int W, int64_t mean_count, float gscale, nq_stream_t stream) {
+static int head_forward_loss(const float* x, const float* wt, int ld, const float* bias, float* y, const float* tgt,
+                             const uint8_t* cache_u8, const int64_t* idx, float* loss, float* dconv, float* db, float* ws, int B,
+                             int Cin, int H, int W, int64_t mean_count, float gscale, nq_head_tail* tail, nq_stream_t stream) {
   if (!x || !wt || !y || !loss || !dconv || !db || !ws || B <= 0 || Cin <= 0 || H <= 0 || W <= 0 || mean_count <= 0) return NQ_ERR_INVALID;
   if ((tgt == nullptr) == (cache_u8 == nullptr) || (cache_u8 && !idx)) return NQ_ERR_INVALID;
   if ((W & 3) != 0 || (ld & 3) != 0 || (int64_t)B * Cin * H * W * 4 >= 0xFFFFFF00ll) return NQ_ERR_UNSUPPORTED;
@@ -656,7 +654,34 @@
   const int waves = B * a.strips * a.rblocks;
   hipStream_t st = nq_s(stream);
   hipLaunchKernelGGL((head_fwd2_kernel<R, 3, true, true>), dim3((unsigned)((waves + 3) / 4)), dim3(256), 0, st, x, wt, bias, y, a, la);
+  if (tail) {
+    *tail = nq_head_tail{ws, loss, db, waves, (float)(1.0 / (double)mean_count)};
+    return nq_launch_status();
+  }
   hipLaunchKernelGGL(head_loss_stage2, dim3(4), dim3(256), 0, st, ws, waves, (float)(1.0 / (double)mean_count), loss, db);
+  return nq_launch_status();
+}
+
+int nq_head_forward_loss(const float* x, const float* wt, int ld, const float* bias, float* y, const float* tgt,
+                         const uint8_t* cache_u8, const int64_t* idx, float* loss, float* dconv, float* db, float* ws, int B,
+                         int Cin, int H, int W, int64_t mean_count, float gscale, nq_stream_t stream) {
+  return head_forward_loss(x, wt, ld, bias, y, tgt, cache_u8, idx, loss, dconv, db, ws, B, Cin, H, W, mean_count, gscale, nullptr,
+                           stream);
+}
+
+int nq_head_forward_loss_deferred(const float* x, const float* wt, int ld, const float* bias, float* y, const float* tgt,
+                                  const uint8_t* cache_u8, const int64_t* idx, float* loss, float* dconv, float* db, float* ws,
+                                  int B, int Cin, int H, int W, int64_t mean_count, float gscale, nq_head_tail* tail,
+                                  nq_stream_t stream) {
+  if (!tail) return NQ_ERR_INVALID;
+  return head_forward_loss(x, wt, ld, bias, y, tgt, cache_u8, idx, loss, dconv, db, ws, B, Cin, H, W, mean_count, gscale, tail,
+                           stream);
+}
+
+int nq_head_loss_finish(const nq_head_tail* tail, nq_stream_t stream) {
+  if (!tail || !tail->ws || !tail->loss || !tail->db || tail->waves <= 0) return NQ_ERR_INVALID;
+  hipLaunchKernelGGL(head_loss_stage2, dim3(4), dim3(256), 0, nq_s(stream), tail->ws, tail->waves, tail->scale, tail->loss,
+                     tail->db);
   return nq_launch_status();
 }
 
diff --git a/neuroquant_amd/csrc/conv_tiny.hip b/neuroquant_amd/csrc/conv_tiny.hip
--- a/neuroquant_amd/csrc/conv_tiny.hip
+++ b/neuroquant_amd/csrc/conv_tiny.hip
@@ -1,4 +1,5 @@
 #include "nq_common.h"
+#include "tiny_wgrad.h"
 
 namespace {
 
@@ -63,33 +64,24 @@
                                                             int HW, int Cout) {
   const int64_t t = (int64_t)blockIdx.x * 256 + threadIdx.x;
   const int64_t nw = (int64_t)Cout * Cin;
-  if (t < nw) {
-    const int co = (int)(t / Cin), ci = (int)(t - (int64_t)co * Cin);
-    float acc = 0.f;
-    for (int b = 0; b < B; ++b) {
-      const float* __restrict__ dp = dy + ((int64_t)b * Cout + co) * HW;
-      const float* __restrict__ xp = x + ((int64_t)b * Cin + ci) * HW;
-      if ((HW & 7) == 0) {
-        for (int p = 0; p < HW; p += 8) {
-          const float4 d0 = *reinterpret_cast<const float4*>(dp + p), d1 = *reinterpret_cast<const float4*>(dp + p + 4);
-          const float4 x0 = *reinterpret_cast<const float4*>(xp + p), x1 = *reinterpret_cast<const float4*>(xp + p + 4);
-          acc = fmaf(d0.x, x0.x, acc); acc = fmaf(d0.y, x0.y, acc); acc = fmaf(d0.z, x0.z, acc); acc = fmaf(d0.w, x0.w, acc);
-          acc = fmaf(d1.x, x1.x, acc); acc = fmaf(d1.y, x1.y, acc); acc = fmaf(d1.z, x1.z, acc); acc = fmaf(d1.w, x1.w, acc);
-        }
-      } else {
-        for (int p = 0; p < HW; ++p) acc = fmaf(dp[p], xp[p], acc);
-      }
-    }
-    dw[t] = acc;
-  } else if (db && t < nw + Cout) {
-    const int co = (int)(t - nw);
-    float acc = 0.f;
-    for (int b = 0; b < B; ++b) {
-      const float* __restrict__ dp = dy + ((int64_t)b * Cout + co) * HW;
-      for (int p = 0; p < HW; ++p) acc += dp[p];
-    }
-    db[co] = acc;
-  }
+  if (t < nw) dw[t] = nq_tiny_pw_wgrad_elem(x, dy, B, Cin, HW, Cout, t);
+  else if (db && t < nw + Cout) db[t - nw] = nq_tiny_pw_wgrad_elem(x, dy, B, Cin, HW, Cout, t);
+}
+
+constexpr int TWG_MAXSEG = 8;
+struct TinyWgMulti {
+  nq_tiny_wg_seg s[TWG_MAXSEG];
+  int blk0[TWG_MAXSEG + 1];
+  int nseg;
+};
+__global__ __launch_bounds__(256) void tiny_pw_wgrad_multi_kernel(TinyWgMulti m) {
+  int k = 0;
+  while (k + 1 < m.nseg && (int)blockIdx.x >= m.blk0[k + 1]) ++k;
+  const nq_tiny_wg_seg& g = m.s[k];
+  const int64_t t = (int64_t)((int)blockIdx.x - m.blk0[k]) * 256 + threadIdx.x;
+  const int64_t nw = (int64_t)g.Cout * g.Cin;
+  if (t < nw) g.dw[t] = nq_tiny_pw_wgrad_elem(g.x, g.dy, g.B, g.Cin, g.HW, g.Cout, t);
+  else if (g.db && t < nw + g.Cout) g.db[t - nw] = nq_tiny_pw_wgrad_elem(g.x, g.dy, g.B, g.Cin, g.HW, g.Cout, t);
 }
 
 }
@@ -126,4 +118,30 @@
   return nq_launch_status();
 }
 
+int nq_tiny_pw_wgrad_describe(const float* x, const float* dy, float* dw, float* db, int B, int Cin, int H, int W, int Cout, int k,
+                              nq_tiny_wg_seg* seg) {
+  if (!x || !dy || !dw || !seg || B <= 0 || Cin <= 0 || H <= 0 || W <= 0 || Cout <= 0) return NQ_ERR_INVALID;
+  if (!nq_tiny_pw_supported(B, Cin, H, W, Cout, k)) return NQ_ERR_UNSUPPORTED;
+  *seg = nq_tiny_wg_seg{x, dy, dw, db, B, Cin, H * W, Cout};
+  return NQ_OK;
 }
+
+int nq_tiny_pw_wgrad_multi(const nq_tiny_wg_seg* segs, int nseg, nq_stream_t stream) {
+  if (!segs || nseg <= 0) return NQ_ERR_INVALID;
+  for (int base = 0; base < nseg; base += TWG_MAXSEG) {
+    TinyWgMulti m;
+    m.nseg = (nseg - base < TWG_MAXSEG) ? nseg - base : TWG_MAXSEG;
+    int blocks = 0;
+    for (int k = 0; k < m.nseg; ++k) {
+      if (!nq_tiny_wg_valid(segs[base + k])) return NQ_ERR_INVALID;
+      m.s[k] = segs[base + k];
+      m.blk0[k] = blocks;
+      blocks += nq_tiny_wg_blocks(m.s[k]);
+    }
+    m.blk0[m.nseg] = blocks;
+    hipLaunchKernelGGL(tiny_pw_wgrad_multi_kernel, dim3((unsigned)blocks), dim3(256), 0, nq_s(stream), m);
+  }
+  return nq_launch_status();
+}
+
+}
diff --git a/neuroquant_amd/csrc/nq_common.h b/neuroquant_amd/csrc/nq_common.h
--- a/neuroquant_amd/csrc/nq_common.h
+++ b/neuroquant_amd/csrc/nq_common.h
@@ -103,4 +103,9 @@
   float s = nq_block_sum(acc, red);
   if (threadIdx.x == 0) out[0] = (accumulate ? out[0] : 0.f) + s * scale;
 }
+__device__ __forceinline__ float nq_head_tail_sum(const float* __restrict__ ws, int waves, int c, float* red ) {
+  float acc = 0.f;
+  for (int i = threadIdx.x; i < waves; i += 256) acc += ws[(int64_t)i * 4 + c];
+  return nq_block_sum(acc, red);
+}
 #define NQ_RED_CHUNK 4096
diff --git a/neuroquant_amd/csrc/quant.hip b/neuroquant_amd/csrc/quant.hip
--- a/neuroquant_amd/csrc/quant.hip
+++ b/neuroquant_amd/csrc/quant.hip
@@ -1,5 +1,7 @@
 #include "nq_common.h"
 #include "quant_elem.h"
+#include "wgrad_reduce.h"
+#include "tiny_wgrad.h"
 
 namespace {
 
@@ -344,29 +346,36 @@
   int blk0[MAXSEG + 1];
   int nseg;
 };
-__global__ __launch_bounds__(TPB) void adaround_adam_multi_kernel(AdaAdamMulti t, float reg_b, float step_size, float beta1,
-                                                                  float beta2, float eps, float bc2_sqrt,
-                                                                  const float* __restrict__ dyn) {
-  float gate = 1.f;
+struct AdamScal {
+  float reg_b, gate, step_size, beta1, beta2, eps, bc2_sqrt;
+  int dyn;
+};
+__device__ __forceinline__ AdamScal adam_scal(float reg_b, float step_size, float beta1, float beta2, float eps, float bc2_sqrt,
+                                              const float* __restrict__ dyn) {
+  AdamScal c{reg_b, 1.f, step_size, beta1, beta2, eps, bc2_sqrt, dyn != nullptr};
   if (dyn) {
-    reg_b = dyn[0];
-    gate = dyn[1];
-    step_size = dyn[2];
-    bc2_sqrt = dyn[3];
-  }
-  const int k = find_seg(t, blockIdx.x);
-  const AdaAdamSegD& sg = t.s[k];
-  const int64_t i0 = (int64_t)(blockIdx.x - t.blk0[k]) * (TPB * EPT) + 4 * threadIdx.x;
-  if (i0 >= sg.n) return;
-  const bool vec = sg.vec && (i0 + 3 < sg.n);
-  float xv[4], av[4], gv[4], mv[4], vv[4];
+    c.reg_b = dyn[0];
+    c.gate = dyn[1];
+    c.step_size = dyn[2];
+    c.bc2_sqrt = dyn[3];
+  }
+  return c;
+}
+__device__ __forceinline__ void ada_adam_elem(float x, float gy, float& a, float& m, float& v, float d, float z, float qmax,
+                                              float rw, const AdamScal& c) {
+  const float g = ada_bwd_elem(x, gy, a, d, z, qmax, rw, c.reg_b);
+  m = m + (1.f - c.beta1) * (g - m);
+  v = v * c.beta2 + (1.f - c.beta2) * (g * g);
+  const float denom = sqrtf(v) / c.bc2_sqrt + c.eps;
+  a = a - c.step_size * (m / denom);
+}
+__device__ __forceinline__ void ada_adam_quad(const AdaAdamSegD& sg, int64_t i0, bool vec, const float gv[4], const AdamScal& c) {
+  float xv[4], av[4], mv[4], vv[4];
   if (vec) {
     const float4 x4 = *reinterpret_cast<const float4*>(sg.x + i0), a4 = *reinterpret_cast<const float4*>(sg.alpha + i0);
-    const float4 g4 = *reinterpret_cast<const float4*>(sg.gy + i0);
     const float4 m4 = *reinterpret_cast<const float4*>(sg.m + i0), v4 = *reinterpret_cast<const float4*>(sg.v + i0);
     xv[0] = x4.x; xv[1] = x4.y; xv[2] = x4.z; xv[3] = x4.w;
     av[0] = a4.x; av[1] = a4.y; av[2] = a4.z; av[3] = a4.w;
-    gv[0] = g4.x; gv[1] = g4.y; gv[2] = g4.z; gv[3] = g4.w;
     mv[0] = m4.x; mv[1] = m4.y; mv[2] = m4.z; mv[3] = m4.w;
     vv[0] = v4.x; vv[1] = v4.y; vv[2] = v4.z; vv[3] = v4.w;
   } else {
@@ -375,24 +384,19 @@
       const bool in = i0 + j < sg.n;
       xv[j] = in ? sg.x[i0 + j] : 0.f;
       av[j] = in ? sg.alpha[i0 + j] : 0.f;
-      gv[j] = in ? sg.gy[i0 + j] : 0.f;
       mv[j] = in ? sg.m[i0 + j] : 0.f;
       vv[j] = in ? sg.v[i0 + j] : 0.f;
     }
   }
   const int64_t row0 = sg.per_row ? i0 / sg.row_len : 0;
   const int rem0 = sg.per_row ? (int)(i0 - row0 * sg.row_len) : 0;
-  const float rw = dyn ? sg.reg_weight * gate : sg.reg_weight;
+  const float rw = c.dyn ? sg.reg_weight * c.gate : sg.reg_weight;
 #pragma unroll
   for (int j = 0; j < 4; ++j) {
     int64_t row = 0;
     if (sg.per_row) row = (sg.row_len >= 4) ? row0 + ((rem0 + j >= sg.row_len) ? 1 : 0) : (i0 + j) / sg.row_len;
     if (i0 + j >= sg.n) row = 0;
-    const float g = ada_bwd_elem(xv[j], gv[j], av[j], sg.delta[row], sg.zp[row], sg.qmax, rw, reg_b);
-    mv[j] = mv[j] + (1.f - beta1) * (g - mv[j]);
-    vv[j] = vv[j] * beta2 + (1.f - beta2) * (g * g);
-    const float denom = sqrtf(vv[j]) / bc2_sqrt + eps;
-    av[j] = av[j] - step_size * (mv[j] / denom);
+    ada_adam_elem(xv[j], gv[j], av[j], mv[j], vv[j], sg.delta[row], sg.zp[row], sg.qmax, rw, c);
   }
   if (vec) {
     *reinterpret_cast<float4*>(sg.m + i0) = make_float4(mv[0], mv[1], mv[2], mv[3]);
@@ -406,6 +410,116 @@
         sg.v[i0 + j] = vv[j];
         sg.alpha[i0 + j] = av[j];
       }
+  }
+}
+__device__ __forceinline__ void ada_adam_one(const AdaAdamSegD& sg, int64_t i, float g, const AdamScal& c) {
+  const int64_t row = sg.per_row ? i / sg.row_len : 0;
+  float a = sg.alpha[i], m = sg.m[i], v = sg.v[i];
+  ada_adam_elem(sg.x[i], g, a, m, v, sg.delta[row], sg.zp[row], sg.qmax, c.dyn ? sg.reg_weight * c.gate : sg.reg_weight, c);
+  sg.m[i] = m;
+  sg.v[i] = v;
+  sg.alpha[i] = a;
+}
+__device__ __forceinline__ void ada_adam_block(const AdaAdamSegD& sg, int blk, const AdamScal& c) {
+  const int64_t i0 = (int64_t)blk * (TPB * EPT) + 4 * threadIdx.x;
+  if (i0 >= sg.n) return;
+  const bool vec = sg.vec && (i0 + 3 < sg.n);
+  float gv[4];
+  if (vec) {
+    const float4 g4 = *reinterpret_cast<const float4*>(sg.gy + i0);
+    gv[0] = g4.x; gv[1] = g4.y; gv[2] = g4.z; gv[3] = g4.w;
+  } else {
+#pragma unroll
+    for (int j = 0; j < 4; ++j) gv[j] = (i0 + j < sg.n) ? sg.gy[i0 + j] : 0.f;
+  }
+  ada_adam_quad(sg, i0, vec, gv, c);
+}
+__global__ __launch_bounds__(TPB) void adaround_adam_multi_kernel(AdaAdamMulti t, float reg_b, float step_size, float beta1,
+                                                                  float beta2, float eps, float bc2_sqrt,
+                                                                  const float* __restrict__ dyn) {
+  const AdamScal c = adam_scal(reg_b, step_size, beta1, beta2, eps, bc2_sqrt, dyn);
+  const int k = find_seg(t, blockIdx.x);
+  ada_adam_block(t.s[k], (int)blockIdx.x - t.blk0[k], c);
+}
+
+constexpr int MAXRED = 8, MAXTINY = 4;
+struct RedAdamMulti {
+  AdaAdamSegD s[MAXSEG];
+  nq_wgr_seg r[MAXRED];
+  int rw[MAXRED], rb[MAXRED];
+  int rblk0[MAXRED + 1];
+  int pseg[MAXSEG], pblk0[MAXSEG + 1];
+  nq_tiny_wg_seg tw[MAXTINY];
+  int tww[MAXTINY], twb[MAXTINY], tblk0[MAXTINY + 1];
+  int nred, ntw, np;
+  nq_head_tail tail;
+  int tail_b;
+};
+__global__ __launch_bounds__(TPB) void reduce_adaround_adam_kernel(RedAdamMulti t, float reg_b, float step_size, float beta1,
+                                                                   float beta2, float eps, float bc2_sqrt,
+                                                                   const float* __restrict__ dyn) {
+  __shared__ float4 part[256];
+  const AdamScal c = adam_scal(reg_b, step_size, beta1, beta2, eps, bc2_sqrt, dyn);
+  int blk = (int)blockIdx.x;
+  if (blk < t.rblk0[t.nred]) {
+    int k = 0;
+    while (k + 1 < t.nred && blk >= t.rblk0[k + 1]) ++k;
+    const nq_wgr_seg& q = t.r[k];
+    const int N = q.N, Cout = q.Cout;
+    const int64_t total = (int64_t)Cout * ((N + 3) >> 2);
+    float4 s;
+    int64_t i;
+    int co, n;
+    if (!nq_wgr_sum(q, blk - t.rblk0[k], part, s, i, co, n)) return;
+    if (i < total) {
+      const AdaAdamSegD& sg = t.s[t.rw[k]];
+      const float sv[4] = {s.x, s.y, s.z, s.w};
+      if (q.swap_kk > 0) {
+#pragma unroll
+        for (int e = 0; e < 4; ++e) {
+          if (n + e >= N) break;
+          const int ci = (n + e) / q.swap_kk, tap = (n + e) - ci * q.swap_kk;
+          ada_adam_one(sg, ((int64_t)ci * Cout + co) * q.swap_kk + (q.swap_kk - 1 - tap), sv[e], c);
+        }
+      } else if ((N & 3) == 0) {
+        ada_adam_quad(sg, (int64_t)co * N + n, sg.vec != 0, sv, c);
+      } else {
+#pragma unroll
+        for (int e = 0; e < 4; ++e)
+          if (n + e < N) ada_adam_one(sg, (int64_t)co * N + n + e, sv[e], c);
+      }
+    } else if (q.db && i < total + Cout) {
+      ada_adam_one(t.s[t.rb[k]], i - total, s.x, c);
+    }
+    return;
+  }
+  blk -= t.rblk0[t.nred];
+  if (blk < t.tblk0[t.ntw]) {
+    int k = 0;
+    while (k + 1 < t.ntw && blk >= t.tblk0[k + 1]) ++k;
+    const nq_tiny_wg_seg& g = t.tw[k];
+    const int64_t i = (int64_t)(blk - t.tblk0[k]) * 256 + threadIdx.x;
+    const int64_t nw = (int64_t)g.Cout * g.Cin;
+    if (i < nw) ada_adam_one(t.s[t.tww[k]], i, nq_tiny_pw_wgrad_elem(g.x, g.dy, g.B, g.Cin, g.HW, g.Cout, i), c);
+    else if (g.db && i < nw + g.Cout) ada_adam_one(t.s[t.twb[k]], i - nw, nq_tiny_pw_wgrad_elem(g.x, g.dy, g.B, g.Cin, g.HW, g.Cout, i), c);
+    return;
+  }
+  blk -= t.tblk0[t.ntw];
+  if (blk < t.pblk0[t.np]) {
+    int k = 0;
+    while (k + 1 < t.np && blk >= t.pblk0[k + 1]) ++k;
+    ada_adam_block(t.s[t.pseg[k]], blk - t.pblk0[k], c);
+    return;
+  }
+  blk -= t.pblk0[t.np];
+  const float s = nq_head_tail_sum(t.tail.ws, t.tail.waves, blk, reinterpret_cast<float*>(part));
+  if (threadIdx.x == 0) {
+    if (blk == 0) {
+      t.tail.loss[0] = 0.f + s * t.tail.scale;
+    } else {
+      t.tail.db[blk - 1] = s;
+      if (t.tail_b >= 0) ada_adam_one(t.s[t.tail_b], blk - 1, s, c);
+    }
   }
 }
 
@@ -732,6 +846,95 @@
   return nq_launch_status();
 }
 
+int nq_reduce_adaround_adam_multi(const nq_ada_adam_seg* segs, int nseg, const nq_wgr_seg* reds, int nred, const nq_tiny_wg_seg* tiny,
+                                  int ntiny, const nq_head_tail* tail, float reg_b, float step_size, float beta1, float beta2,
+                                  float eps, float bc2_sqrt, const float* dyn, nq_stream_t stream) {
+  if (!segs || nseg <= 0 || nred < 0 || (nred > 0 && !reds) || ntiny < 0 || (ntiny > 0 && !tiny)) return NQ_ERR_INVALID;
+  if (ntiny > MAXTINY) return NQ_ERR_UNSUPPORTED;
+  if (nseg > MAXSEG) return NQ_ERR_UNSUPPORTED;
+  RedAdamMulti t;
+  bool fed[MAXSEG];
+  for (int k = 0; k < nseg; ++k) {
+    const nq_ada_adam_seg& h = segs[k];
+    if (!h.x || !h.gy || !h.alpha || !h.delta || !h.zp || !h.m || !h.v || h.rows <= 0 || h.row_len <= 0 || h.row_len > 0x7fffffffLL)
+      return NQ_ERR_INVALID;
+    AdaAdamSegD& d = t.s[k];
+    d.x = h.x; d.gy = h.gy; d.alpha = h.alpha; d.delta = h.delta; d.zp = h.zp; d.m = h.m; d.v = h.v;
+    d.n = h.rows * h.row_len; d.row_len = (int)h.row_len; d.per_row = h.per_row;
+    d.qmax = (float)(h.n_levels - 1); d.reg_weight = h.reg_weight;
+    d.vec = (((uintptr_t)h.x | (uintptr_t)h.alpha | (uintptr_t)h.m | (uintptr_t)h.v) & 15) == 0;
+    fed[k] = false;
+  }
+  auto consumer = [&](const float* g, int64_t n) {
+    for (int k = 0; k < nseg; ++k)
+      if (segs[k].gy == g && !fed[k] && t.s[k].n == n) return k;
+    return -1;
+  };
+  t.nred = 0;
+  int blocks = 0;
+  for (int i = 0; i < nred; ++i) {
+    const nq_wgr_seg& h = reds[i];
+    if (h.nsplit == 0) continue;
+    if (!nq_wgr_valid(h)) return NQ_ERR_INVALID;
+    if (t.nred == MAXRED) return NQ_ERR_UNSUPPORTED;
+    const int kw = consumer(h.dw, (int64_t)h.Cout * h.N);
+    if (kw < 0) return NQ_ERR_INVALID;
+    fed[kw] = true;
+    int kb = -1;
+    if (h.db) {
+      kb = consumer(h.db, h.Cout);
+      if (kb < 0) return NQ_ERR_INVALID;
+      fed[kb] = true;
+    }
+    t.r[t.nred] = h; t.rw[t.nred] = kw; t.rb[t.nred] = kb;
+    t.rblk0[t.nred] = blocks;
+    blocks += nq_wgr_blocks(h);
+    ++t.nred;
+  }
+  t.rblk0[t.nred] = blocks;
+  t.ntw = ntiny;
+  int tb = 0;
+  for (int i = 0; i < ntiny; ++i) {
+    const nq_tiny_wg_seg& h = tiny[i];
+    if (!nq_tiny_wg_valid(h)) return NQ_ERR_INVALID;
+    const int kw = consumer(h.dw, (int64_t)h.Cout * h.Cin);
+    if (kw < 0) return NQ_ERR_INVALID;
+    fed[kw] = true;
+    int kb = -1;
+    if (h.db) {
+      kb = consumer(h.db, h.Cout);
+      if (kb < 0) return NQ_ERR_INVALID;
+      fed[kb] = true;
+    }
+    t.tw[i] = h; t.tww[i] = kw; t.twb[i] = kb;
+    t.tblk0[i] = tb;
+    tb += nq_tiny_wg_blocks(h);
+  }
+  t.tblk0[ntiny] = tb;
+  t.tail_b = -1;
+  t.tail = nq_head_tail{nullptr, nullptr, nullptr, 0, 0.f};
+  if (tail) {
+    if (!tail->ws || !tail->loss || !tail->db || tail->waves <= 0) return NQ_ERR_INVALID;
+    t.tail = *tail;
+    t.tail_b = consumer(tail->db, 3);
+    if (t.tail_b >= 0) fed[t.tail_b] = true;
+  }
+  t.np = 0;
+  int pb = 0;
+  for (int k = 0; k < nseg; ++k) {
+    if (fed[k]) continue;
+    t.s[k].vec = t.s[k].vec && ((uintptr_t)segs[k].gy & 15) == 0;
+    t.pseg[t.np] = k;
+    t.pblk0[t.np] = pb;
+    pb += (int)((t.s[k].n + TPB * EPT - 1) / (TPB * EPT));
+    ++t.np;
+  }
+  t.pblk0[t.np] = pb;
+  hipLaunchKernelGGL(reduce_adaround_adam_kernel, dim3((unsigned)(blocks + tb + pb + (tail ? 4 : 0))), dim3(TPB), 0, nq_s(stream), t,
+                     reg_b, step_size, beta1, beta2, eps, bc2_sqrt, dyn);
+  return nq_launch_status();
+}
+
 int nq_adam_step_multi(const nq_adam_seg* segs, int nseg, float step_size, float beta1, float beta2, float eps,
                        float bc2_sqrt, nq_stream_t stream) {
   return adam_multi(segs, nseg, step_size, beta1, beta2, eps, bc2_sqrt, nullptr, stream);
diff --git a/neuroquant_amd/csrc/tiny_wgrad.h b/neuroquant_amd/csrc/tiny_wgrad.h
--- /dev/null
+++ b/neuroquant_amd/csrc/tiny_wgrad.h
@@ -0,0 +1,39 @@
+#pragma once
+#include "nq_common.h"
+
+__device__ __forceinline__ float nq_tiny_pw_wgrad_elem(const float* __restrict__ x, const float* __restrict__ dy, int B, int Cin,
+                                                       int HW, int Cout, int64_t t) {
+  const int64_t nw = (int64_t)Cout * Cin;
+  float acc = 0.f;
+  if (t < nw) {
+    const int co = (int)(t / Cin), ci = (int)(t - (int64_t)co * Cin);
+    for (int b = 0; b < B; ++b) {
+      const float* __restrict__ dp = dy + ((int64_t)b * Cout + co) * HW;
+      const float* __restrict__ xp = x + ((int64_t)b * Cin + ci) * HW;
+      if ((HW & 7) == 0) {
+        for (int p = 0; p < HW; p += 8) {
+          const float4 d0 = *reinterpret_cast<const float4*>(dp + p), d1 = *reinterpret_cast<const float4*>(dp + p + 4);
+          const float4 x0 = *reinterpret_cast<const float4*>(xp + p), x1 = *reinterpret_cast<const float4*>(xp + p + 4);
+          acc = fmaf(d0.x, x0.x, acc); acc = fmaf(d0.y, x0.y, acc); acc = fmaf(d0.z, x0.z, acc); acc = fmaf(d0.w, x0.w, acc);
+          acc = fmaf(d1.x, x1.x, acc); acc = fmaf(d1.y, x1.y, acc); acc = fmaf(d1.z, x1.z, acc); acc = fmaf(d1.w, x1.w, acc);
+        }
+      } else {
+        for (int p = 0; p < HW; ++p) acc = fmaf(dp[p], xp[p], acc);
+      }
+    }
+  } else {
+    const int co = (int)(t - nw);
+    for (int b = 0; b < B; ++b) {
+      const float* __restrict__ dp = dy + ((int64_t)b * Cout + co) * HW;
+      for (int p = 0; p < HW; ++p) acc += dp[p];
+    }
+  }
+  return acc;
+}
+
+static inline bool nq_tiny_wg_valid(const nq_tiny_wg_seg& h) {
+  return h.x && h.dy && h.dw && h.B > 0 && h.Cin > 0 && h.HW > 0 && h.Cout > 0;
+}
+static inline int nq_tiny_wg_blocks(const nq_tiny_wg_seg& h) {
+  return (int)(((int64_t)h.Cout * h.Cin + (h.db ? h.Cout : 0) + 255) / 256);
+}
diff --git a/neuroquant_amd/csrc/wgrad_reduce.h b/neuroquant_amd/csrc/wgrad_reduce.h
--- /dev/null
+++ b/neuroquant_amd/csrc/wgrad_reduce.h
@@ -0,0 +1,50 @@
+#pragma once
+#include "nq_common.h"
+
+__device__ __forceinline__ bool nq_wgr_sum(const nq_wgr_seg& q, int blk, float4* __restrict__ part , float4& s,
+                                           int64_t& i, int& co, int& n) {
+  const int SG = q.sg, OG = 256 / SG;
+  const int o = threadIdx.x % OG, g = threadIdx.x / OG;
+  const int N = q.N, Cout = q.Cout, nsplit = q.nsplit;
+  const int NQ = (N + 3) >> 2;
+  i = (int64_t)blk * OG + o;
+  const int64_t total = (int64_t)Cout * NQ;
+  s = make_float4(0.f, 0.f, 0.f, 0.f);
+  co = 0;
+  n = 0;
+  if (i < total) {
+    co = (int)(i / NQ);
+    n = 4 * (int)(i - (int64_t)co * NQ);
+    const float* p = q.slab + (int64_t)co * q.n_pad + n;
+    const int64_t stride = (int64_t)q.co_pad * q.n_pad;
+#pragma unroll 8
+    for (int j = g; j < nsplit; j += SG) {
+      const float4 v = *reinterpret_cast<const float4*>(p + j * stride);
+      s.x += v.x; s.y += v.y; s.z += v.z; s.w += v.w;
+    }
+  } else if (q.db && i < total + Cout) {
+    const int cb = (int)(i - total);
+#pragma unroll 8
+    for (int j = g; j < nsplit; j += SG) s.x += q.slab_db[(int64_t)j * q.co_pad + cb];
+  }
+  if (SG > 1) {
+    part[g * OG + o] = s;
+    __syncthreads();
+    if (g != 0) return false;
+    s = part[o];
+    for (int j = 1; j < SG; ++j) {
+      const float4 v = part[j * OG + o];
+      s.x += v.x; s.y += v.y; s.z += v.z; s.w += v.w;
+    }
+  }
+  return true;
+}
+
+static inline int nq_wgr_blocks(const nq_wgr_seg& h) {
+  const int og = 256 / h.sg;
+  return (int)(((int64_t)h.Cout * ((h.N + 3) / 4) + h.Cout + og - 1) / og);
+}
+static inline bool nq_wgr_valid(const nq_wgr_seg& h) {
+  return h.slab && h.dw && h.Cout > 0 && h.N > 0 && h.nsplit > 0 && (h.sg == 1 || h.sg == 4 || h.sg == 16) &&
+         !(h.db && !h.slab_db);
+}
diff --git a/neuroquant_amd/ops.py b/neuroquant_amd/ops.py
--- a/neuroquant_amd/ops.py
+++ b/neuroquant_amd/ops.py
@@ -241,7 +241,7 @@
     return outs
 
 
-def adaround_adam_multi(items, opt, reg_b=0.0, dyn=None, beta1=0.9, beta2=0.999, eps=1e-8):
+def adaround_adam_multi(items, opt, reg_b=0.0, dyn=None, beta1=0.9, beta2=0.999, eps=1e-8, tail=None):
     assert len(items) == len(opt.params)
     opt.t += 1
     segs = (L.AdaAdamSeg * len(items))()
@@ -255,6 +255,36 @@
         sg.x, sg.gy, sg.alpha, sg.delta, sg.zp, sg.m, sg.v = _p(x), _p(gy), _p(alpha), _p(delta), _p(zp), _p(opt.m[i]), _p(opt.v[i])
         sg.rows, sg.row_len, sg.per_row, sg.n_levels, sg.reg_weight = rows, rl, per_row, n_levels, float(reg_weight)
     step_size, bc2_sqrt = opt.scalars(opt.t, beta1, beta2)
+    if tail is not None and not tail.empty():
+        def feed(idx, numel):
+            if idx >= len(items) or items[idx][0].numel() != numel:
+                raise RuntimeError("adaround_adam_multi: with a StepTail the items must be the decoder's (weight, bias) pairs in layer order")
+            return segs[idx].gy
+
+        if tail.pending is not None:
+            for sg, l in zip(tail.pending.segs, tail.pending.layers):
+                if sg.nsplit > 0:
+                    sg.dw = feed(2 * l, sg.Cout * sg.N)
+                    if sg.db:
+                        sg.db = feed(2 * l + 1, sg.Cout)
+        for sg, _, l in tail.tiny:
+            sg.dw = feed(2 * l, sg.Cout * sg.Cin)
+            if sg.db:
+                sg.db = feed(2 * l + 1, sg.Cout)
+        if tail.head is not None and tail.head_layer is not None:
+            tail.head[0].db = feed(2 * tail.head_layer + 1, 3)
+        reds = tail.pending.segs if tail.pending is not None else []
+        arr = (L.WgrSeg * max(1, len(reds)))(*reds)
+        tiny = (L.TinyWgSeg * max(1, len(tail.tiny)))(*[t[0] for t in tail.tiny])
+        head = ctypes.byref(tail.head[0]) if tail.head is not None else None
+        rc = L.lib().nq_reduce_adaround_adam_multi(segs, len(items), arr, len(reds), tiny, len(tail.tiny), head, float(reg_b),
+                                                   step_size, beta1, beta2, eps, bc2_sqrt, _p(dyn), _stream())
+        if rc != -2:
+            L.check(rc, "reduce_adaround_adam_multi")
+            tail.clear()
+            return
+    if tail is not None:
+        tail.finish()
     L.check(L.lib().nq_adaround_adam_multi(segs, len(items), float(reg_b), step_size, beta1, beta2, eps, bc2_sqrt, _p(dyn),
                                            _stream()), "adaround_adam_multi")
 
@@ -629,7 +659,7 @@
 class PendingReductions:
 
     def __init__(self):
-        self.segs, self.keep = [], []
+        self.segs, self.keep, self.layers = [], [], []
 
     def add(self, seg, *tensors):
         self.segs.append(seg)
@@ -639,7 +669,7 @@
         if self.segs:
             arr = (L.WgrSeg * len(self.segs))(*self.segs)
             L.check(L.lib().nq_wgrad_reduce_multi(arr, len(self.segs), _stream()), "wgrad_reduce_multi")
-        self.segs, self.keep = [], []
+        self.segs, self.keep, self.layers = [], [], []
 
 
 def conv_wgrad3_raw(x, dy, cout, k, want_db, out=None, defer=None, fmt=0):
@@ -710,6 +740,18 @@
     return dw, db
 
 
+def tiny_wgrad_describe(x, dy, cout, k, want_db):
+    B, cin, H, W = x.shape
+    dw = torch.empty((cout, cin, k, k), device=x.device, dtype=torch.float32)
+    db = torch.empty(cout, device=x.device, dtype=torch.float32) if want_db else None
+    seg = L.TinyWgSeg()
+    rc = L.lib().nq_tiny_pw_wgrad_describe(_p(x), _p(dy), _p(dw), _p(db), B, cin, H, W, cout, k, ctypes.byref(seg))
+    if rc == -2:
+        return None
+    L.check(rc, "tiny_pw_wgrad_describe")
+    return seg, dw, db
+
+
 class _ConvFn(Function):
 
     @staticmethod
@@ -1063,7 +1105,47 @@
         _LOSS_TLS.req = prev
 
 
-def head_forward_loss_raw(x, wt, dims, bias, cout, k, tgt=None, cache_u8=None, idx=None):
+_TAIL_TLS = threading.local()
+
+
+class StepTail:
+    def __init__(self, reduce=True, loss=True, tiny=True):
+        self.want_reduce, self.want_loss, self.want_tiny = bool(reduce), bool(loss), bool(tiny)
+        self.pending = None
+        self.tiny = []
+        self.head = None
+        self.head_layer = None
+
+    def clear(self):
+        self.pending = self.head = None
+        self.tiny = []
+        self.head_layer = None
+
+    def empty(self):
+        return self.pending is None and self.head is None and not self.tiny
+
+    def finish(self):
+        if self.head is not None:
+            L.check(L.lib().nq_head_loss_finish(ctypes.byref(self.head[0]), _stream()), "head_loss_finish")
+        if self.tiny:
+            arr = (L.TinyWgSeg * len(self.tiny))(*[t[0] for t in self.tiny])
+            L.check(L.lib().nq_tiny_pw_wgrad_multi(arr, len(self.tiny), _stream()), "tiny_pw_wgrad_multi")
+        if self.pending is not None:
+            self.pending.flush()
+        self.clear()
+
+
+@contextlib.contextmanager
+def step_tail(tail):
+    prev = getattr(_TAIL_TLS, "req", None)
+    _TAIL_TLS.req = tail
+    try:
+        yield tail
+    finally:
+        _TAIL_TLS.req = prev
+
+
+def head_forward_loss_raw(x, wt, dims, bias, cout, k, tgt=None, cache_u8=None, idx=None, tail=None):
     B, cin, H, W = x.shape
     if cout != 3 or k != 3 or (W & 3) or (dims[1] & 3) or os.environ.get("NQ_HEAD_FWD") == "1":
         return None
@@ -1084,12 +1166,21 @@
     loss = torch.empty((), device=x.device, dtype=torch.float32)
     db = torch.empty(cout, device=x.device, dtype=torch.float32)
     ws = torch.empty(_q("nq_head_forward_loss_ws_floats", B, H, W), device=x.device, dtype=torch.float32)
-    rc = _timed(("conv_igemm", k, cin, cout, H, W, B, EPI_TANH),
-                lambda: L.lib().nq_head_forward_loss(_p(x), _p(wt), dims[1], _p(bias), _p(y), _p(tgt), _p(cache_u8), _p(idx), _p(loss),
-                                                     _p(dconv), _p(db), _p(ws), B, cin, H, W, B * H * W, 1.0, _stream()))
+    if tail is not None:
+        desc = L.HeadTail()
+        rc = _timed(("conv_igemm", k, cin, cout, H, W, B, EPI_TANH),
+                    lambda: L.lib().nq_head_forward_loss_deferred(_p(x), _p(wt), dims[1], _p(bias), _p(y), _p(tgt), _p(cache_u8),
+                                                                  _p(idx), _p(loss), _p(dconv), _p(db), _p(ws), B, cin, H, W,
+                                                                  B * H * W, 1.0, ctypes.byref(desc), _stream()))
+    else:
+        rc = _timed(("conv_igemm", k, cin, cout, H, W, B, EPI_TANH),
+                    lambda: L.lib().nq_head_forward_loss(_p(x), _p(wt), dims[1], _p(bias), _p(y), _p(tgt), _p(cache_u8), _p(idx), _p(loss),
+                                                         _p(dconv), _p(db), _p(ws), B, cin, H, W, B * H * W, 1.0, _stream()))
     if rc == -2:
         return None
     L.check(rc, "head_forward_loss")
+    if tail is not None:
+        tail.head = (desc, (ws, loss))
     return y, loss, dconv, db
 
 
@@ -1174,7 +1265,10 @@
             fused_loss = None
             if last and epi == EPI_TANH and not use3 and getattr(_LOSS_TLS, "req", None) is not None:
                 tgt_, cache_, idx_ = _LOSS_TLS.req
-                fused_loss = head_forward_loss_raw(x, wt, dims, b, cout, k, tgt_, cache_, idx_)
+                tail_ = getattr(_TAIL_TLS, "req", None)
+                if tail_ is not None and not (tail_.want_loss and tail_.head is None and _arena_state()[0] is None):
+                    tail_ = None
+                fused_loss = head_forward_loss_raw(x, wt, dims, b, cout, k, tgt_, cache_, idx_, tail=tail_)
             if fused_loss is not None:
                 y, z = fused_loss[0], None
             elif use3:
@@ -1197,6 +1291,7 @@
         ctx.spec, ctx.metas, ctx.n = spec, metas, n
         ctx.save_for_backward(x, *saved_in, *saved_z)
         ctx.nq_arena, ctx.nq_arena_reduced = _arena_state(), False
+        ctx.nq_tail = getattr(_TAIL_TLS, "req", None)
         ctx.nq_head = _HeadHandoff() if spec.tanh_out else None
         if fused_loss is not None:
             ctx.nq_head.loss, ctx.nq_head.dconv, ctx.nq_head.db = fused_loss[1], fused_loss[2], fused_loss[3]
@@ -1265,6 +1360,13 @@
     pending = PendingReductions() if side is None and os.environ.get("NQ_DEFER_REDUCE", "1") != "0" else None
 
     def wgrad(l, dconv):
+        n0 = len(pending.segs) if pending is not None else 0
+        res = wgrad_of(l, dconv)
+        if pending is not None:
+            pending.layers += [l] * (len(pending.segs) - n0)
+        return res
+
+    def wgrad_of(l, dconv):
         k, r, act, cout, cin, in_gelu, wbk, dims_b, has_b, W3, x_split, g_split = metas[l]
         x_in = xs[l]
         Bx, _, Hx, Wx = x_in.shape
@@ -1275,12 +1377,21 @@
         if spec.precision == "bf16x3" and not in_gelu and cout <= 4 and cin > 4 and cout * k * k <= 64 \
                 and conv_wgrad3_supported(Bx, cout, Hx, Wx, cin, k):
             if l == n - 1 and has_b and head_db is not None:
+                tail_ = getattr(ctx, "nq_tail", None)
+                if tail_ is not None and tail_.head is not None and tail_.head[0].db == head_db.data_ptr():
+                    tail_.head_layer = l
                 dw, _ = conv_wgrad_swapped3(x_in, dconv, cout, k, False, out=out, defer=pending)
                 if out is not None:
                     out[1].copy_(head_db)
                     return dw, out[1]
                 return dw, head_db
             return conv_wgrad_swapped3(x_in, dconv, cout, k, has_b, out=out, defer=pending)
+        tail_ = getattr(ctx, "nq_tail", None)
+        if tail_ is not None and tail_.want_tiny and arena is None and side is None and not in_gelu:
+            d = tiny_wgrad_describe(x_in, dconv, cout, k, has_b)
+            if d is not None:
+                tail_.tiny.append((d[0], (x_in, dconv), l))
+                return d[1], d[2]
         return conv_wgrad_raw(x_in, dconv, cout, k, has_b, x_gelu=in_gelu, out=out, defer=pending)
 
     def dgrad(l, dconv):
@@ -1351,7 +1462,12 @@
         main.wait_stream(side)
         keep.clear()
     if pending is not None:
-        pending.flush()
+        tail = getattr(ctx, "nq_tail", None)
+        if tail is not None and tail.want_reduce and tail.pending is None and arena is None:
+            tail.pending = pending
+            pending.keep = [t[:1] for t in pending.keep]
+        else:
+            pending.flush()
     if arena is not None:
         yield arena, None
         ctx.nq_arena_reduced = True
diff --git a/neuroquant_amd/quantization/calib_model.py b/neuroquant_amd/quantization/calib_model.py
--- a/neuroquant_amd/quantization/calib_model.py
+++ b/neuroquant_amd/quantization/calib_model.py
@@ -264,8 +264,16 @@
                     for i, L in enumerate(layers):
                         L._finish(fq[2 * i], fq[2 * i + 1])
             node = None
+            tail = None
+            if ada and not hadamard and not dp and probe is None and staged is None and device.type == 'cuda' \
+                    and os.environ.get("NQ_FUSED_ADAM", "1") != "0":
+                tail = ops.StepTail(reduce=os.environ.get("NQ_FUSE_REDUCE", "1") != "0",
+                                    loss=os.environ.get("NQ_FUSE_LOSS_TAIL", "1") != "0" and not want_log,
+                                    tiny=os.environ.get("NQ_FUSE_TINY_WGRAD", "1") != "0")
+                if not (tail.want_reduce or tail.want_loss or tail.want_tiny):
+                    tail = None
             loss_req = ops.fused_head_loss(cache_u8=img[0], idx=img[1]) if isinstance(img, tuple) else ops.fused_head_loss(tgt=img)
-            with loss_req:
+            with loss_req, ops.step_tail(tail):
                 if staged is None:
                     img_out, _, _ = model(inputs)
                 else:
@@ -326,7 +334,7 @@
                                   weight if (reg_on or dyn is not None) else 0.0))
                     items.append((L.bias, gb, bq.alpha.data, bq.delta.data, bq.zero_point, bq.n_levels, 0.0))
                 if probe is None and os.environ.get("NQ_FUSED_ADAM", "1") != "0":
-                    ops.adaround_adam_multi(items, opt, b, dyn=dyn)
+                    ops.adaround_adam_multi(items, opt, b, dyn=dyn, tail=tail)
                     grads = None
                 else:
                     grads = ops.adaround_backward_multi(items, b, dyn=dyn)
```
